# ut-vision/Rot-MVGaze

Hardware: AMD Instinct MI355X
Metric: multi-view samples/sec (fwd+bwd), BxVx3x224x224 (higher is better)
Workload: dtype f32; 1 GPU; C3: ResNet-50, V=4, B=128 per GPU, 3x224x224, fwd+loss+bwd; backbone=ResNet-50, views=4, batch_per_gpu=128, global_batch=128, image=3x224x224, parallelism=dp1, weights=random init, seed 0 (kaiming-normal convs, default Linear), rccl_ranks=1, step_launch=eager: every kernel queued from Python

## Files before the change

include/rotmvgaze.h:

```cpp
#ifndef ROTMVGAZE_H
#define ROTMVGAZE_H

#include <stddef.h>
#include <stdint.h>

#ifdef __cplusplus
extern "C" {
#endif

#define MVG_ABI_VERSION 11

int mvg_abi_version(void);
const char *mvg_last_error(void);
int mvg_device_cus(void);
int mvg_set_scratch(void *ptr, size_t bytes, void *stream);
size_t mvg_scratch_bytes(void);
void *mvg_stream_create_low_priority(void);
int mvg_set_reserved_cus(int n);

enum {
  MVG_K_CONV_FPROP = 0, MVG_K_CONV_DGRAD = 1, MVG_K_CONV_WGRAD = 2, MVG_K_WGRAD_REDUCE = 3,
  MVG_K_BN_FINALIZE = 4, MVG_K_BN_APPLY = 5, MVG_K_BN_BWD_REDUCE = 6, MVG_K_BN_BWD_APPLY = 7,
  MVG_K_POOL = 8, MVG_K_LAYOUT = 9, MVG_K_LINEAR_FPROP = 10, MVG_K_LINEAR_DGRAD = 11,
  MVG_K_LINEAR_WGRAD = 12, MVG_K_ROTCAT = 13, MVG_K_COLSUM = 14, MVG_K_LOSS = 15,
// ... 203 lines not shown
                           int fout, void *stream);
int mvg_linear_dgrad_mixed(const float *dy, const void *wt_bf16, const float *mask, const float *addend, float *dx,
                           int rows, int fin, int fout, void *stream);
int mvg_linear_wgrad_mixed(const float *x, const float *dy, float *dw, float *db, int rows, int fin, int fout,
                           float *workspace, int splits, int accumulate, void *stream);
int mvg_bn_apply_bf16(const uint16_t *y, const float *scale, const float *shift, const uint16_t *residual,
                      const float *res_scale, const float *res_shift, int relu, uint16_t *out, int groups,
                      int64_t rows_per_group, int c, void *stream);
int mvg_bn_bwd_reduce_bf16(const uint16_t *g, const uint16_t *act, const uint16_t *y, const float *mean,
                           const float *invstd, const float *relu_scale, const float *relu_shift, int groups,
                           int64_t rows_per_group, int c, float *s1, float *s2, float *dgamma, float *dbeta,
                           int accumulate, float *workspace, uint16_t *dz_out, void *stream);
int mvg_bn_bwd_apply_bf16(const uint16_t *g, const uint16_t *act, const uint16_t *y, const float *mean,
                          const float *invstd, const float *gamma, const float *s1, const float *s2,
                          const float *relu_scale, const float *relu_shift, int groups, int64_t rows_per_group,
                          int c, uint16_t *dy, uint16_t *dz_out, void *stream);
int mvg_bn_relu_maxpool_fwd_bf16(const uint16_t *y, const float *scale, const float *shift, uint16_t *pooled,
                                 uint8_t *argmax, int groups, int n_per_group, int h, int w, int c, int ho,
                                 int wo, void *stream);
int mvg_bn_relu_maxpool_bwd_reduce_bf16(const uint16_t *g_pooled, const uint8_t *argmax, const uint16_t *y,
                                        const float *mean, const float *invstd, const float *scale,
                                        const float *shift, int groups, int n_per_group, int h, int w, int c,
                                        int ho, int wo, float *s1, float *s2, float *dgamma, float *dbeta,
                                        int accumulate, float *workspace, void *stream);
int mvg_bn_relu_maxpool_bwd_apply_bf16(const uint16_t *g_pooled, const uint8_t *argmax, const uint16_t *y,
                                       const float *mean, const float *invstd, const float *gamma,
                                       const float *scale, const float *shift, const float *s1,
                                       const float *s2, int groups, int n_per_group, int h, int w, int c,
                                       int ho, int wo, uint16_t *dy, void *stream);
int mvg_avgpool_fwd_bf16(const uint16_t *x, float *y, int n, int hw, int c, void *stream);
int mvg_avgpool_bwd_bf16(const float *dy, uint16_t *dx, int n, int hw, int c, void *stream);
int mvg_nchw_to_nhwc8_bf16(const float *src, uint16_t *dst, int n, int c, int h, int w, void *stream);
int mvg_preprocess_u8hwc_resize_bf16(const uint8_t *src, uint16_t *dst, int n, int h, int w, int oh, int ow, float mean0,
                                     float mean1, float mean2, float std0, float std1, float std2, int swap_rb,
                                     void *stream);

int mvg_split_f32(const float *x, void *out_sp, int64_t n, float scale, void *stream);
int mvg_merge_sp(const void *x_sp, float *out, int64_t n, float inv_scale, void *stream);
int mvg_split_weights(const mvg_conv_desc *d, const float *w, void *w_krsc_sp, void *w_crsk_sp, float *stat2, void *items_dev,
                      void *stream);
int mvg_weights_prep_batch(const void *items_dev, int n, int mode, int blocks_per_item , void *stream);
int mvg_conv_stats_partials_split(const mvg_conv_desc *d, int32_t *rows_per_partial);
int mvg_conv_fprop_split(const mvg_conv_desc *d, const void *x_sp, const float *x_sinv, const void *w_sp, const float *w_sinv,
                         float *y, float *stats, void *stream);
int mvg_conv_fprop_split_affine(const mvg_conv_desc *d, const void *x_sp, const float *x_sinv, const void *w_sp, const float *w_sinv,
                                void *out, int out_sp, const float *scale, const float *shift, const void *residual,
                                int residual_sp, int relu, void *stream);
int mvg_conv_fprop_split_affine_ranged(const mvg_conv_desc *d, const void *x_sp, const float *x_sinv, const void *w_sp,
                                       const float *w_sinv, void *out, int out_sp, const float *scale, const float *shift,
                                       const void *residual, int residual_sp, int relu, uint32_t *range_word, void *stream);
int mvg_split_f32_ranged(const float *x, void *out_sp, int64_t n, float scale, uint32_t *range_word, void *stream);
int mvg_conv_dgrad_split(const mvg_conv_desc *d, const void *dy_sp, const float *dy_sinv, const void *w_crsk_sp,
                         const float *w_sinv, float *dx, const float *addend, const void *relu_mask_sp, void *stream);
int mvg_bn_apply_split(const float *y, const float *scale, const float *shift, const void *residual, int residual_sp,
                       const float *res_scale, const float *res_shift, int relu, void *out_sp, uint8_t *relu_bits,
                       int groups, int64_t rows_per_group, int c, void *stream);
int mvg_bn_bwd_reduce_split(const float *g, const uint8_t *relu_bits, const float *y, const float *mean, const float *invstd,
                            const float *relu_scale, const float *relu_shift, int groups, int64_t rows_per_group, int c,
                            float *s1, float *s2, float *dgamma, float *dbeta, int accumulate, float *workspace,
                            float *dz_out, float *mx, const float *gamma, float *dy_sinv, void *stream);
int mvg_bn_bwd_apply_split(const float *g, const float *y, const float *mean, const float *invstd, const float *gamma,
                           const float *s1, const float *s2, const float *relu_scale, const float *relu_shift,
                           int groups, int64_t rows_per_group, int c, void *dy_sp, const float *mx, float *dy_sinv,
                           int dy_sinv_ready, void *stream);
int mvg_bn_relu_maxpool_fwd_split(const float *y, const float *scale, const float *shift, void *pooled_sp,
                                  uint8_t *argmax, int groups, int n_per_group, int h, int w, int c, int ho, int wo,
                                  void *stream);
int mvg_avgpool_fwd_split(const void *x_sp, float *y, int n, int hw, int c, void *stream);
int mvg_act_scales(const void *items_dev, int n, float *slots, int n_slots, void *stream);
int mvg_bn_apply_split_scaled(const float *y, const float *scale, const float *shift, const void *residual, int residual_sp,
                              const float *res_scale, const float *res_shift, const float *res_sinv, int relu, void *out_sp,
                              const float *out_sinv, uint8_t *relu_bits, int groups, int64_t rows_per_group, int c,
                              void *stream);
int mvg_bn_relu_maxpool_fwd_split_scaled(const float *y, const float *scale, const float *shift, void *pooled_sp,
                                         const float *pooled_sinv, uint8_t *argmax, int groups, int n_per_group, int h, int w,
                                         int c, int ho, int wo, void *stream);
int mvg_avgpool_fwd_split_scaled(const void *x_sp, const float *x_sinv, float *y, int n, int hw, int c, void *stream);
int mvg_conv_dgrad_bn_partials_split(const mvg_conv_desc *d);
int mvg_conv_dgrad_split_bnreduce(const mvg_conv_desc *d, const void *dy_sp, const float *dy_sinv, const void *w_crsk_sp,
                                  const float *w_sinv, float *dx, const float *addend, const float *bn_y, const uint8_t *bn_bits,
                                  const float *bn_mean, const float *bn_invstd, const float *relu_scale, const float *relu_shift,
                                  float *partials, float *s1, float *s2, float *dgamma, float *dbeta, int accumulate,
                                  float *mx, const float *bn_gamma, float *dx_dy_sinv, void *stream);
int mvg_conv_dgrad_split_bnapply_bnreduce(const mvg_conv_desc *d, void *dy_sp, const float *dy_sinv, const float *dz, const float *y,
                                          const float *mean, const float *invstd, const float *gamma, const float *un_s1,
                                          const float *un_s2, int64_t rows_per_group, const void *w_crsk_sp, const float *w_sinv,
                                          float *dx, const float *addend, const float *bn_y, const uint8_t *bn_bits,
                                          const float *bn_mean, const float *bn_invstd, const float *relu_scale,
                                          const float *relu_shift, float *partials, float *s1, float *s2, float *dgamma, float *dbeta,
                                          int accumulate, float *mx, const float *bn_gamma, float *dx_dy_sinv, void *stream);
int mvg_conv_fprop_split_stages(const mvg_conv_desc *d);
int mvg_conv_dgrad_split_stages(const mvg_conv_desc *d, int fused_reduce);
int mvg_conv_fprop_split_bnapply(const mvg_conv_desc *d, void *out_sp, const float *out_sinv, const float *bn_y, const float *scale,
                                 const float *shift, const void *residual, int residual_sp, const float *res_scale,
                                 const float *res_shift, const float *res_sinv, uint8_t *relu_bits, const void *w_sp,
                                 const float *w_sinv, float *y, float *stats, void *stream);
int mvg_stem_rowwindow_split(const float *x_nhwc4, void *xw_sp, int64_t images, int h, int w, void *stream);
int mvg_stem_rowwindow_split_nchw(const float *x_nchw, void *xw_sp, int64_t images, int h, int w, void *stream);
int mvg_stem_fprop_split(const mvg_conv_desc *d, const void *xw_sp, const void *w_sp, const float *w_sinv, float *y, float *stats,
                         void *stream);
int mvg_stem_wgrad_splits_split(const mvg_conv_desc *d);
int mvg_stem_wgrad_split(const mvg_conv_desc *d, const void *xw_sp, const void *dy_sp, const float *dy_sinv, float *dw_rw,
                         float *workspace, int splits, int accumulate, void *stream);
int mvg_bn_relu_maxpool_bwd_reduce_split(const float *g_pooled, const uint8_t *argmax, const float *y, const float *mean,
                                         const float *invstd, const float *scale, const float *shift, int groups,
                                         int n_per_group, int h, int w, int c, int ho, int wo, float *s1, float *s2,
                                         float *dgamma, float *dbeta, int accumulate, float *workspace, float *mx, const float *gamma,
                                         float *dy_sinv, void *stream);
int mvg_bn_relu_maxpool_bwd_apply_split(const float *g_pooled, const uint8_t *argmax, const float *y, const float *mean,
                                        const float *invstd, const float *gamma, const float *scale, const float *shift,
                                        const float *s1, const float *s2, int groups, int n_per_group, int h, int w, int c,
                                        int ho, int wo, void *dy_sp, const float *mx, float *dy_sinv, int dy_sinv_ready, void *stream);
int mvg_conv_wgrad_splits_split(const mvg_conv_desc *d);
int mvg_conv_wgrad_split_tile(const mvg_conv_desc *d, int32_t *bm, int32_t *bn, int32_t *incremental);
int mvg_conv_wgrad_split(const mvg_conv_desc *d, const void *x_sp, const void *dy_sp, const float *dy_sinv, float *dw,
                         float *workspace, int splits, int accumulate, void *stream);
int mvg_conv_wgrad_split_slabs(const mvg_conv_desc *d, const void *x_sp, const void *dy_sp, const float *dy_sinv, float *workspace,
                               int splits, void *stream);
int mvg_conv_wgrad_split_xs(const mvg_conv_desc *d, const void *x_sp, const float *x_sinv, const void *dy_sp, const float *dy_sinv,
                            float *dw, float *workspace, int splits, int accumulate, void *stream);
int mvg_conv_wgrad_split_slabs_xs(const mvg_conv_desc *d, const void *x_sp, const float *x_sinv, const void *dy_sp,
                                  const float *dy_sinv, float *workspace, int splits, void *stream);
int mvg_wgrad_reduce_batch(const float *const *host_slabs, float *const *host_dw, const int64_t *host_n, const int32_t *host_splits,
                           const int32_t *host_accumulate, int n, void *stream);

int mvg_absmax_multi(const float *const *host_ptrs, const int64_t *host_counts, float *const *host_out_slots, int n, void *stream);
int mvg_fuse_build_split(const float *img_feat, const float *feat, const float *rel, const int32_t *row_img, const int32_t *row_src_f,
                         const int32_t *row_src_h, void *xf_sp, void *xh_sp, const float *am_img, const float *am_feat,
                         float *xf_sinv, float *xh_sinv, int rows, int cf, int nvec, void *stream);
int mvg_fuse_unbuild(const float *dxh, const float *dxn, const float *rel, const int32_t *seg, const int32_t *vi, float *dfeat, float *da,
                     int da_accumulate, int segments, int views, int dirs, int batch, int cf, int nvec, float *absmax, void *stream);
int mvg_linear_fprop_split(int rows, int fin, int fout, const void *x_sp, const float *x_sinv, const void *w_sp, const float *w_sinv,
                           const float *bias, int relu, void *out, int out_sp, float *out_sinv, const float *bias_absmax,
                           float *out_absmax, void *stream);
int mvg_linear_dgrad_split(int rows, int fin, int fout, const void *dy_sp, const float *dy_sinv, const void *wt_sp, const float *w_sinv,
                           float *dx, const float *addend, const void *relu_mask_sp, float *out_absmax, void *stream);
int mvg_linear_wgrad_split(int rows, int fin, int fout, const void *x_sp, const float *x_sinv, const void *dy_sp, const float *dy_sinv,
                           float *dw, float *workspace, int splits, int accumulate, void *stream);
int mvg_split_colsum(const float *g, int rows, int cols, const float *absmax, void *out_sp, float *out_sinv, float *db, int accumulate,
                     void *stream);

typedef struct mvg_session mvg_session;
typedef struct {
  int32_t depth;
  int32_t num_iter;
  int32_t views, batch;
  int32_t height, width;
  int32_t share_weights, ignore_rotmat;
  int32_t split;
  int32_t raw_u8;
  int32_t in_h, in_w, input_bgr;
} mvg_session_cfg;

int mvg_session_create(const mvg_session_cfg *cfg, mvg_session **out);
#define MVG_SESSION_FP32 0
#define MVG_SESSION_BF16 1
int mvg_session_create_ex(const mvg_session_cfg *cfg, int32_t compute, mvg_session **out);
int mvg_session_compute(const mvg_session *s);
void mvg_session_destroy(mvg_session *s);
int mvg_session_num_tensors(const mvg_session *s);
const char *mvg_session_tensor_name(const mvg_session *s, int i);
int64_t mvg_session_tensor_numel(const mvg_session *s, int i);
size_t mvg_session_workspace_bytes(const mvg_session *s);
int mvg_session_launches(const mvg_session *s);
int mvg_session_num_steps(const mvg_session *s);
const char *mvg_session_step_name(const mvg_session *s, int i);
// ... 12 lines not shown
```

rot-mvgaze_amd/_lib.py:

```python
from __future__ import annotations

import ctypes as C
import os

_HERE = os.path.dirname(os.path.abspath(__file__))
LIB_PATH = os.path.join(_HERE, "csrc", "librotmvgaze_hip.so")

K_FAMILIES = 18
ABI_VERSION = 11
SESSION_FP32, SESSION_BF16 = 0, 1


class ConvDesc(C.Structure):
    _fields_ = [(n, C.c_int32) for n in
                ("groups", "n", "h", "w", "cin", "cout", "r", "s", "stride", "pad", "ho", "wo")]

    @classmethod
    def make(cls, groups, n, h, w, cin, cout, k, stride, pad):
        ho = (h + 2 * pad - k) // stride + 1
        wo = (w + 2 * pad - k) // stride + 1
        return cls(groups, n, h, w, cin, cout, k, k, stride, pad, ho, wo)

    @classmethod
    def linear(cls, rows, fin, fout):
        return cls(1, rows, 1, 1, fin, fout, 1, 1, 1, 0, 1, 1)


class ProfEntry(C.Structure):
    _fields_ = [("launches", C.c_int64), ("ms", C.c_double), ("flops", C.c_double), ("bytes", C.c_double)]


class SessionCfg(C.Structure):
    _fields_ = [(n, C.c_int32) for n in
                ("depth", "num_iter", "views", "batch", "height", "width", "share_weights", "ignore_rotmat", "split", "raw_u8",
                 "in_h", "in_w", "input_bgr")]


_P = C.c_void_p
_I = C.c_int
_I64 = C.c_int64
_F = C.c_float
_D = C.POINTER(ConvDesc)

SIGNATURES = {
    "mvg_abi_version": (_I, []),
    "mvg_last_error": (C.c_char_p, []),
    "mvg_device_cus": (_I, []),
    "mvg_set_scratch": (_I, [_P, C.c_size_t, _P]),
    "mvg_scratch_bytes": (C.c_size_t, []),
    "mvg_set_reserved_cus": (_I, [_I]),
    "mvg_stream_create_low_priority": (_P, []),
    "mvg_prof_enable": (_I, [_I]),
    "mvg_prof_reset": (_I, []),
    "mvg_prof_collect": (_I, [C.POINTER(ProfEntry)]),
    "mvg_prof_family_name": (C.c_char_p, [_I]),
    "mvg_conv_fprop": (_I, [_D, _P, _P, _P, _P, _I, _P, _P]),
    "mvg_conv_fprop_affine": (_I, [_D, _P, _P, _P, _P, _P, _P, _I, _P]),
    "mvg_conv_stats_partials": (_I, [_D, C.POINTER(C.c_int32)]),
    "mvg_conv_dgrad": (_I, [_D, _P, _P, _P, _P, _P, _P]),
    "mvg_conv_wgrad": (_I, [_D, _P, _P, _P, _P, _I, _I, _P]),
    "mvg_conv_wgrad_splits": (_I, [_D]),
    "mvg_linear_wgrad": (_I, [_P, _P, _P, _P, _I, _I, _I, _P, _I, _I, _P]),
    "mvg_fuser_fprop": (_I, [_P, _P, _P, _P, _P, _P, _P, _I, _P, _I, _I, _I, _I, _I, _I, _P, C.c_size_t, _P]),
    "mvg_fuser_wgrad": (_I, [_P, _P, _P, _P, _P, _P, _P, _P, _I, _I, _I, _I, _I, _I, _P, _I, _I, _P]),
    "mvg_linear_workspace_floats": (C.c_size_t, [_I, _I, _I]),
    "mvg_linear_fprop": (_I, [_P, _P, _P, _I, _P, _I, _I, _I, _P, C.c_size_t, _P]),
    "mvg_linear_dgrad": (_I, [_P, _P, _P, _P, _P, _I, _I, _I, _P, C.c_size_t, _P]),
    "mvg_bn_finalize": (_I, [_P, _I, _I, _I, _I64, _I, _P, _P, _P, _P, _F, _F, _P, _P, _P, _P, _P]),
    "mvg_bn_eval_affine": (_I, [_I, _I, _P, _P, _P, _P, _F, _P, _P, _P]),
    "mvg_bn_eval_affine_batch": (_I, [_P, _I, _I, _F, _P]),
    "mvg_bn_apply": (_I, [_P, _P, _P, _P, _P, _P, _I, _P, _I, _I64, _I, _P]),
    "mvg_bn_bwd_reduce": (_I, [_P, _P, _P, _P, _P, _P, _P, _I, _I64, _I, _P, _P, _P, _P, _I, _P, _P, _P]),
    "mvg_split_f32": (_I, [_P, _P, _I64, _F, _P]),
    "mvg_merge_sp": (_I, [_P, _P, _I64, _F, _P]),
    "mvg_split_weights": (_I, [_D, _P, _P, _P, _P, _P, _P]),
    "mvg_weights_prep_batch": (_I, [_P, _I, _I, _I, _P]),
    "mvg_conv_stats_partials_split": (_I, [_D, C.POINTER(C.c_int32)]),
    "mvg_conv_fprop_split": (_I, [_D, _P, _P, _P, _P, _P, _P, _P]),
    "mvg_conv_fprop_split_affine": (_I, [_D, _P, _P, _P, _P, _P, _I, _P, _P, _P, _I, _I, _P]),
    "mvg_conv_dgrad_split": (_I, [_D, _P, _P, _P, _P, _P, _P, _P, _P]),
    "mvg_bn_apply_split": (_I, [_P, _P, _P, _P, _I, _P, _P, _I, _P, _P, _I, _I64, _I, _P]),
    "mvg_bn_bwd_apply_split": (_I, [_P, _P, _P, _P, _P, _P, _P, _P, _P, _I, _I64, _I, _P, _P, _P, _I, _P]),
    "mvg_bn_bwd_reduce_split": (_I, [_P, _P, _P, _P, _P, _P, _P, _I, _I64, _I, _P, _P, _P, _P, _I, _P, _P, _P, _P, _P, _P]),
    "mvg_bn_relu_maxpool_fwd_split": (_I, [_P, _P, _P, _P, _P, _I, _I, _I, _I, _I, _I, _I, _P]),
    "mvg_avgpool_fwd_split": (_I, [_P, _P, _I, _I, _I, _P]),
    "mvg_act_scales": (_I, [_P, _I, _P, _I, _P]),
    "mvg_bn_apply_split_scaled": (_I, [_P, _P, _P, _P, _I, _P, _P, _P, _I, _P, _P, _P, _I, _I64, _I, _P]),
    "mvg_bn_relu_maxpool_fwd_split_scaled": (_I, [_P, _P, _P, _P, _P, _P, _I, _I, _I, _I, _I, _I, _I, _P]),
    "mvg_avgpool_fwd_split_scaled": (_I, [_P, _P, _P, _I, _I, _I, _P]),
    "mvg_conv_wgrad_split_xs": (_I, [_D, _P, _P, _P, _P, _P, _P, _I, _I, _P]),
    "mvg_conv_wgrad_split_slabs_xs": (_I, [_D, _P, _P, _P, _P, _P, _I, _P]),
    "mvg_stem_rowwindow_split": (_I, [_P, _P, _I64, _I, _I, _P]),
    "mvg_stem_rowwindow_split_nchw": (_I, [_P, _P, _I64, _I, _I, _P]),
    "mvg_stem_fprop_split": (_I, [_D, _P, _P, _P, _P, _P, _P]),
    "mvg_stem_wgrad_splits_split": (_I, [_D]),
    "mvg_stem_wgrad_split": (_I, [_D, _P, _P, _P, _P, _P, _I, _I, _P]),
    "mvg_bn_relu_maxpool_bwd_reduce_split": (_I, [_P, _P, _P, _P, _P, _P, _P, _I, _I, _I, _I, _I, _I, _I, _P, _P, _P, _P, _I, _P, _P, _P, _P, _P]),
    "mvg_bn_relu_maxpool_bwd_apply_split": (_I, [_P, _P, _P, _P, _P, _P, _P, _P, _P, _P, _I, _I, _I, _I, _I, _I, _I, _P, _P, _P, _I, _P]),
    "mvg_conv_dgrad_bn_partials_split": (_I, [_D]),
    "mvg_conv_dgrad_split_bnreduce": (_I, [_D, _P, _P, _P, _P, _P, _P, _P, _P, _P, _P, _P, _P, _P, _P, _P, _P, _P, _I, _P, _P, _P, _P]),
    "mvg_conv_dgrad_split_bnapply_bnreduce": (_I, [_D] + [_P] * 9 + [_I64] + [_P] * 15 + [_I, _P, _P, _P, _P]),
    "mvg_conv_fprop_split_stages": (_I, [_D]),
    "mvg_conv_dgrad_split_stages": (_I, [_D, _I]),
    "mvg_conv_fprop_split_bnapply": (_I, [_D] + [_P] * 6 + [_I] + [_P] * 9),
    "mvg_conv_wgrad_splits_split": (_I, [_D]),
    "mvg_conv_wgrad_split_tile": (_I, [_D, C.POINTER(C.c_int32), C.POINTER(C.c_int32), C.POINTER(C.c_int32)]),
    "mvg_conv_wgrad_split": (_I, [_D, _P, _P, _P, _P, _P, _I, _I, _P]),
    "mvg_conv_wgrad_split_slabs": (_I, [_D, _P, _P, _P, _P, _I, _P]),
    "mvg_wgrad_reduce_batch": (_I, [C.POINTER(C.c_void_p), C.POINTER(C.c_void_p), C.POINTER(C.c_int64), C.POINTER(C.c_int32),
                                    C.POINTER(C.c_int32), _I, _P]),
    "mvg_bn_apply_bits": (_I, [_P, _P, _P, _P, _P, _P, _P, _P, _I, _I64, _I, _P]),
    "mvg_bn_bwd_reduce_bits": (_I, [_P, _P, _P, _P, _P, _I, _I64, _I, _P, _P, _P, _P, _I, _P, _P, _P]),
    "mvg_bn_apply_bits_bf16": (_I, [_P, _P, _P, _P, _P, _P, _P, _P, _I, _I64, _I, _P]),
    "mvg_bn_bwd_reduce_bits_bf16": (_I, [_P, _P, _P, _P, _P, _I, _I64, _I, _P, _P, _P, _P, _I, _P, _P, _P]),
    "mvg_bn_bwd_workspace_floats": (C.c_size_t, [_I, _I64, _I]),
    "mvg_bn_bwd_apply": (_I, [_P, _P, _P, _P, _P, _P, _P, _P, _P, _P, _I, _I64, _I, _P, _P, _P]),
    "mvg_maxpool3x3s2_fwd": (_I, [_P, _P, _P, _I, _I, _I, _I, _I, _I, _P]),
    "mvg_maxpool3x3s2_bwd": (_I, [_P, _P, _P, _I, _I, _I, _I, _I, _I, _P]),
    "mvg_bn_relu_maxpool_fwd": (_I, [_P, _P, _P, _P, _P, _I, _I, _I, _I, _I, _I, _I, _P]),
    "mvg_bn_relu_maxpool_bwd_reduce": (_I, [_P, _P, _P, _P, _P, _P, _P, _I, _I, _I, _I, _I, _I, _I, _P, _P, _P, _P, _I, _P,
                                            _P]),
    "mvg_bn_relu_maxpool_bwd_apply": (_I, [_P, _P, _P, _P, _P, _P, _P, _P, _P, _P, _I, _I, _I, _I, _I, _I, _I, _P, _P]),
    "mvg_bn_eval_bwd": (_I, [_P, _P, _P, _P, _P, _P, _P, _P, _P, _F, _I, _I64, _I, _P, _P, _P, _P, _I, _P, _P]),
    "mvg_bn_eval_bwd_workspace_floats": (C.c_size_t, [_I, _I64, _I]),
    "mvg_bn_relu_maxpool_eval_bwd": (_I, [_P, _P, _P, _P, _P, _P, _P, _P, _F, _I, _I, _I, _I, _I, _I, _I, _P, _P, _P, _I, _P,
                                          _P]),
    "mvg_avgpool_fwd": (_I, [_P, _P, _I, _I, _I, _P]),
    "mvg_avgpool_bwd": (_I, [_P, _P, _I, _I, _I, _P]),
    "mvg_nchw_to_nhwc4": (_I, [_P, _P, _I, _I, _I, _I, _P]),
    "mvg_nhwc4_to_nchw": (_I, [_P, _P, _I, _I, _I, _I, _P]),
    "mvg_preprocess_u8hwc": (_I, [_P, _P, _I, _I, _I, _F, _F, _F, _F, _F, _F, _I, _P]),
    "mvg_gaze_lp_loss": (_I, [_P, _P, _I, _I, _P, _P, _P]),
    "mvg_preprocess_u8hwc_resize": (_I, [_P, _P, _I, _I, _I, _I, _I, _F, _F, _F, _F, _F, _F, _I, _P]),
    "mvg_multi_erase_nchw": (_I, [_P, _P, _P, _I, _I, _I, _I, _I, _P]),
    "mvg_rotation_matrix_2d": (_I, [_P, _P, _I, _I, _P]),
    "mvg_relative_rotation": (_I, [_P, _P, _P, _P, _I, _I, _I, _P]),
    "mvg_rotcat_fwd": (_I, [_P, _P, _P, _P, _P, _P, _I, _I, _I, _I, _P]),
    "mvg_rotcat_bwd": (_I, [_P, _P, _P, _P, _I, _I, _I, _I, _P]),
    "mvg_rotcat_ext_fwd": (_I, [_P, _P, _P, _P, _P, _P, _P, _I, _I, _I, _I, _I, _P]),
    "mvg_rotcat_ext_bwd": (_I, [_P, _I, _P, _P, _P, _I, _I, _I, _I, _P]),
    "mvg_ibn_scales": (_I, [_P, _P, _P, _P, _P, _I, _F, _F, _P, _I, _I, _I, _P]),
    "mvg_paircat_fwd": (_I, [_P, _P, _P, _P, _P, _P, _P, _I, _I, _I, _P]),
    "mvg_paircat_bwd": (_I, [_P, _P, _P, _P, _P, _P, _I, _I, _I, _P]),
    "mvg_segment_sum": (_I, [_P, _I64, _I, _P, _P, _I, _I, _I, _I, _P]),
    "mvg_axpby": (_I, [_P, _P, _F, _F, _I64, _P]),
    "mvg_scale_by": (_I, [_P, _P, _P, _I64, _P]),
    "mvg_linear_skinny_fwd": (_I, [_P, _P, _P, _P, _I, _I, _I, _P]),
    "mvg_linear_skinny_bwd": (_I, [_P, _P, _P, _P, _P, _P, _P, _I, _I, _I, _I, _P, _P]),
    "mvg_adam_step": (_I, [_P, _P, _P, _P, _I64, _F, _F, _F, _F, _F, _I, _P]),
    "mvg_gaze_angular_loss": (_I, [_P, _P, _I, _F, _P, _I, _P, _P, _P]),
    "mvg_gaze_angular_loss_multi": (_I, [_P, _P, _I, _I, _I, C.POINTER(C.c_float), _P, _P, _P]),
    "mvg_adam_step_dev": (_I, [_P, _P, _P, _P, _I64, _P, _P, _F, _F, _F, _F, _P]),
    "mvg_absmax_multi": (_I, [C.POINTER(C.c_void_p), C.POINTER(C.c_int64), C.POINTER(C.c_void_p), _I, _P]),
    "mvg_fuse_build_split": (_I, [_P, _P, _P, _P, _P, _P, _P, _P, _P, _P, _P, _P, _I, _I, _I, _P]),
    "mvg_fuse_unbuild": (_I, [_P, _P, _P, _P, _P, _P, _P, _I, _I, _I, _I, _I, _I, _I, _P, _P]),
    "mvg_linear_fprop_split": (_I, [_I, _I, _I, _P, _P, _P, _P, _P, _I, _P, _I, _P, _P, _P, _P]),
    "mvg_linear_dgrad_split": (_I, [_I, _I, _I, _P, _P, _P, _P, _P, _P, _P, _P, _P]),
    "mvg_linear_wgrad_split": (_I, [_I, _I, _I, _P, _P, _P, _P, _P, _P, _I, _I, _P]),
    "mvg_split_colsum": (_I, [_P, _I, _I, _P, _P, _P, _P, _I, _P]),
    "mvg_cast_weights_bf16": (_I, [_D, _P, _I, _P, _P, _P]),
    "mvg_conv_fprop_bf16": (_I, [_D, _P, _P, _P, _P, _I, _P, _P]),
    "mvg_conv_stats_partials_bf16": (_I, [_D, C.POINTER(C.c_int32)]),
    "mvg_conv_fprop_bf16_affine": (_I, [_D, _P, _P, _P, _P, _P, _P, _I, _P]),
    "mvg_conv_dgrad_bf16": (_I, [_D, _P, _P, _P, _P, _P, _P]),
    "mvg_conv_dgrad_bn_partials_bf16": (_I, [_D]),
    "mvg_conv_dgrad_bf16_bnreduce": (_I, [_D, _P, _P, _P, _P, _P, _P, _P, _P, _P, _P, _P, _P, _P, _P, _P, _I, _P]),
    "mvg_conv_wgrad_bf16": (_I, [_D, _P, _P, _P, _P, _I, _I, _P]),
    "mvg_stem_rowwindow_bf16": (_I, [_P, _P, _I64, _I, _I, _P]),
    "mvg_stem_fprop_bf16": (_I, [_D, _P, _P, _P, _P, _P]),
    "mvg_stem_wgrad_splits_bf16": (_I, [_D]),
    "mvg_stem_wgrad_bf16": (_I, [_D, _P, _P, _P, _P, _I, _I, _P]),
    "mvg_conv_wgrad_splits_bf16": (_I, [_D]),
    "mvg_conv_wgrad_bf16_slabs": (_I, [_D, _P, _P, _P, _I, _P]),
    "mvg_linear_fprop_mixed": (_I, [_P, _P, _P, _I, _P, _I, _I, _I, _P]),
    "mvg_linear_dgrad_mixed": (_I, [_P, _P, _P, _P, _P, _I, _I, _I, _P]),
    "mvg_linear_wgrad_mixed": (_I, [_P, _P, _P, _P, _I, _I, _I, _P, _I, _I, _P]),
    "mvg_bn_apply_bf16": (_I, [_P, _P, _P, _P, _P, _P, _I, _P, _I, _I64, _I, _P]),
    "mvg_bn_bwd_reduce_bf16": (_I, [_P, _P, _P, _P, _P, _P, _P, _I, _I64, _I, _P, _P, _P, _P, _I, _P, _P, _P]),
    "mvg_bn_bwd_apply_bf16": (_I, [_P, _P, _P, _P, _P, _P, _P, _P, _P, _P, _I, _I64, _I, _P, _P, _P]),
    "mvg_bn_relu_maxpool_fwd_bf16": (_I, [_P, _P, _P, _P, _P, _I, _I, _I, _I, _I, _I, _I, _P]),
    "mvg_bn_relu_maxpool_bwd_reduce_bf16": (_I, [_P, _P, _P, _P, _P, _P, _P, _I, _I, _I, _I, _I, _I, _I, _P, _P, _P, _P, _I,
                                                 _P, _P]),
    "mvg_bn_relu_maxpool_bwd_apply_bf16": (_I, [_P, _P, _P, _P, _P, _P, _P, _P, _P, _P, _I, _I, _I, _I, _I, _I, _I, _P, _P]),
# ... 56 lines not shown
```

rot-mvgaze_amd/backbone.py:

```python
from __future__ import annotations

import math
import os
from dataclasses import dataclass
from typing import Callable, Dict, List, NamedTuple, Optional

import numpy as np
import torch

from . import ops
from ._lib import ConvDesc
from .arch import RANGE_OVER_BITS, BackboneSpec, ConvSpec, backbone_spec, range_unit_names

Tensor = torch.Tensor
BN_EPS, BN_MOMENTUM = 1e-5, 0.1
IMAGE_MEAN, IMAGE_STD = (0.485, 0.456, 0.406), (0.229, 0.224, 0.225)


BN_APPLY_DGRAD_MAX_COUT = 512


def bn_apply_dgrad_eligible(c: ConvSpec, *, split: bool, trained: bool, fused_in: bool, carries_reduce: bool,
                            need_dimg: bool = False) -> bool:
    return bool(split and trained and not need_dimg and fused_in and carries_reduce
                and c.k == 1 and c.stride == 1 and c.pad == 0 and c.cin in (64, 128)
                and c.cout % 32 == 0 and c.cout <= BN_APPLY_DGRAD_MAX_COUT)


def bn_apply_dgrad_units(spec: BackboneSpec, *, split: bool = True, bf16: bool = False, training: bool = True,
                         need_dimg: bool = False, fuse_bn_split: bool = True, enabled: bool = True) -> List[str]:
    on = enabled and split and not bf16 and fuse_bn_split
    nb = len(spec.blocks)
    return [blk.convs[-1].name for bi, blk in reversed(list(enumerate(spec.blocks)))
            if bn_apply_dgrad_eligible(blk.convs[-1], split=on, trained=training, fused_in=bi < nb - 1,
                                       carries_reduce=len(blk.convs) > 1, need_dimg=need_dimg)]


BN_APPLY_FPROP_MAX_CIN = 512


def bn_apply_fprop_eligible(producer: ConvSpec, consumer: ConvSpec, *, split: bool, trained: bool, residual: bool = True,
                            relu: bool = True, single_stage: bool = True) -> bool:
    return bool(split and trained and residual and relu and single_stage
                and consumer.k == 1 and consumer.stride == 1 and consumer.pad == 0 and consumer.cout in (64, 128)
                and consumer.cin == producer.cout and consumer.cin % 32 == 0 and consumer.cin <= BN_APPLY_FPROP_MAX_CIN)


def bn_apply_fprop_pairs(spec: BackboneSpec, *, split: bool = True, bf16: bool = False, training: bool = True, enabled: bool = True,
                         single_stage: Optional[Callable[[ConvSpec], bool]] = None) -> List[tuple]:
    on = enabled and split and not bf16
    return [(a.convs[-1].name, b.convs[0].name) for a, b in zip(spec.blocks[:-1], spec.blocks[1:])
            if bn_apply_fprop_eligible(a.convs[-1], b.convs[0], split=on, trained=training,
                                       single_stage=True if single_stage is None else single_stage(b.convs[0]))]


class GradSink:

    def view(self, p: torch.nn.Parameter) -> Tensor:
        raise NotImplementedError

    def accumulate(self, p: torch.nn.Parameter) -> bool:
        raise NotImplementedError

    def publish(self, ps: List[torch.nn.Parameter]) -> None:
        raise NotImplementedError


@dataclass(slots=True)
class _Unit:
    spec: Optional[ConvSpec] = None
    desc: Optional[ConvDesc] = None
    x_in: Optional[Tensor] = None
    y: Optional[Tensor] = None
    out: Optional[Tensor] = None
    mean: Optional[Tensor] = None
    invstd: Optional[Tensor] = None
    relu: bool = False
    rows: int = 0
    w: Optional[Tensor] = None
    trained: bool = True
    pool: Optional[tuple] = None
    relu_affine: Optional[tuple] = None
    fused_s12: Optional[object] = None
    relu_bits: Optional[Tensor] = None
    split: bool = False
    stem_rw: bool = False


class _Fwd(NamedTuple):
    out: Tensor
    affine: Optional[tuple] = None
    pending: Optional[tuple] = None


class Backbone:
    _guard_scale = 1
    _debug_units: Optional[list] = None

    def __init__(self, depth: int, params: Dict[str, Tensor], prefix: str = "_feat_extractor.0."):
        self.spec: BackboneSpec = backbone_spec(depth, prefix)
        self.p = params
        self.fc_dim = self.spec.fc_dim
        self.overlap_wgrad = True
        self.overlap_head = True
        self.wgrad_low_priority = True
        self.grad_streams: List[torch.cuda.Stream] = []
        self._wg_stream: Optional[torch.cuda.Stream] = None
        self._wg_low = True
        self.act_dtype = torch.float32
        self.relu_bits = True
        self.split = os.environ.get("MVG_SPLIT", "1") != "0"
        self.fuse_bn_split = True
        self.fuse_bn_apply_dgrad = True
        self.fuse_bn_apply_fprop = True
        self.stem_rowwindow = True
        self.split_eval = True
        self.split_eval_guard: Optional[str] = None
        self._range_record: Optional[Tensor] = None
        self._range_slot: Dict[str, int] = {n: i for i, n in enumerate(range_unit_names(depth, prefix))}
        self._range_live = False
        self._range_tripped = False
        self.bf16_fold_eval = True
        self._wprep_infer_ok = False
        self._wk_cache: Dict[str, tuple] = {}
        self.batch_weight_prep = True
        self._wprep: Optional[Dict[str, tuple]] = None
        self._wprep_state = None
        self._wprep_versions = None
        self._ascale_state = None
        self._act_sinv: Optional[Dict[str, Tensor]] = None
        self._wg_defer: Optional[list] = None
        self._split_now = self.split
        self._stem_rw = False
        self._stem_w8 = None

    @property
    def bf16(self) -> bool:
        return self.act_dtype == torch.bfloat16

    def _prepare_weights(self, dev, reuse: bool = False) -> Dict[str, tuple]:
        mode = 0 if self.bf16 else 1
        stem_rw = self._stem_rw
        convs = [c for c in self.spec.all_convs() if not (mode == 1 and c.cin == 3 and not stem_rw)]
        key = (mode, stem_rw, str(dev), tuple(self.p[c.name + ".weight"].data_ptr() for c in convs))
        if self._wprep_state is None or self._wprep_state[0] != key:
            out, rows = {}, []
            wstat = torch.zeros(len(convs), 2, dtype=torch.float32, device=dev)
            self._stem_w8 = None
            for ci, c in enumerate(convs):
                wsrc = self.p[c.name + ".weight"]
                assert wsrc.is_contiguous(memory_format=torch.channels_last) or (c.k == 1 and wsrc.is_contiguous())
                rs = c.k * c.k
                if mode == 1 and c.cin == 3:
                    assert c.k == 7
                    self._stem_w8 = torch.zeros(c.cout, 7, 8, 4, dtype=torch.float32, device=dev)
                    wk = ops.sp_empty(c.cout, 7 * 32, device=dev)
                    wk.sinv = wstat[ci, 1:2]
                    out[c.name] = (wk, None)
                    rows.append([self._stem_w8.data_ptr(), wk.data_ptr(), 0, c.cout | (7 << 32), 32 | (32 << 32), wstat[ci].data_ptr()])
                    continue
                if mode == 0 and c.cin == 3 and stem_rw:
                    assert c.k == 7
                    self._stem_w8 = torch.zeros(2 * c.cout, 7, 16, 4, dtype=torch.float32, device=dev)
                    wk = torch.empty(2 * c.cout, 7, 1, 64, dtype=torch.bfloat16, device=dev)
                    out[c.name] = (wk, None)
                    rows.append([self._stem_w8.data_ptr(), wk.data_ptr(), 0, (2 * c.cout) | (7 << 32), 64 | (64 << 32), wstat[ci].data_ptr()])
                    continue
                if mode == 1:
                    wk = ops.sp_empty(c.cout, rs * c.cin, device=dev)
                    wt = ops.sp_empty(c.cin, rs * c.cout, device=dev)
                    wk.sinv = wt.sinv = wstat[ci, 1:2]
                    cin_pad = c.cin
                else:
                    cin_pad = 8 if c.cin == 3 else c.cin
                    wk = torch.empty(c.cout, c.k, c.k, cin_pad, dtype=torch.bfloat16, device=dev)
                    wt = None if c.cin == 3 else torch.empty(cin_pad, c.k, c.k, c.cout, dtype=torch.bfloat16, device=dev)
                out[c.name] = (wk, wt)
                rows.append([wsrc.data_ptr(), wk.data_ptr(), wt.data_ptr() if wt is not None else 0, c.cout | (rs << 32),
                             c.cin | (cin_pad << 32), wstat[ci].data_ptr()])
            table = torch.tensor(rows, dtype=torch.int64).to(dev)
            self._wprep_state = (key, out, table, len(rows), mode, wstat)
        elif (reuse and self._wprep_infer_ok and
              self._wprep_versions == tuple(self.p[c.name + ".weight"]._version for c in self.spec.all_convs())):
            return self._wprep_state[1]
        _, out, table, n, mode, wstat = self._wprep_state
        self._wprep_infer_ok = reuse
        if mode == 1:
            wstat.zero_()
            if self._stem_w8 is not None:
                self._stem_w8[:, :, 1:, :3].copy_(self.p[self.spec.stem.name + ".weight"].detach().permute(0, 2, 3, 1))
        elif self._stem_w8 is not None:
            wsrc, co = self.p[self.spec.stem.name + ".weight"].detach().permute(0, 2, 3, 1), self.spec.stem.cout
            self._stem_w8[:co, :, 1:8, :3].copy_(wsrc)
            self._stem_w8[co:, :, 3:10, :3].copy_(wsrc)
        ops.weights_prep_batch(table, n, mode)
        self._wprep_versions = tuple(self.p[c.name + ".weight"]._version for c in self.spec.all_convs())
# ... 368 lines not shown
    def _unit_params(self, c: ConvSpec) -> List[torch.nn.Parameter]:
        return [self.p[c.name + ".weight"], self.p[c.bn + ".weight"], self.p[c.bn + ".bias"]]

    def _bn_bwd(self, u: _Unit, g: Tensor, need_dz: bool, sink: GradSink, defer_apply: bool = False):
        if not u.trained:
            return self._bn_bwd_eval(u, g, need_dz, sink)
        c = u.spec
        G = u.y.shape[0]
        gp, bp, acc = self._bn_params(c, sink)
        if u.fused_s12 is not None and u.split:
            (s12, sinv), u.fused_s12 = u.fused_s12, None
            dy = ops.sp_empty(*u.y.shape, device=g.device)
            if defer_apply:
                dy.sinv = sinv
                dy.bn_apply = (g, u.y, u.mean, u.invstd, gp.detach(), s12[0], s12[1], u.rows)
            else:
                ops.bn_bwd_apply_split(g, u.y, u.mean, u.invstd, gp.detach(), s12[0], s12[1], G, u.rows, c.cout, dy, None, s12[2], sinv)
            return dy, (g if need_dz else None)
        if u.fused_s12 is not None:
            s12, u.fused_s12 = u.fused_s12, None
            dy = torch.empty_like(g) if need_dz else g
            ops.bn_bwd_apply(g, None, u.y, u.mean, u.invstd, gp.detach(), s12[0], s12[1], G, u.rows, c.cout, dy, None, None)
            return dy, (g if need_dz else None)
        s12 = torch.empty(3 if u.split else 2, G, c.cout, dtype=torch.float32, device=g.device)
        ra = u.relu_affine
        act = u.out if (u.relu and ra is None) else None
        if u.split:
            assert not (u.relu and ra is None) or u.relu_bits is not None
            sinv = torch.empty(1, dtype=torch.float32, device=g.device)
            bits = u.relu_bits
            ra = None if bits is not None else ra
            ops.bn_bwd_reduce_split(g, bits, u.y, u.mean, u.invstd, G, u.rows, c.cout, s12[0], s12[1], sink.view(gp), sink.view(bp),
                                    acc, s12[2], ra, dz_out=g if bits is not None else None, gamma=gp.detach(), dy_sinv=sinv)
            dy = ops.sp_empty(*u.y.shape, device=g.device)
            ops.bn_bwd_apply_split(g, u.y, u.mean, u.invstd, gp.detach(), s12[0], s12[1], G, u.rows, c.cout, dy, ra, s12[2], sinv)
            return dy, (g if need_dz else None)
        if need_dz and u.relu_bits is not None:
            ops.bn_bwd_reduce_bits(g, u.relu_bits, u.y, u.mean, u.invstd, G, u.rows, c.cout, s12[0], s12[1], sink.view(gp),
                                   sink.view(bp), acc, dz_out=g)
        else:
            ops.bn_bwd_reduce(g, act, u.y, u.mean, u.invstd, G, u.rows, c.cout, s12[0], s12[1], sink.view(gp), sink.view(bp),
                              acc, ra, dz_out=g if need_dz else None)
        if need_dz:
            dy = torch.empty_like(g)
            ops.bn_bwd_apply(g, None, u.y, u.mean, u.invstd, gp.detach(), s12[0], s12[1], G, u.rows, c.cout, dy, None, None)
            return dy, g
        ops.bn_bwd_apply(g, act, u.y, u.mean, u.invstd, gp.detach(), s12[0], s12[1], G, u.rows, c.cout, g, None, ra)
        return g, None

    def _bn_bwd_eval(self, u: _Unit, g: Tensor, need_dz: bool, sink: GradSink):
        c = u.spec
        G = u.y.shape[0]
        gp, bp, acc = self._bn_params(c, sink)
        rm, rv = self.p[c.bn + ".running_mean"], self.p[c.bn + ".running_var"]
        if u.relu_bits is not None:
            mask = {"relu_bits": u.relu_bits}
        elif u.relu_affine is not None:
            mask = {"relu_affine": u.relu_affine}
        elif u.relu:
            mask = {"act": u.out}
        else:
            mask = {}
        dy = torch.empty_like(g) if need_dz else g
        ops.bn_eval_bwd(g, u.y, gp.detach(), rm, rv, BN_EPS, G, u.rows, c.cout, dy, sink.view(gp), sink.view(bp), acc,
                        dz_out=g if need_dz else None, **mask)
        return dy, (g if need_dz else None)

    def _side(self, dev) -> "torch.cuda.Stream":
        if self._wg_stream is None or self._wg_stream.device != dev or self._wg_low != self.wgrad_low_priority:
            old = self._wg_stream if (self._wg_stream is not None and self._wg_stream.device == dev) else None
            self._wg_low = self.wgrad_low_priority
            try:
                if not self._wg_low:
                    raise RuntimeError
                self._wg_stream = ops.low_priority_stream(dev)
            except RuntimeError:
                self._wg_stream = torch.cuda.Stream(device=dev)
            if old is not None:
                self._wg_stream.wait_stream(old)
            self.grad_streams[:] = [self._wg_stream]
        return self._wg_stream

    def _conv_bwd(self, u: _Unit, dy: Tensor, need_dx: bool, addend: Optional[Tensor], sink: GradSink,
                  fuse_for: Optional[_Unit] = None):
        dx = None
        if getattr(dy, "bn_apply", None) is not None:
            dx = torch.empty(ops.sp_shape(u.x_in), dtype=torch.float32, device=dy.device)
            self._dgrad(u, dy, dx, addend, fuse_for, sink)
            need_dx = False
        if self.overlap_wgrad and dy.is_cuda:
            side = self._side(dy.device)
            side.wait_stream(torch.cuda.current_stream())
            with torch.cuda.stream(side):
                self._wgrad(u, dy, sink)
            if getattr(dy, "sinv", None) is not None:
                dy.sinv.record_stream(side)
            dy.record_stream(side)
            u.x_in.record_stream(side)
            if getattr(u.x_in, "sinv", None) is not None:
                u.x_in.sinv.record_stream(side)
        else:
            self._wgrad(u, dy, sink)
        if need_dx:
            dx = torch.empty(ops.sp_shape(u.x_in), dtype=torch.float32, device=dy.device) if u.split else torch.empty_like(u.x_in)
            self._dgrad(u, dy, dx, addend, fuse_for, sink)
        return dx

    def _wgrad(self, u: _Unit, dy: Tensor, sink: GradSink):
        c = u.spec
        wp = self.p[c.name + ".weight"]
        if u.split:
            ops.conv_wgrad_split(u.desc, u.x_in, dy, sink.view(wp), sink.accumulate(wp), defer=self._wg_defer)
        elif u.stem_rw and self.bf16:
            dw16 = torch.empty(2 * c.cout, 7, 16, 4, dtype=torch.float32, device=dy.device)
            ops.stem_wgrad_bf16(u.desc, u.x_in, dy, dw16, False)
            self._stem_grad(wp, sink, dw16[:c.cout, :, 1:8, :3], dw16[c.cout:, :, 3:10, :3])
        elif u.stem_rw:
            dw8 = torch.empty(c.cout, 7, 8, 4, dtype=torch.float32, device=dy.device)
            ops.stem_wgrad_split(u.desc, u.x_in, dy, dw8, False)
            self._stem_grad(wp, sink, dw8[:, :, 1:, :3])
        elif c.cin == 3:
            dw4 = torch.empty(c.cout, c.k, c.k, u.desc.cin, dtype=torch.float32, device=dy.device)
            ops.conv_wgrad(u.desc, u.x_in, dy, dw4, False)
            self._stem_grad(wp, sink, dw4[..., :3])
        else:
            ops.conv_wgrad(u.desc, u.x_in, dy, sink.view(wp), sink.accumulate(wp), defer=self._wg_defer if self.bf16 else None)

    @staticmethod
    def _stem_grad(wp: torch.nn.Parameter, sink: GradSink, dw: Tensor, dw_odd: Optional[Tensor] = None):
        gv = sink.view(wp).permute(0, 2, 3, 1)
        if sink.accumulate(wp):
            gv.add_(dw)
        else:
            gv.copy_(dw)
        if dw_odd is not None:
            gv.add_(dw_odd)

    def _flush_wgrad_reduces(self, dev):
        if not self._wg_defer:
            return
        if self.overlap_wgrad and dev.type == "cuda":
            with torch.cuda.stream(self._side(dev)):
                ops.wgrad_reduce_batch(self._wg_defer)
        else:
            ops.wgrad_reduce_batch(self._wg_defer)

    def _dgrad(self, u: _Unit, dy: Tensor, dx: Tensor, addend: Optional[Tensor], fuse_for: Optional[_Unit] = None,
               sink: Optional[GradSink] = None):
        U = fuse_for
        if (self.bf16 and U is not None and self.fuse_bn_split and u.spec.cin != 3 and u.desc.cin % 64 == 0 and u.desc.cout % 64 == 0
                and (not U.relu or U.relu_bits is not None or U.relu_affine is not None)):
            c = U.spec
            gp, bp, acc = self._bn_params(c, sink)
            s12 = torch.empty(2, dx.shape[0], c.cout, dtype=torch.float32, device=dx.device)
            ops.conv_dgrad_bf16_bnreduce(u.desc, dy, u.w, dx, addend, U.y, U.relu_bits, U.mean, U.invstd,
                                         None if U.relu_bits is not None else U.relu_affine, s12[0], s12[1], sink.view(gp),
                                         sink.view(bp), acc)
            U.fused_s12 = s12
            return
        if u.split:
            if U is not None and U.split and self.fuse_bn_split:
                c = U.spec
                gp, bp, acc = self._bn_params(c, sink)
                s12 = torch.empty(3, dx.shape[0], c.cout, dtype=torch.float32, device=dx.device)
                sinv = torch.empty(1, dtype=torch.float32, device=dx.device)
                ra = None if U.relu_bits is not None else U.relu_affine
                pend = getattr(dy, "bn_apply", None)
                if pend is not None:
                    dz, y, mean, invstd, gamma, us1, us2, rows = pend
                    dy.bn_apply = None
                    ops.conv_dgrad_split_bnapply_bnreduce(u.desc, dy, dy.sinv, dz, y, mean, invstd, gamma, us1, us2, rows, u.w, dx,
                                                          addend, U.y, U.relu_bits, U.mean, U.invstd, ra, s12[0], s12[1],
                                                          sink.view(gp), sink.view(bp), acc, s12[2], gp.detach(), sinv)
                else:
                    ops.conv_dgrad_split_bnreduce(u.desc, dy, u.w, dx, addend, U.y, U.relu_bits, U.mean, U.invstd, ra, s12[0], s12[1],
                                                  sink.view(gp), sink.view(bp), acc, s12[2], gp.detach(), sinv)
                U.fused_s12 = (s12, sinv)
            else:
                ops.conv_dgrad_split(u.desc, dy, u.w, dx, addend)
        else:
            ops.conv_dgrad(u.desc, dy, u.w, dx, None, addend)

    def _stem_bn_bwd(self, stem: _Unit, g: Tensor, V: int, B: int, sink: GradSink) -> Tensor:
        argmax, scale, shift, H1, W1, Hp, Wp = stem.pool
        sc = stem.spec
        P = self.p
        gp, bp, acc = self._bn_params(sc, sink)
        stem_sp = stem.stem_rw and not self.bf16
        s12 = torch.empty(3 if stem_sp else 2, V, sc.cout, dtype=torch.float32, device=g.device)
        if not stem.trained:
            dy = torch.empty_like(stem.y)
            ops.bn_relu_maxpool_eval_bwd(g, argmax, stem.y, scale, shift, gp.detach(), P[sc.bn + ".running_mean"],
                                         P[sc.bn + ".running_var"], BN_EPS, V, B, H1, W1, sc.cout, Hp, Wp, dy, sink.view(gp),
                                         sink.view(bp), acc)
        elif stem_sp:
            sinv = torch.empty(1, dtype=torch.float32, device=g.device)
            ops.bn_relu_maxpool_bwd_reduce_split(g, argmax, stem.y, stem.mean, stem.invstd, scale, shift, V, B, H1, W1, sc.cout, Hp, Wp,
                                                 s12[0], s12[1], sink.view(gp), sink.view(bp), acc, s12[2], gp.detach(), sinv)
            dy = ops.sp_empty(*stem.y.shape, device=g.device)
            ops.bn_relu_maxpool_bwd_apply_split(g, argmax, stem.y, stem.mean, stem.invstd, gp.detach(), scale, shift, s12[0], s12[1],
                                                V, B, H1, W1, sc.cout, Hp, Wp, dy, s12[2], sinv)
        else:
            ops.bn_relu_maxpool_bwd_reduce(g, argmax, stem.y, stem.mean, stem.invstd, scale, shift, V, B, H1, W1, sc.cout, Hp, Wp,
                                           s12[0], s12[1], sink.view(gp), sink.view(bp), acc)
            dy = torch.empty_like(stem.y)
            ops.bn_relu_maxpool_bwd_apply(g, argmax, stem.y, stem.mean, stem.invstd, gp.detach(), scale, shift, s12[0], s12[1],
                                          V, B, H1, W1, sc.cout, Hp, Wp, dy)
        return dy

    def backward(self, tape: dict, dfeat: Tensor, sink: GradSink, need_dimg: bool = False):
        V, B = tape["V"], tape["B"]
        units: List[_Unit] = tape["units"]
        if self.bf16 and not all(u.trained for u in units):
            raise NotImplementedError("backward through eval-mode BatchNorm (running statistics) is not implemented on the "
                                      "bf16 path: call model.train() for gradient steps, or use the fp32 model")
        Hc, Wc = tape["final_hw"]
        if need_dimg and self.bf16:
            raise NotImplementedError("d(loss)/d(img) is not produced by the bf16 path")
        if tape.get("wprep_versions") is not None and tape["wprep_versions"] != getattr(self, "_wprep_versions", None):
            raise RuntimeError("backward of a tape whose bf16 / sp weight copies were overwritten by a later forward with "
                               "DIFFERENT weights (forward, optimizer step, forward, then backward of the first call): "
                               "backward-data would run with the new weights.  Run backward before the weights change "
                               "(PyTorch raises its version-counter error in the same situation)")
        g = torch.empty(V, B, Hc, Wc, self.fc_dim, dtype=self.act_dtype, device=dfeat.device)
        ops.avgpool_bwd(dfeat.contiguous(), g, V * B, Hc * Wc, self.fc_dim)
        self._wg_defer = []
        blocks = tape["blocks"]
        for bi in range(len(blocks) - 1, -1, -1):
            idx, ds_idx = blocks[bi]
            last = units[idx[-1]]
            prev_last = units[blocks[bi - 1][0][-1]] if bi > 0 else None
            done: List[torch.nn.Parameter] = []
            below = units[idx[-2]]
            merge = self.fuse_bn_apply_dgrad and bn_apply_dgrad_eligible(
                last.spec, split=last.split and not self.bf16, trained=last.trained, fused_in=last.fused_s12 is not None,
                carries_reduce=below.split and self.fuse_bn_split, need_dimg=need_dimg)
            dy, dz = self._bn_bwd(last, g, True, sink, defer_apply=merge)
            d = self._conv_bwd(last, dy, True, None, sink, fuse_for=below)
            done += self._unit_params(last.spec)
            last.y = last.out = None
            del dy
            for k in range(len(idx) - 2, -1, -1):
                u = units[idx[k]]
                dy, _ = self._bn_bwd(u, d, False, sink)
                if k == 0:
                    d = self._conv_bwd(u, dy, True, dz if ds_idx is None else None, sink,
                                       fuse_for=prev_last if ds_idx is None else None)
                else:
                    d = self._conv_bwd(u, dy, True, None, sink, fuse_for=units[idx[k - 1]])
                done += self._unit_params(u.spec)
                u.y = u.out = None
            if ds_idx is not None:
                ud = units[ds_idx]
                dyd, _ = self._bn_bwd(ud, dz, False, sink)
                self._conv_bwd(ud, dyd, False, None, sink)
                self._dgrad(ud, dyd, d, d, prev_last, sink)
                done += self._unit_params(ud.spec)
                ud.y = ud.out = None
            self._flush_wgrad_reduces(g.device)
            sink.publish(done)
            g = d
            if "debug" in tape:
                tape["debug"].append(g.clone())
        stem = units[0]
        dy = self._stem_bn_bwd(stem, g, V, B, sink)
        dx0 = self._conv_bwd(stem, dy, need_dimg, None, sink)
        self._flush_wgrad_reduces(g.device)
        self._wg_defer = None
        sink.publish(self._unit_params(stem.spec))
        if self._wg_stream is not None and dy.is_cuda and (self.overlap_wgrad or not torch.cuda.is_current_stream_capturing()):
            torch.cuda.current_stream().wait_stream(self._wg_stream)
        if not need_dimg:
            return None
        H, W = dx0.shape[2], dx0.shape[3]
        outs = []
        for v in range(V):
            o = torch.empty(B, 3, H, W, dtype=torch.float32, device=dx0.device)
            ops.nhwc4_to_nchw(dx0[v], o, B, 3, H, W)
            outs.append(o)
        return outs
```

rot-mvgaze_amd/csrc/bf16_tile.h:

```cpp
#pragma once
#include "conv_shared.h"
#include "bn_math.h"
#include "elem.h"

namespace mvg {

typedef __bf16 bf16x8 __attribute__((ext_vector_type(8)));
typedef short s16x4 __attribute__((ext_vector_type(4)));

__device__ __forceinline__ float bf_lo(unsigned v) { return __uint_as_float(v << 16); }
__device__ __forceinline__ float bf_hi(unsigned v) { return __uint_as_float(v & 0xFFFF0000u); }
__device__ __forceinline__ unsigned pack_bf2(float a, float b) {
  const __bf16 x = (__bf16)a, y = (__bf16)b;
  return (unsigned)__builtin_bit_cast(unsigned short, x) | ((unsigned)__builtin_bit_cast(unsigned short, y) << 16);
}

__device__ __forceinline__ void ld8(const float *p, float (&v)[8]) {
  const float4 a = *reinterpret_cast<const float4 *>(p), b = *reinterpret_cast<const float4 *>(p + 4);
  v[0] = a.x; v[1] = a.y; v[2] = a.z; v[3] = a.w; v[4] = b.x; v[5] = b.y; v[6] = b.z; v[7] = b.w;
}

constexpr unsigned RANGE_OVER_BITS = 0x477FF000u;
__device__ __forceinline__ unsigned range_bits(unsigned mx, float v) {
  const unsigned b = __float_as_uint(v) & 0x7FFFFFFFu;
  return b > mx ? b : mx;
}
__device__ __forceinline__ void range_commit(unsigned mx, unsigned *lds, unsigned *__restrict__ word, int tid) {
#pragma unroll
  for (int o = 32; o > 0; o >>= 1) {
    const unsigned other = (unsigned)__shfl_xor((int)mx, o, 64);
    mx = other > mx ? other : mx;
  }
  __syncthreads();
  if ((tid & 63) == 0) lds[tid >> 6] = mx;
  __syncthreads();
  if (tid == 0) {
    unsigned m = lds[0];
    for (int k = 1; k < 4; ++k) m = lds[k] > m ? lds[k] : m;
    if (m > *word) atomicMax(word, m);
  }
}

template <int BM, int BN, int PASSES, bool BNF, bool AFF = false>
constexpr int bf16_epilogue_bytes() {
  return (BM / PASSES) * (BN + 4) * 4 + BM * 4 + (BNF ? 4 * BN * 4 : 0) + (AFF ? 2 * BN * 4 : 0);
}

template <int BM, int BN, int WGM, bool DGRAD, bool F32IO, int PASSES = 1, bool ACC16 = false, bool BNF = false, bool LIN = false, int WGN = 2,
          bool AFF = false, bool RNG = false, class AccT>
__device__ __forceinline__ void bf16_epilogue(const IgemmParams &p, const IgemmClass &c, AccT &acc,
                                              unsigned short *smem, int tid, int g, int mtile, int ntile) {
  constexpr int NT = WGM * WGN * 64;
  constexpr int WTM = BM / WGM, WTN = BN / WGN;
  constexpr int TS = ACC16 ? 16 : 32, NE = ACC16 ? 4 : 16;
  constexpr int TM = WTM / TS, TN = WTN / TS;
  constexpr int LDO = BN + 4;
  const int lane = tid & 63, wave = tid >> 6;
  const int wm = wave / WGN, wn = wave % WGN;
  const int li = ACC16 ? (lane & 15) : (lane & 31), lh = ACC16 ? (lane >> 4) : (lane >> 5);
  auto erow = [&](int e) { return ACC16 ? 4 * lh + e : (e & 3) + 8 * (e >> 2) + 4 * lh; };
  const int ohw = c.out_h * c.out_w;
  const long long row_base = (long long)mtile * BM + wm * WTM;
  const float osc = F32IO ? (p.a_sinv ? *p.a_sinv : 1.f) * (p.b_sinv ? *p.b_sinv : 1.f) : 1.f;
  float lin_scale = 1.f, lin_max = 0.f;
  unsigned rng_max = 0u;
  static_assert(!RNG || (F32IO && !DGRAD && !LIN && !BNF && !AFF && WGM * WGN == 4), "bf16_epilogue: RNG is a forward form of the split conv kernels");
  if constexpr (LIN && F32IO) {
    if (!DGRAD && p.out_sp && p.out_sinv) {
      const float bound = (float)p.ktotal * 1073741824.f * osc + (p.bias_absmax ? *p.bias_absmax : 0.f);
      lin_scale = sp_scale_for(bound);
      if (tid == 0 && mtile == 0 && ntile == 0 && g == 0) *p.out_sinv = 1.f / lin_scale;
    }
  }
  if (!DGRAD && !AFF && p.stats) {
    long long cnt_ll = c.rows_per_group - row_base;
    const int cnt = cnt_ll <= 0 ? 0 : (cnt_ll > WTM ? WTM : (int)cnt_ll);
#pragma unroll
    for (int j = 0; j < TN; ++j) {
      const int col = ntile * BN + wn * WTN + j * TS + li;
      float csum = 0.f;
#pragma unroll
      for (int i = 0; i < TM; ++i)
#pragma unroll
        for (int e = 0; e < NE; ++e) {
          const int r = i * TS + erow(e);
          csum += (r < cnt) ? acc[i][j][e] : 0.f;
        }
      csum += __shfl_xor(csum, 32, 64);
      if (ACC16) csum += __shfl_xor(csum, 16, 64);
      const float mean = cnt > 0 ? csum / (float)cnt : 0.f;
      float q = 0.f;
#pragma unroll
      for (int i = 0; i < TM; ++i)
#pragma unroll
        for (int e = 0; e < NE; ++e) {
          const int r = i * TS + erow(e);
          const float dlt = acc[i][j][e] - mean;
          q += (r < cnt) ? dlt * dlt : 0.f;
        }
      q += __shfl_xor(q, 32, 64);
      if (ACC16) q += __shfl_xor(q, 16, 64);
      long long P = p.stats_partials ? p.stats_partials : (long long)c.mtiles_per_group * WGM;
      long long pi = (long long)mtile * WGM + wm;
      if (lh == 0 && col < p.ncols && (pi < P || p.stats_fold)) {
        int nc = p.ncols, ch = col;
        if (p.stats_fold) {
          nc = p.ncols >> 1;
          pi = 2 * pi + (col >= nc);
          ch = col - (col >= nc ? nc : 0);
          P *= 2;
        }
        float *st = p.stats + (((long long)g * P + pi) * 2) * nc;
        st[ch] = csum * osc;
        st[nc + ch] = q * (osc * osc);
      }
    }
  }
  static_assert(WGM % PASSES == 0, "bf16_epilogue: the wave rows must divide into the passes");
  constexpr int PR = BM / PASSES;
  float *ot = reinterpret_cast<float *>(smem);
  int *rowoff = reinterpret_cast<int *>(ot + PR * LDO);
  for (int r = tid; r < BM; r += NT) {
    const long long m = (long long)mtile * BM + r;
    int off = -1;
    if (m < c.rows_per_group) {
      if (DGRAD && p.cls_step == 2) {
        const int rr = (int)m;
        const int img = (int)fdiv((unsigned)rr, c.ohw_div), rem = rr - img * ohw;
        const int y2 = (int)fdiv((unsigned)rem, c.ow_div), x2 = rem - y2 * c.out_w;
        off = ((img * p.full_h + 2 * y2 + c.cls_py) * p.full_w + 2 * x2 + c.cls_px) * p.ncols;
      } else {
        off = (int)m * p.ncols;
      }
    }
    rowoff[r] = off;
  }
  const long long gelems = DGRAD ? (long long)p.imgs_per_group * p.full_h * p.full_w * p.ncols
                                 : c.rows_per_group * (long long)p.ncols;
  unsigned short *out_g = reinterpret_cast<unsigned short *>(p.out) + (long long)g * gelems;
  const unsigned short *add_g = p.addend ? reinterpret_cast<const unsigned short *>(p.addend) + (long long)g * gelems : nullptr;
  const unsigned short *mask_g = p.mask ? reinterpret_cast<const unsigned short *>(p.mask) + (long long)g * gelems : nullptr;
  float *out_f = p.out + (long long)g * gelems;
  const float *add_f = p.addend ? p.addend + (long long)g * gelems : nullptr;
  const float *mask_f = p.mask ? p.mask + (long long)g * gelems : nullptr;
  constexpr int CV = BN / 8;
  const bool bnf = BNF && DGRAD && p.bn_part != nullptr;
  bool quad = false;
  if constexpr (F32IO && DGRAD && !LIN) quad = !p.mask && (p.ncols % BN) == 0;
  float bn_s1[8], bn_s2[8], bn_mx[8];
  const bool bn_aff = bnf && p.bn_rscale != nullptr;
  float *bnc = reinterpret_cast<float *>(smem) + (BM / PASSES) * LDO + BM;
  if (bnf) {
    for (int cc = tid; cc < BN; cc += NT) {
      const int colc = ntile * BN + cc;
      const bool ok = colc < p.ncols;
      bnc[cc] = ok ? p.bn_mean[(long long)g * p.ncols + colc] : 0.f;
      bnc[BN + cc] = ok ? p.bn_invstd[(long long)g * p.ncols + colc] : 0.f;
      bnc[2 * BN + cc] = (ok && bn_aff) ? p.bn_rscale[(long long)g * p.ncols + colc] : 0.f;
      bnc[3 * BN + cc] = (ok && bn_aff) ? p.bn_rshift[(long long)g * p.ncols + colc] : 0.f;
    }
#pragma unroll
    for (int k = 0; k < 8; ++k) bn_s1[k] = bn_s2[k] = bn_mx[k] = 0.f;
  }
  float *affc = reinterpret_cast<float *>(smem) + (BM / PASSES) * LDO + BM;
  if constexpr (AFF) {
    static_assert(!DGRAD && !F32IO && !BNF && !LIN, "bf16_epilogue: AFF is the forward form of the bf16 storage kernels");
    for (int cc = tid; cc < BN; cc += NT) {
      const int colc = ntile * BN + cc;
      const bool ok = colc < p.ncols;
      affc[cc] = ok ? p.scale[colc] : 0.f;
      affc[BN + cc] = ok ? p.bias[colc] : 0.f;
    }
  }
#pragma unroll
  for (int ph = 0; ph < PASSES; ++ph) {
  if (PASSES > 1 && ph > 0) __syncthreads();
  if (wm / (WGM / PASSES) == ph) {
#pragma unroll
    for (int i = 0; i < TM; ++i)
#pragma unroll
      for (int j = 0; j < TN; ++j)
#pragma unroll
        for (int e = 0; e < NE; ++e)
          ot[((wm % (WGM / PASSES)) * WTM + i * TS + erow(e)) * LDO + wn * WTN + j * TS + li] = acc[i][j][e];
  }
  __syncthreads();
  auto store_rows = [&](int it) {
    const int v = tid + it * NT;
    const int rl = v / CV, cv = v - rl * CV;
    const int r = ph * PR + rl;
    const int col = ntile * BN + cv * 8;
    const int off = rowoff[r];
    if (off < 0 || col >= p.ncols) return;
    const float4 lo = *reinterpret_cast<const float4 *>(ot + rl * LDO + cv * 8);
    const float4 hi = *reinterpret_cast<const float4 *>(ot + rl * LDO + cv * 8 + 4);
    float x[8] = {lo.x, lo.y, lo.z, lo.w, hi.x, hi.y, hi.z, hi.w};
    if constexpr (F32IO) {
#pragma unroll
      for (int k = 0; k < 8; ++k) x[k] *= osc;
    }
    if constexpr (AFF) {
      asm volatile("" ::: "memory");
      float sa[8], sb[8];
      ld8(affc + cv * 8, sa);
      ld8(affc + BN + cv * 8, sb);
#pragma unroll
      for (int k = 0; k < 8; ++k) x[k] = __builtin_fmaf(x[k], sa[k], sb[k]);
      if (add_g) {
        const u32x4 a = *reinterpret_cast<const u32x4 *>(add_g + off + col);
        const unsigned aa[4] = {a.x, a.y, a.z, a.w};
#pragma unroll
        for (int k = 0; k < 4; ++k) {
          x[2 * k] += bf_lo(aa[k]);
          x[2 * k + 1] += bf_hi(aa[k]);
        }
      }
      if (p.relu) {
#pragma unroll
        for (int k = 0; k < 8; ++k) x[k] = fmaxf(x[k], 0.f);
      }
      u32x4 o;
      o.x = pack_bf2(x[0], x[1]);
      o.y = pack_bf2(x[2], x[3]);
      o.z = pack_bf2(x[4], x[5]);
      o.w = pack_bf2(x[6], x[7]);
      *reinterpret_cast<u32x4 *>(out_g + off + col) = o;
// ... 96 lines not shown
        typedef float f4v __attribute__((ext_vector_type(4)));
        f4v s0 = {x[0], x[1], x[2], x[3]}, s1 = {x[4], x[5], x[6], x[7]};
        __builtin_nontemporal_store(s0, reinterpret_cast<f4v *>(out_f + off + col));
        __builtin_nontemporal_store(s1, reinterpret_cast<f4v *>(out_f + off + col + 4));
      } else {
        *reinterpret_cast<float4 *>(out_f + off + col) = make_float4(x[0], x[1], x[2], x[3]);
        *reinterpret_cast<float4 *>(out_f + off + col + 4) = make_float4(x[4], x[5], x[6], x[7]);
      }
      return;
    }
    if (mask_g) {
      const u32x4 m = *reinterpret_cast<const u32x4 *>(mask_g + off + col);
      const unsigned mm[4] = {m.x, m.y, m.z, m.w};
#pragma unroll
      for (int k = 0; k < 4; ++k) {
        x[2 * k] = bf_lo(mm[k]) > 0.f ? x[2 * k] : 0.f;
        x[2 * k + 1] = bf_hi(mm[k]) > 0.f ? x[2 * k + 1] : 0.f;
      }
    }
    if (add_g) {
      const u32x4 a = *reinterpret_cast<const u32x4 *>(add_g + off + col);
      const unsigned aa[4] = {a.x, a.y, a.z, a.w};
#pragma unroll
      for (int k = 0; k < 4; ++k) {
        x[2 * k] += bf_lo(aa[k]);
        x[2 * k + 1] += bf_hi(aa[k]);
      }
    }
    u32x4 o;
    if (bnf) {
      const u32x4 yv = *reinterpret_cast<const u32x4 *>(reinterpret_cast<const unsigned short *>(p.bn_y) + (long long)g * gelems + off + col);
      const unsigned yw[4] = {yv.x, yv.y, yv.z, yv.w};
      unsigned bits = p.bn_bits ? (unsigned)p.bn_bits[((long long)g * gelems + off + col) >> 3] : 0xFFu;
      asm volatile("" ::: "memory");
      if (bn_aff) {
        float bn_ra[8], bn_rb[8];
        ld8(bnc + 2 * BN + cv * 8, bn_ra);
        ld8(bnc + 3 * BN + cv * 8, bn_rb);
        bits = 0u;
#pragma unroll
        for (int k = 0; k < 4; ++k) {
          bits |= (relu_on(bf_lo(yw[k]), bn_ra[2 * k], bn_rb[2 * k]) ? 1u : 0u) << (2 * k);
          bits |= (relu_on(bf_hi(yw[k]), bn_ra[2 * k + 1], bn_rb[2 * k + 1]) ? 1u : 0u) << (2 * k + 1);
        }
      }
      unsigned ow[4];
#pragma unroll
      for (int k = 0; k < 4; ++k) {
        const float y0 = bf_lo(yw[k]), y1 = bf_hi(yw[k]);
        const bool on0 = ((bits >> (2 * k)) & 1u) != 0u, on1 = ((bits >> (2 * k + 1)) & 1u) != 0u;
        ow[k] = pack_bf2(on0 ? x[2 * k] : 0.f, on1 ? x[2 * k + 1] : 0.f);
        const float d0 = bf_lo(ow[k]), d1 = bf_hi(ow[k]);
        bn_s1[2 * k] += d0;
        bn_s1[2 * k + 1] += d1;
        bn_s2[2 * k] = __builtin_fmaf(d0, y0, bn_s2[2 * k]);
        bn_s2[2 * k + 1] = __builtin_fmaf(d1, y1, bn_s2[2 * k + 1]);
      }
      o.x = ow[0]; o.y = ow[1]; o.z = ow[2]; o.w = ow[3];
    } else {
      o.x = pack_bf2(x[0], x[1]);
      o.y = pack_bf2(x[2], x[3]);
      o.z = pack_bf2(x[4], x[5]);
      o.w = pack_bf2(x[6], x[7]);
    }
    *reinterpret_cast<u32x4 *>(out_g + off + col) = o;
  };
  if (quad) {
    constexpr int HB = BN / 2;
    const int cq = tid % CV;
    const int cA = cq * 4, cB = HB + cq * 4;
    const int colA = ntile * BN + cA, colB = ntile * BN + cB;
#pragma unroll 1
    for (int it = 0; it < PR * CV / NT; ++it) {
      const int rl = (tid + it * NT) / CV;
      const int off = rowoff[ph * PR + rl];
      if (off < 0) continue;
      const float4 qa = *reinterpret_cast<const float4 *>(ot + rl * LDO + cA);
      const float4 qb = *reinterpret_cast<const float4 *>(ot + rl * LDO + cB);
      float x[8] = {qa.x * osc, qa.y * osc, qa.z * osc, qa.w * osc, qb.x * osc, qb.y * osc, qb.z * osc, qb.w * osc};
      if (add_f) {
        const float4 a0 = *reinterpret_cast<const float4 *>(add_f + off + colA), a1 = *reinterpret_cast<const float4 *>(add_f + off + colB);
        x[0] += a0.x; x[1] += a0.y; x[2] += a0.z; x[3] += a0.w; x[4] += a1.x; x[5] += a1.y; x[6] += a1.z; x[7] += a1.w;
      }
      if (bnf) {
        const float *yg = p.bn_y + (long long)g * gelems + off;
        const float4 y0 = *reinterpret_cast<const float4 *>(yg + colA), y1 = *reinterpret_cast<const float4 *>(yg + colB);
        const float yy[8] = {y0.x, y0.y, y0.z, y0.w, y1.x, y1.y, y1.z, y1.w};
        unsigned bits = 0xFFu;
        if (p.bn_bits) {
          const uint8_t *bb = p.bn_bits + (((long long)g * gelems + off) >> 2);
          bits = (bb[colA >> 2] & 0xFu) | ((bb[colB >> 2] & 0xFu) << 4);
        }
        asm volatile("" ::: "memory");
        auto ld44 = [&](const float *base, float (&v)[8]) {
          const float4 u = *reinterpret_cast<const float4 *>(base + cA), w = *reinterpret_cast<const float4 *>(base + cB);
          v[0] = u.x; v[1] = u.y; v[2] = u.z; v[3] = u.w; v[4] = w.x; v[5] = w.y; v[6] = w.z; v[7] = w.w;
        };
        if (bn_aff) {
          float bn_ra[8], bn_rb[8];
          ld44(bnc + 2 * BN, bn_ra);
          ld44(bnc + 3 * BN, bn_rb);
#pragma unroll
          for (int k = 0; k < 8; ++k) bits = (bits & ~(1u << k)) | ((relu_on(yy[k], bn_ra[k], bn_rb[k]) ? 1u : 0u) << k);
        }
        float bn_mu[8], bn_is[8];
        ld44(bnc, bn_mu);
        ld44(bnc + BN, bn_is);
#pragma unroll
        for (int k = 0; k < 8; ++k) {
          x[k] = ((bits >> k) & 1u) != 0u ? x[k] : 0.f;
          bn_mx[k] = fmaxf(bn_mx[k], fabsf(x[k]));
          bn_s1[k] += x[k];
          bn_s2[k] += x[k] * xhat(yy[k], bn_mu[k], bn_is[k]);
        }
      }
      if (p.nt_out) {
        typedef float f4v __attribute__((ext_vector_type(4)));
        const f4v s0 = {x[0], x[1], x[2], x[3]}, s1 = {x[4], x[5], x[6], x[7]};
        __builtin_nontemporal_store(s0, reinterpret_cast<f4v *>(out_f + off + colA));
        __builtin_nontemporal_store(s1, reinterpret_cast<f4v *>(out_f + off + colB));
      } else {
        *reinterpret_cast<float4 *>(out_f + off + colA) = make_float4(x[0], x[1], x[2], x[3]);
        *reinterpret_cast<float4 *>(out_f + off + colB) = make_float4(x[4], x[5], x[6], x[7]);
      }
    }
    continue;
  }
  bool plain4 = false;
  if constexpr (F32IO && !LIN) plain4 = p.nt_out && !p.scale && !p.bias && !p.addend && !p.mask && !p.out_sp && !bnf && !p.relu;
  if (plain4) {
    constexpr int CV4 = BN / 4;
#pragma unroll
    for (int it = 0; it < PR * CV4 / NT; ++it) {
      const int v = tid + it * NT;
      const int rl = v / CV4, c4 = v - rl * CV4;
      const int col = ntile * BN + c4 * 4;
      const int off = rowoff[ph * PR + rl];
      if (off < 0 || col >= p.ncols) continue;
      const float4 q = *reinterpret_cast<const float4 *>(ot + rl * LDO + c4 * 4);
      typedef float f4v __attribute__((ext_vector_type(4)));
      const f4v sv = {q.x * osc, q.y * osc, q.z * osc, q.w * osc};
      __builtin_nontemporal_store(sv, reinterpret_cast<f4v *>(out_f + off + col));
    }
  } else if constexpr (BNF) {
#pragma unroll 1
    for (int it = 0; it < PR * CV / NT; ++it) store_rows(it);
  } else {
#pragma unroll
    for (int it = 0; it < PR * CV / NT; ++it) store_rows(it);
  }
  }
  if constexpr (RNG) range_commit(rng_max, reinterpret_cast<unsigned *>(smem), p.out_absmax, tid);
  if constexpr (LIN && F32IO) {
    if (p.out_absmax) {
#pragma unroll
      for (int o = 32; o > 0; o >>= 1) lin_max = fmaxf(lin_max, __shfl_xor(lin_max, o, 64));
      __syncthreads();
      float *wred = reinterpret_cast<float *>(smem);
      if (lane == 0) wred[wave] = lin_max;
      __syncthreads();
      if (tid == 0) {
        float mx = wred[0];
        for (int k = 1; k < NT / 64; ++k) mx = fmaxf(mx, wred[k]);
        if (mx > 0.f) atomicMax(p.out_absmax, __float_as_uint(mx));
      }
      __syncthreads();
// ... 44 lines not shown
```

rot-mvgaze_amd/csrc/conv_shared.h:

```cpp
#pragma once
#include <stdlib.h>

#include "common.h"

namespace mvg {


typedef float f32x16 __attribute__((ext_vector_type(16)));
typedef unsigned int u32x4 __attribute__((ext_vector_type(4)));

__device__ __forceinline__ unsigned pred_off(unsigned off, bool ok) { return off | ((unsigned)(!ok) << 31); }
__device__ __forceinline__ float4 buf_ld16(__amdgpu_buffer_rsrc_t r, unsigned byte_off) {
  const u32x4 v = __builtin_amdgcn_raw_buffer_load_b128(r, byte_off, 0, 0);
  return make_float4(__uint_as_float(v.x), __uint_as_float(v.y), __uint_as_float(v.z), __uint_as_float(v.w));
}
__device__ __forceinline__ __amdgpu_buffer_rsrc_t make_rsrc(const void *base, long long bytes) {
  unsigned n = bytes > 0x7FFFFFF0ll ? 0x7FFFFFF0u : (bytes < 0 ? 0u : (unsigned)bytes);
  const unsigned long long b = (unsigned long long)base;
  const unsigned lo = __builtin_amdgcn_readfirstlane((unsigned)b);
  const unsigned hi = __builtin_amdgcn_readfirstlane((unsigned)(b >> 32));
  n = __builtin_amdgcn_readfirstlane(n);
  void *ub = (void *)(((unsigned long long)hi << 32) | lo);
  return __builtin_amdgcn_make_buffer_rsrc(ub, 0, (int)n, 0x00020000);
}
// ... 13 lines not shown
}
__device__ __forceinline__ unsigned fdiv(unsigned n, const FastDiv &f) {
  const unsigned t = __umulhi(f.mul, n);
  return (t + ((n - t) >> f.sh1)) >> f.sh2;
}

struct IgemmClass {
  int out_h, out_w;
  int ntaps, tap_ns, tap_r0, tap_s0;
  int ktotal;
  int cls_py, cls_px, cls_cy, cls_cx;
  int mtiles_per_group;
  long long rows_per_group;
  FastDiv tap_ns_div, ohw_div, ow_div;
  int korder;
  FastDiv per_div;
  long long unit0;
  int tile0;
  int KT;
  int part0;
};

struct IgemmParams {
  const float *a;
  const float *b;
  float *out;
  const float *bias;
  const float *scale;
  const float *mask;
  const float *addend;
  float *stats;
  int relu;
  int groups;
  int out_h, out_w;
  int src_h, src_w;
  int src_c;
  int src_c_shift;
  int ncols;
  int r, s, stride_shift, stride, pad;
  int ktotal;
  int cin;
  int rs;
  long long rows_per_group;
  long long src_img_stride;
  int imgs_per_group;
  int mtiles_per_group, ntiles;
  int ntaps, tap_ns, tap_r0, tap_s0, tap_step;
  int cls_step, cls_py, cls_px, cls_cy, cls_cx;
  int full_h, full_w;
  long long a_group_bytes;
  long long b_bytes;
  FastDiv tap_ns_div;
  FastDiv ohw_div, ow_div;
  int splits, ktiles_per_split;
  float *slab;
  int sk_tiles;
  int no_remap;
  int nt_out;
  int ncls;
  IgemmClass cls[4];
  int b_row_len;
  int stats_partials;
  const float *bn_y, *bn_mean, *bn_invstd, *bn_rscale, *bn_rshift;
  float *bn_part;
  int bn_parts;
  int addend_sp, out_sp, mask_sp;
  const float *a_sinv, *b_sinv;
  unsigned *out_absmax;
  float *out_sinv;
  const float *bias_absmax;
  int stride_w, pad_w;
  int stats_fold;
  int bn_part_rows;
  const unsigned char *bn_bits;
  const float *rc_feat, *rc_rel;
  const int *rc_row_img, *rc_row_src;
  int rc_cf, rc_nvec, rc_nvec_shift;
  long long rc_img_bytes, rc_feat_bytes;
  const float *bna_dz, *bna_y, *bna_mean, *bna_invstd, *bna_gamma, *bna_s1, *bna_s2;
  float bna_inv_rows;
  const float *fap_y, *fap_scale, *fap_shift, *fap_res_scale, *fap_res_shift, *fap_res_sinv;
  const void *fap_res;
  unsigned short *fap_bits;
};

__device__ __forceinline__ int xcd_remap(int orig, int nwg) {
  const int q = nwg >> 3, rr = nwg & 7, xcd = orig & 7;
  const int base = (xcd < rr) ? xcd * (q + 1) : rr * (q + 1) + (xcd - rr) * q;
  return base + (orig >> 3);
}


struct WgradParams {
  const float *x;
  const float *dy;
  float *out;
  int h, w, cin, cout, r, s, stride, pad, ho, wo;
  int ncols;
  long long pixels;
  long long pixels_per_split;
  long long x_bytes;
  int mtiles, ntiles;
  int accumulate;
  float *db;
  const float *rc_feat, *rc_rel;
  const int *rc_row_img, *rc_row_src;
  int rc_cf, rc_nvec;
  long long rc_img_bytes, rc_feat_bytes;
  FastDiv ohw_div, wo_div, cin_div, s_div;
  const float *dy_sinv;
  const float *x_sinv;
  int stride_w, pad_w;
};

static __global__ __launch_bounds__(256) void wgrad_reduce_kernel(const float *__restrict__ slabs, float *__restrict__ dw,
                                                           long long n4, int splits, int accumulate, int lanes) {
  __shared__ float4 sh[256];
  const int cols = 256 / lanes;
  const int c = threadIdx.x % cols, l = threadIdx.x / cols;
  const long long i = (long long)blockIdx.x * cols + c;
  float4 s = make_float4(0.f, 0.f, 0.f, 0.f);
  if (i < n4)
    for (int k = l; k < splits; k += lanes) {
      const float4 v = reinterpret_cast<const float4 *>(slabs)[(long long)k * n4 + i];
      s.x += v.x;
      s.y += v.y;
      s.z += v.z;
      s.w += v.w;
    }
  sh[threadIdx.x] = s;
  __syncthreads();
  if (l == 0 && i < n4) {
    float4 t = accumulate ? reinterpret_cast<const float4 *>(dw)[i] : make_float4(0.f, 0.f, 0.f, 0.f);
    for (int k = 0; k < lanes; ++k) {
      const float4 v = sh[k * cols + c];
      t.x += v.x;
      t.y += v.y;
      t.z += v.z;
      t.w += v.w;
    }
    reinterpret_cast<float4 *>(dw)[i] = t;
  }
}

static double alg_cin(const mvg_conv_desc *d) { return d->cin == 4 ? 3.0 : (double)d->cin; }

static int ilog2_exact(int v) {
  int s = 0;
  while ((1 << s) < v) ++s;
  return ((1 << s) == v) ? s : -1;
}

static int validate(const mvg_conv_desc *d) {
  MVG_REQUIRE(d != nullptr, "conv: null descriptor");
  MVG_REQUIRE(d->groups > 0 && d->n > 0 && d->h > 0 && d->w > 0 && d->cin > 0 && d->cout > 0, "conv: bad sizes");
  MVG_REQUIRE(d->stride == 1 || d->stride == 2, "conv: stride must be 1 or 2 (got %d)", d->stride);
  MVG_REQUIRE(d->ho == (d->h + 2 * d->pad - d->r) / d->stride + 1 && d->wo == (d->w + 2 * d->pad - d->s) / d->stride + 1,
              "conv: ho/wo inconsistent with h/w/pad/stride");
  MVG_REQUIRE(d->cin % 4 == 0, "conv: cin %% 4 != 0 (%d)", d->cin);
  if (d->r * d->s > 1) {
    MVG_REQUIRE(ilog2_exact(d->cin) >= 0 && ilog2_exact(d->cout) >= 0, "conv: r*s>1 needs power-of-two channels");
  }
  MVG_REQUIRE((long long)d->n * d->ho * d->wo < (1LL << 31) && (long long)d->n * d->h * d->w < (1LL << 31),
              "conv: rows per group overflow int32");
  return 0;
}
// ... 74 lines not shown
  p.src_h = d->ho;
  p.src_w = d->wo;
  p.src_c = d->cout;
  p.src_c_shift = (d->r * d->s > 1) ? ilog2_exact(d->cout) : 0;
  p.ncols = d->cin;
  p.r = d->r;
  p.s = d->s;
  p.rs = d->r * d->s;
  p.stride = d->stride;
  p.stride_shift = d->stride == 2 ? 1 : 0;
  p.pad = d->pad;
  p.ktotal = d->r * d->s * d->cout;
  p.b_row_len = p.ktotal;
  p.cin = d->cin;
  p.src_img_stride = (long long)d->ho * d->wo * d->cout;
  p.imgs_per_group = d->n;
  p.full_h = d->h;
  p.full_w = d->w;
  p.a_group_bytes = (long long)a_elem * d->n * p.src_img_stride;
  p.b_bytes = (long long)b_elem * d->cin * p.b_row_len;
  MVG_REQUIRE(p.a_group_bytes < 0x7FFFFFF0ll && p.b_bytes < 0x7FFFFFF0ll, "%s: a group / the weights exceed 2 GiB", what);
  return 0;
}

static __global__ __launch_bounds__(256) void dgrad_empty_class_kernel(uint4 *__restrict__ dx, const uint4 *__restrict__ addend,
                                                                       long long n, int sub_h, int sub_w, int full_h, int full_w,
                                                                       int cv, int py, int px) {
  const long long stride = (long long)gridDim.x * blockDim.x;
  for (long long i = (long long)blockIdx.x * blockDim.x + threadIdx.x; i < n; i += stride) {
    const int cc = (int)(i % cv);
    long long t = i / cv;
    const int x2 = (int)(t % sub_w);
    t /= sub_w;
    const int y2 = (int)(t % sub_h);
    const long long img = t / sub_h;
    const long long off = ((img * full_h + 2 * y2 + py) * full_w + 2 * x2 + px) * cv + cc;
    dx[off] = addend ? addend[off] : make_uint4(0u, 0u, 0u, 0u);
  }
}

struct DgradDropped {
  int n;
  struct { int py, px, sub_h, sub_w; } c[4];
};
static void dgrad_plan_classes(IgemmParams &p, const mvg_conv_desc *d, bool keep_tapless, DgradDropped &dropped) {
  const int step = d->stride;
  p.ncls = 0;
  dropped.n = 0;
  for (int py = 0; py < step; ++py)
    for (int px = 0; px < step; ++px) {
      const int sub_h = (d->h - py + step - 1) / step, sub_w = (d->w - px + step - 1) / step;
      if (sub_h <= 0 || sub_w <= 0) continue;
      const int r0 = (py + d->pad) % step, s0 = (px + d->pad) % step;
      const int nr = r0 < d->r ? (d->r - r0 + step - 1) / step : 0;
      const int ns = s0 < d->s ? (d->s - s0 + step - 1) / step : 0;
      if (nr * ns == 0 && !keep_tapless) {
        dropped.c[dropped.n++] = {py, px, sub_h, sub_w};
        continue;
      }
      IgemmClass &c = p.cls[p.ncls++];
      c = make_class(d->n, sub_h, sub_w, nr * ns, ns > 0 ? ns : 1, r0, s0, d->cout);
      c.cls_py = py;
      c.cls_px = px;
      c.cls_cy = (py + d->pad - r0) / step;
      c.cls_cx = (px + d->pad - s0) / step;
      if (p.ncls == 1) {
        p.tap_step = step;
        p.cls_step = step;
        p.rows_per_group = c.rows_per_group;
        p.ktotal = c.ktotal;
        p.out_h = sub_h;
        p.out_w = sub_w;
      }
    }
  for (int i = 1; i < p.ncls; ++i)
    for (int j = i; j > 0 && p.cls[j].ktotal > p.cls[j - 1].ktotal; --j) {
      const IgemmClass t = p.cls[j];
      p.cls[j] = p.cls[j - 1];
      p.cls[j - 1] = t;
    }
  p.no_remap = p.ncls > 1;
}

static int dgrad_classes(IgemmParams &p, const mvg_conv_desc *d, bool keep_tapless, int dx_elem, void *dx, const void *addend,
                         hipStream_t st) {
  DgradDropped dropped;
  dgrad_plan_classes(p, d, keep_tapless, dropped);
  if (addend == dx && addend) return 0;
  for (int i = 0; i < dropped.n; ++i) {
    const int cv = d->cin * dx_elem / 16;
    const long long n = (long long)d->groups * d->n * dropped.c[i].sub_h * dropped.c[i].sub_w * cv;
    long long blocks = (n + 255) / 256;
    if (blocks > 4096) blocks = 4096;
    hipLaunchKernelGGL(dgrad_empty_class_kernel, dim3((unsigned)blocks), dim3(256), 0, st, (uint4 *)dx, (const uint4 *)addend, n,
                       dropped.c[i].sub_h, dropped.c[i].sub_w, d->h, d->w, cv, dropped.c[i].py, dropped.c[i].px);
    if (check_launch("dgrad(empty class)")) return 1;
  }
  return 0;
}

static int wgrad_geometry(WgradParams &p, const mvg_conv_desc *d, int elem, int px_align, float *dw, float *db, float *workspace,
                          int splits, int accumulate, const char *what, int stride_w = -1, int pad_w = -1) {
  MVG_REQUIRE(splits >= 1, "%s: splits < 1", what);
  MVG_REQUIRE(splits == 1 || workspace != nullptr, "%s: workspace required for splits > 1", what);
  p.h = d->h;
  p.w = d->w;
  p.cin = d->cin;
  p.cout = d->cout;
  p.r = d->r;
  p.s = d->s;
  p.stride = d->stride;
  p.pad = d->pad;
  p.stride_w = stride_w >= 0 ? stride_w : d->stride;
  p.pad_w = stride_w >= 0 ? pad_w : d->pad;
  p.ho = d->ho;
  p.wo = d->wo;
  p.ncols = d->r * d->s * d->cin;
  p.pixels = (long long)d->groups * d->n * d->ho * d->wo;
  p.pixels_per_split = ((p.pixels + splits - 1) / splits + px_align - 1) / px_align * px_align;
  p.x_bytes = (long long)elem * d->groups * d->n * d->h * d->w * d->cin;
  p.ohw_div = make_fastdiv((unsigned)(d->ho * d->wo));
  p.wo_div = make_fastdiv((unsigned)d->wo);
  p.cin_div = make_fastdiv((unsigned)d->cin);
  p.s_div = make_fastdiv((unsigned)d->s);
  MVG_REQUIRE(p.pixels_per_split * d->cout * elem < 0x7FFFFFF0ll, "%s: split too large for 32-bit offsets", what);
  MVG_REQUIRE((long long)elem * (p.pixels_per_split / (d->ho * d->wo) + 2) * d->h * d->w * d->cin < 0x7FFFFFF0ll,
              "%s: split too large for 32-bit offsets", what);
  p.out = splits == 1 ? dw : workspace;
  p.accumulate = (splits == 1) ? accumulate : 0;
  p.db = db ? (splits == 1 ? db : workspace + (size_t)splits * d->cout * p.ncols) : nullptr;
  return 0;
}

static int wgrad_reduce_slabs(const WgradParams &p, float *workspace, float *dw, float *db, int splits, int accumulate, hipStream_t st,
                              const char *what) {
  const long long n = (long long)p.cout * p.ncols;
  MVG_REQUIRE(n % 4 == 0, "%s: weight elements %% 4 != 0", what);
  ProfScope ps(MVG_K_WGRAD_REDUCE, st, 0.0, 4.0 * n * (splits + 1));
  const int lanes = splits >= 32 ? 16 : (splits >= 8 ? 4 : 1);
  const long long blocks = (n / 4 + 256 / lanes - 1) / (256 / lanes);
  hipLaunchKernelGGL(wgrad_reduce_kernel, dim3((unsigned)blocks), dim3(256), 0, st, workspace, dw, n / 4, splits, accumulate, lanes);
  if (check_launch("wgrad_reduce")) return 1;
  if (!db) return 0;
  const long long nb = p.cout;
  const long long bblocks = (nb / 4 + 256 / lanes - 1) / (256 / lanes);
  hipLaunchKernelGGL(wgrad_reduce_kernel, dim3((unsigned)bblocks), dim3(256), 0, st, workspace + (size_t)splits * n, db, nb / 4, splits,
                     accumulate, lanes);
  return check_launch("wgrad_reduce(bias)");
}

static int wgrad_split_count(long long tiles, long long pixels, int workgroups_per_cu, int min_pixels) {
  long long want = ((long long)workgroups_per_cu * compute_cus()) / tiles;
  long long maxs = pixels / min_pixels;
  if (maxs < 1) maxs = 1;
  if (want > maxs) want = maxs;
  if (want < 1) want = 1;
  if (want > 1024) want = 1024;
  return (int)want;
}

}
```

rot-mvgaze_amd/csrc/conv_split.hip:

```cpp
#include "bf16_tile.h"
#include "elem.h"

namespace mvg {

typedef _Float16 f16x8 __attribute__((ext_vector_type(8)));

#define SPLIT_ONE(PA, PB, av, bv, acc)                                                                         \
  _Pragma("unroll") for (int i = 0; i < TM; ++i) _Pragma("unroll") for (int j = 0; j < TN; ++j)                \
      acc[i][j] = __builtin_amdgcn_mfma_f32_32x32x16_f16(av[PA][i], bv[PB][j], acc[i][j], 0, 0, 0);
#define SPLIT_PRODUCTS(av, bv, acc) SPLIT_ONE(0, 1, av, bv, acc) SPLIT_ONE(1, 0, av, bv, acc) SPLIT_ONE(0, 0, av, bv, acc)

constexpr int SP_BM = 128, SP_BK = 32;

__global__ __launch_bounds__(256) void split_f32_kernel(const float4 *__restrict__ x, uint4 *__restrict__ out, long long n8, float scale) {
  const long long stride = (long long)gridDim.x * 256;
  for (long long i = (long long)blockIdx.x * 256 + threadIdx.x; i < n8; i += stride) {
    const float4 lo = x[2 * i], hi = x[2 * i + 1];
    const float v[8] = {lo.x * scale, lo.y * scale, lo.z * scale, lo.w * scale, hi.x * scale, hi.y * scale, hi.z * scale, hi.w * scale};
    uint4 q1, q2;
    split2_chunk(v, q1, q2);
    out[2 * i] = q1;
    out[2 * i + 1] = q2;
  }
}
// ... 246 lines not shown
  }
  __device__ __forceinline__ void consts(const float *kc, int C) {
    ld8(kc, mu);
    ld8(kc + C, is);
    ld8(kc + 2 * C, ga);
    ld8(kc + 3 * C, sa);
    ld8(kc + 4 * C, sb);
  }
  __device__ __forceinline__ void form(int i, bool ok, float (&o)[8]) {
    float d[8], v[8];
    unpack8(dzv[i], d);
    unpack8(yv[i], v);
    bn_dy_chunk(d, v, mu, is, ga, sa, sb, inv_rows, dsc, o, false, mu, mu);
#pragma unroll
    for (int k = 0; k < 8; ++k) o[k] = ok ? o[k] : 0.f;
  }
  __device__ __forceinline__ void store_extra(int, unsigned) {}
};

template <bool AFFINE>
struct OutFormer {
  static constexpr int TABLES = AFFINE ? 4 : 2;
  __amdgpu_buffer_rsrc_t rs_y, rs_r;
  float osc, rsi;
  unsigned short *bits_out;
  float4 yv[2][2], rv[2][2];
  float sc[8], sh[8], rs[8], rh[8];
  unsigned mb[2];
  static __device__ __forceinline__ void stage(float *t, const IgemmParams &p, int g, int C, int tid) {
    for (int i = tid; i < C; i += 256) {
      const long long gc = (long long)g * C + i;
      t[i] = p.fap_scale[gc];
      t[C + i] = p.fap_shift[gc];
      if constexpr (AFFINE) {
        t[2 * C + i] = p.fap_res_scale[gc];
        t[3 * C + i] = p.fap_res_shift[gc];
      }
    }
  }
  __device__ __forceinline__ OutFormer(const IgemmParams &p, long long grow0, long long rows_per_group, int C)
      : rs_y(make_rsrc(p.fap_y + grow0 * C, 4ll * rows_per_group * C)),
        rs_r(make_rsrc(reinterpret_cast<const float *>(p.fap_res) + grow0 * C, 4ll * rows_per_group * C)),
        osc(__uint_as_float(__builtin_amdgcn_readfirstlane(__float_as_uint(p.a_sinv ? 1.f / *p.a_sinv : 1.f)))),
        rsi(__uint_as_float(__builtin_amdgcn_readfirstlane(__float_as_uint((!AFFINE && p.fap_res_sinv) ? *p.fap_res_sinv : 1.f)))),
        bits_out(p.fap_bits ? p.fap_bits + grow0 * (C >> 3) : nullptr) {}
  __device__ __forceinline__ void load(int i, unsigned off) {
    yv[i][0] = buf_ld16(rs_y, off);
    yv[i][1] = buf_ld16(rs_y, off + 16u);
    rv[i][0] = buf_ld16(rs_r, off);
    rv[i][1] = buf_ld16(rs_r, off + 16u);
  }
  __device__ __forceinline__ void consts(const float *kc, int C) {
    ld8(kc, sc);
    ld8(kc + C, sh);
    if constexpr (AFFINE) {
      ld8(kc + 2 * C, rs);
      ld8(kc + 3 * C, rh);
    }
  }
  __device__ __forceinline__ void form(int i, bool ok, float (&o)[8]) {
    float v[8], r[8];
    unpack8(yv[i], v);
    if constexpr (AFFINE) {
      unpack8(rv[i], r);
    } else {
      const uint4 r1 = make_uint4(__float_as_uint(rv[i][0].x), __float_as_uint(rv[i][0].y), __float_as_uint(rv[i][0].z), __float_as_uint(rv[i][0].w));
      const uint4 r2 = make_uint4(__float_as_uint(rv[i][1].x), __float_as_uint(rv[i][1].y), __float_as_uint(rv[i][1].z), __float_as_uint(rv[i][1].w));
      merge2_chunk(r1, r2, r);
    }
    mb[i] = bn_apply_chunk(v, sc, sh, true, r, AFFINE, rs, rh, !AFFINE, rsi, true, osc, o);
#pragma unroll
    for (int k = 0; k < 8; ++k) o[k] = ok ? o[k] : 0.f;
  }
  __device__ __forceinline__ void store_extra(int i, unsigned off) {
    if (bits_out) bits_out[off >> 5] = (unsigned short)mb[i];
  }
};

#define MVG_SPLIT_RNG 0
#include "conv_split_igemm.inc"
#undef MVG_SPLIT_RNG
#define MVG_SPLIT_RNG 1
#include "conv_split_igemm.inc"
#undef MVG_SPLIT_RNG

template <int BM, int BN, bool INCR>
__global__ __launch_bounds__(256, BN >= 256 ? 2 : 3) void wgrad_split_kernel(WgradParams p) {
  constexpr int BK = 16, WGM = 2, WGN = 2;
  constexpr int WTM = BM / WGM, WTN = BN / WGN;
  constexpr int TM = WTM / 32, TN = WTN / 32;
  constexpr int LDA = BM + 32, LDB = BN + 32;
  constexpr int MV = BM / 8, NVB = BN / 8;
  constexpr int A_TPR = 256 / BK;
  constexpr int A_CPT = MV / A_TPR > 0 ? MV / A_TPR : 1;
  constexpr int B_CPT = (NVB + A_TPR - 1) / A_TPR;
  constexpr int A_ELEMS = BK * LDA, B_ELEMS = BK * LDB;
  constexpr int STAGE = SP_NP * (A_ELEMS + B_ELEMS);
  __shared__ __attribute__((aligned(16))) unsigned short smem[2 * STAGE];

  const int tid = threadIdx.x;
  const int lane = tid & 63, wave = tid >> 6;
  const int wm = wave / WGN, wn = wave % WGN;
  const int li = lane & 31, lh = lane >> 5;
  const int tiles = p.mtiles * p.ntiles;
  const int logical = xcd_remap(blockIdx.x, gridDim.x);
  const int split = logical / tiles;
  const int tile = logical - split * tiles;
  const int ntile = tile % p.ntiles, mtile = tile / p.ntiles;
  const long long m_begin = (long long)split * p.pixels_per_split;
  long long m_end = m_begin + p.pixels_per_split;
  if (m_end > p.pixels) m_end = p.pixels;
  const int m_count = m_end > m_begin ? (int)(m_end - m_begin) : 0;
  const int ohw = p.ho * p.wo;
  const long long img0 = m_begin / ohw;
  const unsigned rem0 = (unsigned)(m_begin - img0 * ohw);

  const char *dy = reinterpret_cast<const char *>(p.dy);
  const char *x = reinterpret_cast<const char *>(p.x);
  const __amdgpu_buffer_rsrc_t rs_a = make_rsrc(dy + m_begin * p.cout * SP_BYTES, (long long)SP_BYTES * m_count * p.cout);
  const long long x_img_elems = (long long)p.h * p.w * p.cin;
  const __amdgpu_buffer_rsrc_t rs_b = make_rsrc(x + img0 * x_img_elems * SP_BYTES, p.x_bytes - (long long)SP_BYTES * img0 * x_img_elems);
  const int i_row = tid / A_TPR, i_v0 = tid % A_TPR;
  unsigned a_off[A_CPT];
  bool a_on[A_CPT];
#pragma unroll
  for (int j = 0; j < A_CPT; ++j) {
    const int cv = i_v0 + j * A_TPR;
    const int col = mtile * BM + cv * 8;
    a_on[j] = cv < MV;
    a_off[j] = (a_on[j] && col < p.cout) ? (unsigned)(i_row * p.cout + col) * (unsigned)SP_BYTES : 0x80000000u;
  }
  int i_dy[B_CPT], i_dx[B_CPT];
  unsigned i_tconst[B_CPT];
  bool i_cok[B_CPT], b_on[B_CPT];
#pragma unroll
  for (int j = 0; j < B_CPT; ++j) {
    const int cv = i_v0 + j * A_TPR;
    const int col = ntile * BN + cv * 8;
    b_on[j] = cv < NVB;
    i_cok[j] = b_on[j] && col < p.ncols;
    const int tap = (int)fdiv((unsigned)(i_cok[j] ? col : 0), p.cin_div);
    const int cc = (i_cok[j] ? col : 0) - tap * p.cin;
    const int fr = (int)fdiv((unsigned)tap, p.s_div), fs = tap - fr * p.s;
    i_dy[j] = fr - p.pad;
    i_dx[j] = fs - p.pad_w;
    i_tconst[j] = (unsigned)((i_dy[j] * p.w + i_dx[j]) * p.cin + cc) * (unsigned)SP_BYTES;
  }
  const unsigned row_bytes = (unsigned)(p.stride * p.w * p.cin) * (unsigned)SP_BYTES, col_bytes = (unsigned)(p.stride_w * p.cin) * (unsigned)SP_BYTES;
  const unsigned img_bytes = (unsigned)x_img_elems * (unsigned)SP_BYTES;
  int s_oy = 0, s_ox = 0;
  unsigned s_imgoff = 0;
  if (INCR) {
    const unsigned pix = rem0 + (unsigned)i_row;
    const unsigned img = fdiv(pix, p.ohw_div);
    const unsigned rem = pix - img * (unsigned)ohw;
    const unsigned oy = fdiv(rem, p.wo_div);
    s_oy = (int)oy;
    s_ox = (int)(rem - oy * (unsigned)p.wo);
    s_imgoff = img * img_bytes;
  }
  u32x4 a_reg[A_CPT][SP_NP], b_reg[B_CPT][SP_NP];
  auto load_tiles = [&](int kt) {
#pragma unroll
    for (int j = 0; j < A_CPT; ++j) {
#pragma unroll
      for (int pc = 0; pc < SP_NP; ++pc)
// ... 169 lines not shown
}

__global__ __launch_bounds__(256) void stem_rowwindow_nchw_kernel(const float *__restrict__ x, uint4 *__restrict__ xw, long long n, int h, int w) {
  const int wo = w >> 1;
  const long long plane = (long long)h * w;
  for (long long i = (long long)blockIdx.x * 256 + threadIdx.x; i < n; i += (long long)gridDim.x * 256) {
    const int q = (int)(i & 3);
    const long long t = i >> 2;
    const int ox = (int)(t % wo);
    const long long row = t / wo;
    const long long img = row / h;
    const int yy = (int)(row - img * h);
    const int c0 = 2 * ox - 4 + 2 * q;
    float v[8] = {0.f, 0.f, 0.f, 0.f, 0.f, 0.f, 0.f, 0.f};
    if (c0 >= 0 && c0 < w) {
      const float *src = x + img * 3 * plane + (long long)yy * w + c0;
      const float2 r = *reinterpret_cast<const float2 *>(src), g = *reinterpret_cast<const float2 *>(src + plane),
                   b = *reinterpret_cast<const float2 *>(src + 2 * plane);
      v[0] = r.x; v[1] = g.x; v[2] = b.x; v[4] = r.y; v[5] = g.y; v[6] = b.y;
    }
    uint4 q1, q2;
    split2_chunk(v, q1, q2);
    xw[SP_NP * i] = q1;
    xw[SP_NP * i + 1] = q2;
  }
}

static int validate_split(const mvg_conv_desc *d) {
  if (validate(d)) return 2;
  MVG_REQUIRE(d->cin % 32 == 0 && d->cout % 32 == 0, "split conv: cin and cout must be multiples of 32 (got %d, %d)", d->cin,
              d->cout);
  MVG_REQUIRE(d->r * d->s <= 32, "split conv: at most 32 filter taps");
  return 0;
}

static int split_tile_rows(int ncols, int taps, long long rows) { return (ncols < 128 && taps > 1 && rows >= 65536) ? 256 : SP_BM; }

struct SplitPlan { int bm, bn, kt_max; long long tiles; bool pipelined; };
static int split_conv_stages(const SplitPlan &pl) { return (pl.pipelined && pl.bn == 128 && pl.bm == SP_BM) ? 2 : 1; }
static SplitPlan split_plan(int ncols, int taps, long long rows, int groups, bool lin, IgemmClass *cls, int ncls) {
  SplitPlan pl;
  pl.bm = lin ? SP_BM : split_tile_rows(ncols, taps, rows);
  pl.bn = ncols >= 128 ? 128 : 64;
  if (lin && pl.bn == 128 && ncls == 1) {
    const long long t128 = (long long)groups * ceil_div(cls[0].rows_per_group, pl.bm) * ceil_div(ncols, 128);
    if (2 * t128 <= compute_cus()) pl.bn = 64;
  }
  pl.tiles = 0, pl.kt_max = 0;
  for (int i = 0; i < ncls; ++i) {
    IgemmClass &c = cls[i];
    c.mtiles_per_group = ceil_div(c.rows_per_group, pl.bm);
    c.KT = ceil_div(c.ktotal, SP_BK);
    c.tile0 = (int)pl.tiles;
    pl.tiles += (long long)groups * c.mtiles_per_group * ceil_div(ncols, pl.bn);
    pl.kt_max = c.KT > pl.kt_max ? c.KT : pl.kt_max;
  }
  pl.pipelined = pl.tiles <= 2LL * compute_cus() || (pl.tiles <= 4LL * compute_cus() && pl.kt_max >= 48);
  return pl;
}

template <bool DGRAD>
static int launch_igemm_split(IgemmParams &p, hipStream_t st, bool lin, int taps, long long rows, AForm af = A_DMA, bool ranged = false) {
  const SplitPlan pl = split_plan(p.ncols, taps, rows, p.groups, lin, p.cls, p.ncls);
  const int bm = pl.bm, bn = pl.bn;
  const bool pipelined = pl.pipelined;
  p.ntiles = ceil_div(p.ncols, bn);
  p.splits = 1;
  p.sk_tiles = 0;
  p.bn_parts = 0;
  for (int i = 0; i < p.ncls; ++i) {
    IgemmClass &c = p.cls[i];
    c.korder = c.ntaps > 1 ? 1 : 0;
    c.per_div = make_fastdiv((unsigned)(c.ntaps > 0 ? c.ntaps : 1));
    c.unit0 = 0;
    c.part0 = p.bn_parts;
    p.bn_parts += c.mtiles_per_group;
    MVG_REQUIRE((c.ntaps >= 1 || (DGRAD && p.bn_part)) && c.ntaps <= 32 && c.ktotal % SP_BK == 0, "split conv: class shape not covered");
  }
  MVG_REQUIRE(pl.tiles < (1LL << 31), "split conv: grid too large");
  if (pl.tiles <= 0) return 0;
  p.nt_out = (!lin && !(DGRAD && p.cls_step == 2)) ? 1 : 0;
  dim3 grid((unsigned)pl.tiles), block(256);
  if (af != A_DMA) {
    MVG_REQUIRE(!lin && bm == SP_BM && p.ntiles == 1 && p.ncls == 1 && DGRAD == (af == A_DY), "split conv: the operand-forming loaders take one column tile");
    if constexpr (DGRAD) {
      if (bn == 128) hipLaunchKernelGGL((igemm_split16_kernel<128, true, false, 2, 1, A_DY>), grid, block, 0, st, p);
      else hipLaunchKernelGGL((igemm_split16_kernel<64, true, false, 2, 1, A_DY>), grid, block, 0, st, p);
      return check_launch("conv_dgrad_split_bnapply");
    } else {
      if (bn == 128 && af == A_OUT_AFFINE) hipLaunchKernelGGL((igemm_split16_kernel<128, false, false, 2, 1, A_OUT_AFFINE>), grid, block, 0, st, p);
      else if (bn == 128) hipLaunchKernelGGL((igemm_split16_kernel<128, false, false, 2, 1, A_OUT_SP>), grid, block, 0, st, p);
      else if (af == A_OUT_AFFINE) hipLaunchKernelGGL((igemm_split16_kernel<64, false, false, 2, 1, A_OUT_AFFINE>), grid, block, 0, st, p);
      else hipLaunchKernelGGL((igemm_split16_kernel<64, false, false, 2, 1, A_OUT_SP>), grid, block, 0, st, p);
      return check_launch("conv_fprop_split_bnapply");
    }
  }
  if (ranged) {
    MVG_REQUIRE(!DGRAD && !lin && p.out_sp && p.out_absmax, "split conv: the range record goes with a forward that stores sp");
    if constexpr (!DGRAD) {
      if (bm == 256) hipLaunchKernelGGL((igemm_split16_ranged_kernel<64, 4>), grid, block, 0, st, p);
      else if (split_conv_stages(pl) == 2) hipLaunchKernelGGL((igemm_split16_ranged_kernel<128, 2, 2>), grid, block, 0, st, p);
      else if (bn == 128) hipLaunchKernelGGL((igemm_split16_ranged_kernel<128>), grid, block, 0, st, p);
      else hipLaunchKernelGGL((igemm_split16_ranged_kernel<64>), grid, block, 0, st, p);
    }
    return check_launch("conv_fprop_split_ranged");
  }
  if (lin) {
    if (bn == 128 && pipelined) hipLaunchKernelGGL((igemm_split16_kernel<128, DGRAD, true, 2, 2>), grid, block, 0, st, p);
    else if (bn == 128) hipLaunchKernelGGL((igemm_split16_kernel<128, DGRAD, true>), grid, block, 0, st, p);
    else if (pipelined) hipLaunchKernelGGL((igemm_split16_kernel<64, DGRAD, true, 2, 2>), grid, block, 0, st, p);
    else hipLaunchKernelGGL((igemm_split16_kernel<64, DGRAD, true>), grid, block, 0, st, p);
  } else if (bm == 256) hipLaunchKernelGGL((igemm_split16_kernel<64, DGRAD, false, 4>), grid, block, 0, st, p);
  else if (split_conv_stages(pl) == 2) hipLaunchKernelGGL((igemm_split16_kernel<128, DGRAD, false, 2, 2>), grid, block, 0, st, p);
  else if (bn == 128) hipLaunchKernelGGL((igemm_split16_kernel<128, DGRAD>), grid, block, 0, st, p);
  else hipLaunchKernelGGL((igemm_split16_kernel<64, DGRAD>), grid, block, 0, st, p);
  return check_launch(DGRAD ? "conv_dgrad_split" : "conv_fprop_split");
}

}

using namespace mvg;

extern "C" {

int mvg_split_f32(const float *x, void *out_sp, int64_t n, float scale, void *stream) {
  MVG_REQUIRE(x && out_sp && n >= 0 && n % 8 == 0, "split_f32: null argument or n %% 8 != 0");
  MVG_REQUIRE(scale > 0.f, "split_f32: scale must be positive (a power of two keeps the round trip exact)");
  if (n == 0) return 0;
  hipStream_t st = (hipStream_t)stream;
  ProfScope ps(MVG_K_LAYOUT, st, 0.0, (4.0 + SP_BYTES) * (double)n);
  long long blocks = (n / 8 + 255) / 256;
  if (blocks > 8192) blocks = 8192;
  hipLaunchKernelGGL(split_f32_kernel, dim3((unsigned)blocks), dim3(256), 0, st, (const float4 *)x, (uint4 *)out_sp, (long long)(n / 8), scale);
  return check_launch("split_f32");
}

int mvg_split_f32_ranged(const float *x, void *out_sp, int64_t n, float scale, uint32_t *range_word, void *stream) {
  MVG_REQUIRE(x && out_sp && range_word && n >= 0 && n % 8 == 0, "split_f32_ranged: null argument or n %% 8 != 0");
  MVG_REQUIRE(scale > 0.f, "split_f32_ranged: scale must be positive (a power of two keeps the round trip exact)");
  if (n == 0) return 0;
  hipStream_t st = (hipStream_t)stream;
  ProfScope ps(MVG_K_LAYOUT, st, 0.0, (4.0 + SP_BYTES) * (double)n);
  long long blocks = (n / 8 + 255) / 256;
  if (blocks > 8192) blocks = 8192;
  hipLaunchKernelGGL(split_f32_ranged_kernel, dim3((unsigned)blocks), dim3(256), 0, st, (const float4 *)x, (uint4 *)out_sp, (long long)(n / 8), scale,
                     (unsigned *)range_word);
  return check_launch("split_f32_ranged");
}

int mvg_merge_sp(const void *x_sp, float *out, int64_t n, float inv_scale, void *stream) {
  MVG_REQUIRE(x_sp && out && n >= 0 && n % 8 == 0, "merge_sp: null argument or n %% 8 != 0");
  if (n == 0) return 0;
  hipStream_t st = (hipStream_t)stream;
  ProfScope ps(MVG_K_LAYOUT, st, 0.0, (4.0 + SP_BYTES) * (double)n);
  long long blocks = (n / 8 + 255) / 256;
  if (blocks > 8192) blocks = 8192;
  hipLaunchKernelGGL(merge_sp_kernel, dim3((unsigned)blocks), dim3(256), 0, st, (const uint4 *)x_sp, (float4 *)out, (long long)(n / 8), inv_scale);
  return check_launch("merge_sp");
}

int mvg_split_weights(const mvg_conv_desc *d, const float *w, void *w_krsc_sp, void *w_crsk_sp, float *stat2, void *items_dev,
                      void *stream) {
  MVG_REQUIRE(d && w && w_krsc_sp && stat2 && items_dev, "split_weights: null argument");
  if (validate_split(d)) return 2;
  hipStream_t st = (hipStream_t)stream;
  WPrepItem it;
  memset(&it, 0, sizeof(it));
  it.w = w;
  it.wk = w_krsc_sp;
  it.wt = w_crsk_sp;
  it.cout = d->cout;
  it.rs = d->r * d->s;
  it.cin = d->cin;
  it.cin_pad = d->cin;
  it.stat = stat2;
  static_assert(sizeof(WPrepItem) <= 64, "WPrepItem grew: update the callers' table record size");
  hipLaunchKernelGGL(wprep_stage_item_kernel, dim3(1), dim3(64), 0, st, it, (WPrepItem *)items_dev);
  if (check_launch("split_weights: staging the table record")) return 1;
// ... 68 lines not shown
    p.fap_shift = fap->shift;
    p.fap_res = fap->res;
    p.fap_res_scale = fap->res_scale;
    p.fap_res_shift = fap->res_shift;
    p.fap_res_sinv = fap->res_sinv;
    p.fap_bits = (unsigned short *)fap->bits;
  }
  if (fprop_geometry(p, d, SP_BYTES, SP_BYTES, "split conv", stride_w, pad_w)) return 2;
  MVG_REQUIRE(p.rows_per_group * (long long)d->cout < (1ll << 31), "split conv: a group of the output exceeds 2^31 elements");
  const double flops = 2.0 * d->groups * (double)p.rows_per_group * d->cout * d->r * d->s * d->cin * (stride_w >= 0 ? 147.0 / 224.0 : 1.0);
  const double bytes = (double)SP_BYTES * (d->groups * (double)d->n * d->h * d->w * d->cin + (double)d->cout * d->r * d->s * d->cin) +
                       4.0 * d->groups * (double)p.rows_per_group * d->cout +
                       (fap ? 8.0 + 1.0 / 4.0 : 0.0) * d->groups * (double)d->n * d->h * d->w * d->cin;
  const bool lin = d->r == 1 && d->s == 1 && d->h == 1 && d->w == 1;
  ProfScope ps(lin ? MVG_K_LINEAR_FPROP : MVG_K_CONV_FPROP, (hipStream_t)stream, flops, bytes);
  p.stats_partials = ceil_div(p.rows_per_group, SP_BM) * 2;
  return launch_igemm_split<false>(p, (hipStream_t)stream, aff && aff->lin, d->r * d->s, p.rows_per_group,
                                   fap ? (fap->res_scale ? A_OUT_AFFINE : A_OUT_SP) : A_DMA, aff && aff->range_word);
}

int mvg_conv_fprop_split(const mvg_conv_desc *d, const void *x_sp, const float *x_sinv, const void *w_sp, const float *w_sinv, float *y,
                         float *stats, void *stream) {
  return fprop_split_impl(d, x_sp, x_sinv, w_sp, w_sinv, y, stats, stream, nullptr);
}

int mvg_conv_fprop_split_stages(const mvg_conv_desc *d) {
  if (validate_split(d)) return -1;
  IgemmClass c;
  memset(&c, 0, sizeof(c));
  c.rows_per_group = (long long)d->n * d->ho * d->wo;
  c.ktotal = d->r * d->s * d->cin;
  const SplitPlan pl = split_plan(d->cout, d->r * d->s, c.rows_per_group, d->groups, false, &c, 1);
  return split_conv_stages(pl);
}

int mvg_conv_fprop_split_bnapply(const mvg_conv_desc *d, void *out_sp, const float *out_sinv, const float *bn_y, const float *scale,
                                 const float *shift, const void *residual, int residual_sp, const float *res_scale,
                                 const float *res_shift, const float *res_sinv, uint8_t *relu_bits, const void *w_sp,
                                 const float *w_sinv, float *y, float *stats, void *stream) {
  MVG_REQUIRE(d && out_sp && bn_y && scale && shift && residual && w_sp && y, "fprop_split_bnapply: null argument");
  MVG_REQUIRE(d->r == 1 && d->s == 1 && d->stride == 1 && d->pad == 0, "fprop_split_bnapply: 1x1, stride 1, pad 0 only");
  MVG_REQUIRE(d->cout == 64 || d->cout == 128, "fprop_split_bnapply: cout must be 64 or 128 (one column tile; got %d)", d->cout);
  MVG_REQUIRE(d->cin % 32 == 0 && d->cin <= BNA_MAX_C, "fprop_split_bnapply: cin must be a multiple of 32, at most %d (got %d)", BNA_MAX_C,
              d->cin);
  MVG_REQUIRE(residual_sp ? (!res_scale && !res_shift) : (res_scale && res_shift && !res_sinv),
              "fprop_split_bnapply: the residual is an sp identity (no res_scale / res_shift) or fp32 with res_scale and res_shift");
  MVG_REQUIRE((long long)d->n * d->h * d->w * d->cin < (1ll << 29), "fprop_split_bnapply: a group of the input exceeds 2 GiB");
  const SplitFwdApply a = {bn_y, scale, shift, res_scale, res_shift, res_sinv, residual, relu_bits};
  return fprop_split_impl(d, out_sp, out_sinv, w_sp, w_sinv, y, stats, stream, nullptr, -1, -1, &a);
}

int mvg_conv_fprop_split_affine(const mvg_conv_desc *d, const void *x_sp, const float *x_sinv, const void *w_sp, const float *w_sinv,
                                void *out, int out_sp, const float *scale, const float *shift, const void *residual, int residual_sp,
                                int relu, void *stream) {
  MVG_REQUIRE(scale && shift && out, "fprop_split_affine: scale, shift and out are required");
  const SplitAffine a = {scale, shift, residual, residual_sp, relu, out_sp, 0, nullptr, nullptr, nullptr, nullptr};
  return fprop_split_impl(d, x_sp, x_sinv, w_sp, w_sinv, out, nullptr, stream, &a);
}

int mvg_conv_fprop_split_affine_ranged(const mvg_conv_desc *d, const void *x_sp, const float *x_sinv, const void *w_sp, const float *w_sinv,
                                       void *out, int out_sp, const float *scale, const float *shift, const void *residual,
                                       int residual_sp, int relu, uint32_t *range_word, void *stream) {
  MVG_REQUIRE(scale && shift && out, "fprop_split_affine_ranged: scale, shift and out are required");
  MVG_REQUIRE(range_word && out_sp, "fprop_split_affine_ranged: range_word is required and the output must be sp (out_sp != 0)");
  const SplitAffine a = {scale, shift, residual, residual_sp, relu, out_sp, 0, nullptr, nullptr, nullptr, range_word};
  return fprop_split_impl(d, x_sp, x_sinv, w_sp, w_sinv, out, nullptr, stream, &a);
}

struct SplitBnFuse {
  const float *y;
  const uint8_t *bits;
  const float *mean, *invstd, *rscale, *rshift;
  float *part;
  int part_rows;
};

struct SplitBnApply {
  const float *dz, *y, *mean, *invstd, *gamma, *s1, *s2;
  long long rows_per_group;
};

static int dgrad_split_impl(const mvg_conv_desc *d, const void *dy_sp, const float *dy_sinv, const void *w_crsk_sp, const float *w_sinv,
                            float *dx, const float *addend, void *stream, const SplitBnFuse *bnf, const void *relu_mask_sp = nullptr,
                            bool lin_kernel = false, float *out_absmax = nullptr, const SplitBnApply *bna = nullptr) {
  if (validate_split(d)) return 2;
  IgemmParams p;
  memset(&p, 0, sizeof(p));
  p.a = (const float *)dy_sp;
  p.b = (const float *)w_crsk_sp;
  p.a_sinv = dy_sinv;
  p.b_sinv = w_sinv;
  p.out = dx;
  p.addend = addend;
  p.mask = (const float *)relu_mask_sp;
  p.mask_sp = relu_mask_sp != nullptr;
  p.out_absmax = (unsigned *)out_absmax;
  if (bnf) {
    p.bn_y = bnf->y;
    p.bn_bits = bnf->bits;
    p.bn_mean = bnf->mean;
    p.bn_invstd = bnf->invstd;
    p.bn_rscale = bnf->rscale;
    p.bn_rshift = bnf->rshift;
    p.bn_part = bnf->part;
    p.bn_part_rows = bnf->part_rows;
  }
  if (bna) {
    p.bna_dz = bna->dz;
    p.bna_y = bna->y;
    p.bna_mean = bna->mean;
    p.bna_invstd = bna->invstd;
    p.bna_gamma = bna->gamma;
    p.bna_s1 = bna->s1;
    p.bna_s2 = bna->s2;
    p.bna_inv_rows = 1.0f / (float)bna->rows_per_group;
  }
  if (dgrad_geometry(p, d, SP_BYTES, SP_BYTES, "split conv")) return 2;
  MVG_REQUIRE((long long)d->n * d->h * d->w * d->cin < (1ll << 31), "split conv: a group of dx exceeds 2^31 elements");
  const double flops = 2.0 * d->groups * (double)d->n * d->ho * d->wo * d->cout * d->r * d->s * d->cin;
  const double bytes = (double)SP_BYTES * (d->groups * (double)d->n * d->ho * d->wo * d->cout + (double)d->cout * d->r * d->s * d->cin) +
                       (bnf ? 8.25 : 4.0) * d->groups * (double)d->n * d->h * d->w * d->cin +
                       (bna ? 8.0 : 0.0) * d->groups * (double)d->n * d->ho * d->wo * d->cout;
  const bool lin = d->r == 1 && d->s == 1 && d->h == 1 && d->w == 1;
  ProfScope ps(lin ? MVG_K_LINEAR_DGRAD : MVG_K_CONV_DGRAD, (hipStream_t)stream, flops, bytes);
  if (int e = dgrad_classes(p, d, bnf != nullptr, 4, dx, addend, (hipStream_t)stream)) return e;
  if (p.ncls == 0) return 0;
  return launch_igemm_split<true>(p, (hipStream_t)stream, lin_kernel, d->r * d->s, (long long)d->n * d->h * d->w, bna ? A_DY : A_DMA);
}

int mvg_conv_dgrad_split(const mvg_conv_desc *d, const void *dy_sp, const float *dy_sinv, const void *w_crsk_sp, const float *w_sinv,
                         float *dx, const float *addend, const void *relu_mask_sp, void *stream) {
  MVG_REQUIRE(!relu_mask_sp || d->stride == 1, "dgrad_split: the sp ReLU mask is for stride-1 launches (Linear layers)");
  return dgrad_split_impl(d, dy_sp, dy_sinv, w_crsk_sp, w_sinv, dx, addend, stream, nullptr, relu_mask_sp);
}

int mvg_conv_dgrad_split_stages(const mvg_conv_desc *d, int fused_reduce) {
  if (validate_split(d)) return -1;
  IgemmParams p;
  memset(&p, 0, sizeof(p));
  if (dgrad_geometry(p, d, SP_BYTES, SP_BYTES, "split conv")) return -1;
  DgradDropped dropped;
  dgrad_plan_classes(p, d, fused_reduce != 0, dropped);
  return split_conv_stages(split_plan(p.ncols, d->r * d->s, (long long)d->n * d->h * d->w, p.groups, false, p.cls, p.ncls));
}

int mvg_conv_dgrad_bn_partials_split(const mvg_conv_desc *d) {
  if (validate_split(d)) return -1;
  return dgrad_bn_partials(d, split_tile_rows(d->cin, d->r * d->s, (long long)d->n * d->h * d->w));
}

static int dgrad_split_bnreduce_impl(const char *who, const mvg_conv_desc *d, const void *dy_sp, const float *dy_sinv, const void *w_crsk_sp,
                                     const float *w_sinv, float *dx, const float *addend, const float *bn_y, const uint8_t *bn_bits,
                                     const float *bn_mean, const float *bn_invstd, const float *relu_scale, const float *relu_shift,
                                     float *partials, float *s1, float *s2, float *dgamma, float *dbeta, int accumulate, float *mx,
                                     const float *bn_gamma, float *dx_dy_sinv, void *stream, const SplitBnApply *bna) {
  MVG_REQUIRE(bn_y && bn_mean && bn_invstd && partials && s1 && s2, "%s: null argument", who);
  MVG_REQUIRE((bn_gamma == nullptr) == (dx_dy_sinv == nullptr) && (!dx_dy_sinv || mx), "%s: bn_gamma, dx_dy_sinv (and mx) go together", who);
  MVG_REQUIRE(!(bn_bits && relu_scale) && ((relu_scale == nullptr) == (relu_shift == nullptr)),
              "%s: give the ReLU mask either as bits or as (relu_scale, relu_shift)", who);
  const int P = mvg_conv_dgrad_bn_partials_split(d);
  MVG_REQUIRE(P > 0, "%s: bad descriptor", who);
  const SplitBnFuse f = {bn_y, bn_bits, bn_mean, bn_invstd, relu_scale, relu_shift, partials, mx ? 3 : 2};
  if (dgrad_split_impl(d, dy_sp, dy_sinv, w_crsk_sp, w_sinv, dx, addend, stream, &f, nullptr, false, nullptr, bna)) return 1;
  ProfScope ps(MVG_K_BN_BWD_REDUCE, (hipStream_t)stream, 0.0, 8.0 * d->groups * (double)P * d->cin);
  return bn_bwd_finalize_launch(partials, d->groups, P, d->cin, s1, s2, dgamma, dbeta, accumulate, (hipStream_t)stream, mx, nullptr, nullptr,
                                bn_gamma, bn_invstd, (long long)d->n * d->h * d->w, dx_dy_sinv);
}

int mvg_conv_dgrad_split_bnreduce(const mvg_conv_desc *d, const void *dy_sp, const float *dy_sinv, const void *w_crsk_sp,
                                  const float *w_sinv, float *dx, const float *addend, const float *bn_y, const uint8_t *bn_bits,
                                  const float *bn_mean, const float *bn_invstd, const float *relu_scale, const float *relu_shift,
                                  float *partials, float *s1, float *s2, float *dgamma, float *dbeta, int accumulate,
                                  float *mx, const float *bn_gamma, float *dx_dy_sinv, void *stream) {
  return dgrad_split_bnreduce_impl("dgrad_split_bnreduce", d, dy_sp, dy_sinv, w_crsk_sp, w_sinv, dx, addend, bn_y, bn_bits, bn_mean, bn_invstd,
                                   relu_scale, relu_shift, partials, s1, s2, dgamma, dbeta, accumulate, mx, bn_gamma, dx_dy_sinv, stream, nullptr);
}

int mvg_conv_dgrad_split_bnapply_bnreduce(const mvg_conv_desc *d, void *dy_sp, const float *dy_sinv, const float *dz, const float *y,
                                          const float *mean, const float *invstd, const float *gamma, const float *un_s1,
                                          const float *un_s2, int64_t rows_per_group, const void *w_crsk_sp, const float *w_sinv,
                                          float *dx, const float *addend, const float *bn_y, const uint8_t *bn_bits,
                                          const float *bn_mean, const float *bn_invstd, const float *relu_scale,
                                          const float *relu_shift, float *partials, float *s1, float *s2, float *dgamma, float *dbeta,
                                          int accumulate, float *mx, const float *bn_gamma, float *dx_dy_sinv, void *stream) {
  MVG_REQUIRE(d && dy_sp && dz && y && mean && invstd && gamma && un_s1 && un_s2 && w_crsk_sp && dx,
              "dgrad_split_bnapply_bnreduce: null argument");
  MVG_REQUIRE(dy_sinv, "dgrad_split_bnapply_bnreduce: dy_sinv (the 2^-k the reduce pass left for this unit's dy) is required");
  MVG_REQUIRE(d->r == 1 && d->s == 1 && d->stride == 1 && d->pad == 0, "dgrad_split_bnapply_bnreduce: 1x1, stride 1, pad 0 only");
  MVG_REQUIRE(d->cin == 64 || d->cin == 128, "dgrad_split_bnapply_bnreduce: cin must be 64 or 128 (one column tile; got %d)", d->cin);
  MVG_REQUIRE(d->cout % 32 == 0 && d->cout <= BNA_MAX_C, "dgrad_split_bnapply_bnreduce: cout must be a multiple of 32, at most %d (got %d)",
              BNA_MAX_C, d->cout);
  MVG_REQUIRE(rows_per_group == (int64_t)d->n * d->ho * d->wo, "dgrad_split_bnapply_bnreduce: rows_per_group is not n * ho * wo");
  const SplitBnApply a = {dz, y, mean, invstd, gamma, un_s1, un_s2, (long long)rows_per_group};
  return dgrad_split_bnreduce_impl("dgrad_split_bnapply_bnreduce", d, dy_sp, dy_sinv, w_crsk_sp, w_sinv, dx, addend, bn_y, bn_bits, bn_mean,
                                   bn_invstd, relu_scale, relu_shift, partials, s1, s2, dgamma, dbeta, accumulate, mx, bn_gamma, dx_dy_sinv, stream, &a);
}

static void wgrad_split_tile(const mvg_conv_desc *d, int &bm, int &bn, bool &incr) {
  incr = (long long)d->ho * d->wo >= 32;
  const int ncols = d->r * d->s * d->cin;
  bm = d->cout >= 128 ? 128 : 64;
  bn = ncols >= 128 ? 128 : 64;
  if (bm == 128 && ncols >= 256 && ncols % 256 == 0) bn = 256;
  else if (ncols % 192 == 0) bn = 192;
}

int mvg_conv_wgrad_splits_split(const mvg_conv_desc *d) {
  if (validate_split(d)) return -1;
  int bm, bn;
  bool incr;
  wgrad_split_tile(d, bm, bn, incr);
  const long long tiles = (long long)ceil_div(d->cout, bm) * ceil_div(d->r * d->s * d->cin, bn);
  return wgrad_split_count(tiles, (long long)d->groups * d->n * d->ho * d->wo, bn == 256 ? 2 : 3, 256);
}

int mvg_conv_wgrad_split_tile(const mvg_conv_desc *d, int32_t *bm, int32_t *bn, int32_t *incremental) {
  if (validate_split(d)) return -1;
  int tm, tn;
  bool incr;
  wgrad_split_tile(d, tm, tn, incr);
  if (bm) *bm = tm;
  if (bn) *bn = tn;
  if (incremental) *incremental = incr ? 1 : 0;
  return 0;
}

static int wgrad_split_impl(const mvg_conv_desc *d, const void *x_sp, const void *dy_sp, const float *dy_sinv, float *dw, float *workspace,
                            int splits, int accumulate, void *stream, int stride_w = -1, int pad_w = -1, const float *x_sinv = nullptr,
                            bool slabs_only = false) {
  if (stride_w < 0 && validate_split(d)) return 2;
  WgradParams p;
  memset(&p, 0, sizeof(p));
  p.x = (const float *)x_sp;
  p.dy = (const float *)dy_sp;
  p.dy_sinv = dy_sinv;
  p.x_sinv = x_sinv;
  if (wgrad_geometry(p, d, SP_BYTES, 16, dw, nullptr, workspace, splits, accumulate, "wgrad_split", stride_w, pad_w)) return 2;
  int bm, bn;
  bool incr;
  wgrad_split_tile(d, bm, bn, incr);
  p.mtiles = ceil_div(d->cout, bm);
  p.ntiles = ceil_div(p.ncols, bn);
  hipStream_t st = (hipStream_t)stream;
  const bool lin = d->r == 1 && d->s == 1 && d->h == 1 && d->w == 1;
  {
    const double flops = 2.0 * (double)p.pixels * d->cout * d->r * d->s * d->cin * (stride_w >= 0 ? 147.0 / 224.0 : 1.0);
    const double bytes = (double)SP_BYTES * ((double)d->groups * d->n * d->h * d->w * d->cin + (double)p.pixels * d->cout) +
                         4.0 * (double)d->cout * d->r * d->s * d->cin;
    ProfScope ps(lin ? MVG_K_LINEAR_WGRAD : MVG_K_CONV_WGRAD, st, flops, bytes);
    MVG_REQUIRE((long long)p.mtiles * p.ntiles * splits < (1LL << 31), "wgrad_split: grid too large");
    dim3 grid(p.mtiles * p.ntiles * splits), block(256);
#define MVG_WGRAD_SPLIT(BM_, BN_)                                                                  \
  do {                                                                                             \
    if (incr) hipLaunchKernelGGL((wgrad_split_kernel<BM_, BN_, true>), grid, block, 0, st, p);     \
    else hipLaunchKernelGGL((wgrad_split_kernel<BM_, BN_, false>), grid, block, 0, st, p);         \
  } while (0)
    if (bm == 128 && bn == 256) MVG_WGRAD_SPLIT(128, 256);
    else if (bm == 128 && bn == 192) MVG_WGRAD_SPLIT(128, 192);
// ... 160 lines not shown
```

rot-mvgaze_amd/csrc/conv_split_igemm.inc:

```
#ifndef MVG_SPLIT_RNG
#error "conv_split_igemm.inc: define MVG_SPLIT_RNG (0 or 1) before including"
#endif

#if MVG_SPLIT_RNG
template <int BN, int WGM = 2, int STAGES = 1>
__global__ __launch_bounds__(256, STAGES == 2 ? 2 : WGM == 4 ? 3 : 4) void igemm_split16_ranged_kernel(IgemmParams p) {
  constexpr bool DGRAD = false, LIN = false;
  constexpr AForm AF = A_DMA;
#else
template <int BN, bool DGRAD, bool LIN = false, int WGM = 2, int STAGES = 1, AForm AF = A_DMA>
__global__ __launch_bounds__(256, STAGES == 2 ? 2 : (DGRAD || WGM == 4 || AF != A_DMA) ? 3 : 4) void igemm_split16_kernel(IgemmParams p) {
#endif
  constexpr int BM = 64 * WGM, WGN = 4 / WGM, NW = 4;
  static_assert(WGM == 2 || (WGM == 4 && BN == 64), "tiles: 128 x BN (2 x 2 waves) or 256 x 64 (4 x 1)");
  static_assert(STAGES == 1 || STAGES == 2, "one LDS stage, or the two-stage pipeline");
  static_assert(AF == A_DMA || (DGRAD == (AF == A_DY) && !LIN && WGM == 2 && STAGES == 1),
                "operand-forming loaders: dy in backward-data, the block output in forward; 128-row tiles, one stage");
  using Former = std::conditional_t<AF == A_DY, DyFormer, OutFormer<AF == A_OUT_AFFINE>>;
  constexpr int WTM = BM / WGM, WTN = BN / WGN;
  constexpr int TM = WTM / 16, TN = WTN / 16;
  constexpr int SLOTS = 4 * SP_NP;
  constexpr int ROWB = 16 * SLOTS, ROWS = BM + BN, STAGE_B = ROWS * ROWB;
  constexpr int NQ = ROWS * SLOTS / 64;
  constexpr int QA = BM * SLOTS / 64;
  constexpr int A_PER = QA / NW, B_PER = (NQ - QA) / NW;
  static_assert(QA % NW == 0 && (NQ - QA) % NW == 0, "whole instructions per wave");
  constexpr int EPI_B = bf16_epilogue_bytes<BM, BN, WGM, DGRAD>();
  constexpr int INFO_OFF = STAGES * STAGE_B > EPI_B ? STAGES * STAGE_B : EPI_B;
  constexpr int BNK_OFF = INFO_OFF + BM * 8;
  constexpr int SMEM_B = BNK_OFF + (AF != A_DMA ? Former::TABLES : 0) * BNA_MAX_C * 4;
  __shared__ __attribute__((aligned(16))) unsigned char smem[SMEM_B];

  const int tid = threadIdx.x;
  const int lane = tid & 63, wave = __builtin_amdgcn_readfirstlane(tid >> 6);
  const int wm = wave / WGN, wn = wave % WGN;
  const int nwg = gridDim.x;
  const int wg_all = p.no_remap ? (int)blockIdx.x : xcd_remap(blockIdx.x, nwg);
  int ci = 0;
  for (int i = 1; i < p.ncls; ++i) ci += wg_all >= p.cls[i].tile0;
  const IgemmClass &c = p.cls[ci];
  const int wg = wg_all - c.tile0;
  const int ntile = wg % p.ntiles;
  const int mt_all = wg / p.ntiles;
  const int g = mt_all / c.mtiles_per_group;
  const int mtile = mt_all - g * c.mtiles_per_group;
  const int KT = c.KT;
  const int ohw = c.out_h * c.out_w;

  uint2 *rowinfo = reinterpret_cast<uint2 *>(smem + INFO_OFF);
  if (tid < BM) {
    const long long m = (long long)mtile * BM + tid;
    const bool ok = m < c.rows_per_group;
    const int mm = ok ? (int)m : 0;
    const int img = (int)fdiv((unsigned)mm, c.ohw_div);
    const int rem = mm - img * ohw;
    const int oy = (int)fdiv((unsigned)rem, c.ow_div), ox = rem - oy * c.out_w;
    const int y0 = DGRAD ? oy + c.cls_cy : oy * p.stride - p.pad;
    const int x0 = DGRAD ? ox + c.cls_cx : ox * p.stride_w - p.pad_w;
    const unsigned base = (unsigned)(img * p.src_img_stride * SP_BYTES) + (unsigned)((y0 * p.src_w + x0) * p.src_c) * (unsigned)SP_BYTES;
    unsigned msk = 0;
    for (int t = 0; t < c.ntaps; ++t) {
      const int fr = (int)fdiv((unsigned)t, c.tap_ns_div), fs = t - fr * c.tap_ns;
      const int iy = DGRAD ? y0 - fr : y0 + fr;
      const int ix = DGRAD ? x0 - fs : x0 + fs;
      msk |= (unsigned)(((unsigned)iy < (unsigned)p.src_h) & ((unsigned)ix < (unsigned)p.src_w)) << t;
    }
    rowinfo[tid] = make_uint2(base, ok ? msk : 0u);
  }
  if constexpr (AF != A_DMA) Former::stage(reinterpret_cast<float *>(smem + BNK_OFF), p, g, p.src_c, tid);
  __syncthreads();
  unsigned a_base[A_PER], a_vmask[A_PER], b_base[B_PER];
#pragma unroll
  for (int i = 0; i < A_PER; ++i) {
    const int sl = (wave + NW * i) * 64 + lane;
    const int row = sl / SLOTS, j = (sl % SLOTS) ^ sp_row_swz(row);
    const uint2 ri = rowinfo[row];
    a_base[i] = ri.x + 16u * (unsigned)j;
    a_vmask[i] = ri.y;
  }
#pragma unroll
  for (int i = 0; i < B_PER; ++i) {
    const int sl = (wave + NW * (A_PER + i)) * 64 + lane - BM * SLOTS;
    const int row = sl / SLOTS, j = (sl % SLOTS) ^ sp_row_swz(row);
    const int n = ntile * BN + row;
    b_base[i] = pred_off(((unsigned)n * (unsigned)p.b_row_len) * (unsigned)SP_BYTES + 16u * (unsigned)j, n < p.ncols);
  }
  const __amdgpu_buffer_rsrc_t rs_a =
      make_rsrc(reinterpret_cast<const char *>(p.a) + (long long)g * p.imgs_per_group * p.src_img_stride * SP_BYTES, p.a_group_bytes);
  const __amdgpu_buffer_rsrc_t rs_b = make_rsrc(p.b, p.b_bytes);
  typedef __attribute__((address_space(3))) void *lds_vp;

  auto issue = [&](int kt, int stage_off) {
    int kstart = kt * SP_BK;
    if (c.korder) {
      const int cblk = (int)fdiv((unsigned)kt, c.per_div), rem = kt - cblk * c.ntaps;
      kstart = (rem << p.src_c_shift) + cblk * SP_BK;
    }
    const int ks = __builtin_amdgcn_readfirstlane(kstart);
    const int tap_u = c.ntaps > 1 ? (ks >> p.src_c_shift) : 0;
    const int chb = ks - (tap_u << p.src_c_shift);
    const int fru = (int)fdiv((unsigned)tap_u, c.tap_ns_div), fsu = tap_u - fru * c.tap_ns;
    const int disp = (fru * p.src_w + fsu) * p.src_c;
    const unsigned sdelta = (unsigned)(((DGRAD ? -disp : disp) + chb) * SP_BYTES);
    unsigned kb = (unsigned)ks * (unsigned)SP_BYTES;
    if (DGRAD) {
      const int btap = (c.tap_r0 + p.tap_step * fru) * p.s + c.tap_s0 + p.tap_step * fsu;
      kb = (unsigned)(btap * p.src_c + chb) * (unsigned)SP_BYTES;
    }
    if constexpr (AF == A_DMA) {
#pragma unroll
      for (int i = 0; i < A_PER; ++i) {
        const bool ok = ((a_vmask[i] >> tap_u) & 1u) != 0u;
        __builtin_amdgcn_raw_ptr_buffer_load_lds(rs_a, (lds_vp)(smem + stage_off + (wave + NW * i) * 1024), 16, (int)pred_off(a_base[i] + sdelta, ok), 0, 0, 0);
      }
    }
#pragma unroll
    for (int i = 0; i < B_PER; ++i)
      __builtin_amdgcn_raw_ptr_buffer_load_lds(rs_b, (lds_vp)(smem + stage_off + (wave + NW * (A_PER + i)) * 1024), 16, (int)(b_base[i] + kb), 0, 0, 0);
  };

  f32x4 acc[TM][TN];
#pragma unroll
  for (int i = 0; i < TM; ++i)
#pragma unroll
    for (int j = 0; j < TN; ++j)
#pragma unroll
      for (int e = 0; e < 4; ++e) acc[i][j][e] = 0.f;

  const int cc_l = lane >> 4;
  int a_off[TM][SP_NP], b_off[TN][SP_NP];
#pragma unroll
  for (int i = 0; i < TM; ++i) {
    const int R = wm * WTM + i * 16 + (lane & 15);
#pragma unroll
    for (int pc = 0; pc < SP_NP; ++pc) a_off[i][pc] = R * ROWB + (((2 * cc_l + pc) ^ sp_row_swz(R)) << 4);
  }
#pragma unroll
  for (int j = 0; j < TN; ++j) {
    const int R = wn * WTN + j * 16 + (lane & 15);
#pragma unroll
    for (int pc = 0; pc < SP_NP; ++pc) b_off[j][pc] = (BM + R) * ROWB + (((2 * cc_l + pc) ^ sp_row_swz(R)) << 4);
// ... 22 lines not shown
      const long long m = (long long)mtile * BM + a_r0 + 64 * i;
      a_ok[i] = m < c.rows_per_group;
      a_goff[i] = pred_off((unsigned)m * (unsigned)C * 4u + 32u * (unsigned)a_cc, a_ok[i]);
    }
    auto a_load = [&](int kt) {
#pragma unroll
      for (int i = 0; i < 2; ++i) f.load(i, a_goff[i] + 128u * (unsigned)kt);
    };
    constexpr bool PREFETCH = BN == 64;
    if (PREFETCH) a_load(0);
    for (int kt = 0; kt < KT; ++kt) {
      issue(kt, 0);
      if (!PREFETCH) a_load(kt);
      uint4 q[2][SP_NP];
      f.consts(reinterpret_cast<const float *>(smem + BNK_OFF) + kt * SP_BK + a_cc * 8, C);
#pragma unroll
      for (int i = 0; i < 2; ++i) {
        float o[8];
        f.form(i, a_ok[i], o);
        split2_chunk(o, q[i][0], q[i][1]);
        const int R = a_r0 + 64 * i;
#pragma unroll
        for (int pc = 0; pc < SP_NP; ++pc)
          *reinterpret_cast<uint4 *>(smem + R * ROWB + (((2 * a_cc + pc) ^ sp_row_swz(R)) << 4)) = q[i][pc];
      }
      asm volatile("s_waitcnt vmcnt(0)" ::: "memory");
      __syncthreads();
#pragma unroll
      for (int i = 0; i < 2; ++i)
        if (a_ok[i]) {
          const unsigned off = a_goff[i] + 128u * (unsigned)kt;
          uint4 *dst = a_out + (off >> 4);
          dst[0] = q[i][0];
          dst[1] = q[i][1];
          f.store_extra(i, off);
        }
      if (PREFETCH && kt + 1 < KT) a_load(kt + 1);
      {
        f16x8 av[SP_NP][TM], bv[SP_NP][TN];
        load_frags(smem, av, bv);
        products(av, bv);
      }
      __syncthreads();
    }
  } else if constexpr (STAGES == 1) {
    for (int kt = 0; kt < KT; ++kt) {
      issue(kt, 0);
      asm volatile("s_waitcnt vmcnt(0)" ::: "memory");
      __syncthreads();
      {
        f16x8 av[SP_NP][TM], bv[SP_NP][TN];
        load_frags(smem, av, bv);
        products(av, bv);
      }
      __syncthreads();
    }
  } else {
    constexpr int G = A_PER + B_PER;
    if (KT > 0) issue(0, 0);
    if (KT > 1) {
      issue(1, STAGE_B);
      asm volatile("s_waitcnt vmcnt(%0)\n\ts_barrier" ::"n"(G) : "memory");
    } else {
      asm volatile("s_waitcnt vmcnt(0)\n\ts_barrier" ::: "memory");
    }
    f16x8 a0[SP_NP][TM], b0[SP_NP][TN], a1[SP_NP][TM], b1[SP_NP][TN];
    load_frags(smem, a0, b0);
    int cur = 0;
    auto step = [&](int kt, const f16x8 (&ca)[SP_NP][TM], const f16x8 (&cb)[SP_NP][TN], f16x8 (&na)[SP_NP][TM], f16x8 (&nb)[SP_NP][TN]) {
      if (kt + 1 < KT) {
        asm volatile("s_waitcnt vmcnt(0) lgkmcnt(0)\n\ts_barrier" ::: "memory");
        if (kt + 2 < KT) issue(kt + 2, cur);
        cur ^= STAGE_B;
        load_frags(smem + cur, na, nb);
      }
      products(ca, cb);
    };
    for (int kt = 0; kt < KT; kt += 2) {
      step(kt, a0, b0, a1, b1);
      if (kt + 1 < KT) step(kt + 1, a1, b1, a0, b0);
    }
    __syncthreads();
  }
#if MVG_SPLIT_RNG
  bf16_epilogue<BM, BN, WGM, DGRAD, true, WGM, true, DGRAD, LIN, WGN, false, true>(p, c, acc, reinterpret_cast<unsigned short *>(smem), tid, g, mtile,
                                                                                     ntile);
#else
  bf16_epilogue<BM, BN, WGM, DGRAD, true, WGM, true, DGRAD, LIN, WGN>(p, c, acc, reinterpret_cast<unsigned short *>(smem), tid, g, mtile, ntile);
#endif
}
```

rot-mvgaze_amd/ops.py:

```python
from __future__ import annotations

import ctypes as C
from typing import Optional

import torch

from ._lib import ConvDesc, K_FAMILIES, ProfEntry, check, lib

Tensor = torch.Tensor


def _p(t: Optional[Tensor]):
    if t is None:
        return None
    assert t.is_cuda and t.dtype in _PTR_DTYPES, (t.device, t.dtype)
    return t.data_ptr()


_PTR_DTYPES = frozenset((torch.float32, torch.int32, torch.uint8, torch.int16, torch.bfloat16, torch.float16))
_workspaces = {}
_MAX_WORKSPACES = 8
_raw_stream = getattr(torch._C, "_cuda_getCurrentRawStream", None)


# ... 243 lines not shown
    check(lib().mvg_conv_dgrad_split(C.byref(d), _p(dy_sp), _sinv(dy_sp), _p(wt_sp), _sinv(wt_sp), _p(dx), _p(addend), _p(relu_mask_sp),
                                     _s()), "conv_dgrad_split")


def stem_rowwindow_split(x_nhwc4: Tensor) -> Tensor:
    G, N, H, W, C = x_nhwc4.shape
    assert C == 4 and W % 2 == 0 and x_nhwc4.dtype == torch.float32 and x_nhwc4.is_contiguous()
    xw = sp_empty(G, N, H, W // 2, 32, device=x_nhwc4.device)
    check(lib().mvg_stem_rowwindow_split(_p(x_nhwc4), _p(xw), G * N, H, W, _s()), "stem_rowwindow_split")
    xw.sinv = None
    return xw


def stem_rowwindow_split_nchw(x_nchw: Tensor, out: Tensor):
    B, Cc, H, W = x_nchw.shape
    assert Cc == 3 and W % 2 == 0 and x_nchw.dtype == torch.float32 and x_nchw.is_contiguous() and is_sp(out) and out.is_contiguous()
    assert sp_shape(out) == (B, H, W // 2, 32)
    check(lib().mvg_stem_rowwindow_split_nchw(_p(x_nchw), _p(out), B, H, W, _s()), "stem_rowwindow_split_nchw")


def stem_fprop_split(d: ConvDesc, xw: Tensor, w_sp: Tensor, y: Tensor, stats: Optional[Tensor]):
    check(lib().mvg_stem_fprop_split(C.byref(d), _p(xw), _p(w_sp), _sinv(w_sp), _p(y), _p(stats), _s()), "stem_fprop_split")


def stem_wgrad_split(d: ConvDesc, xw: Tensor, dy_sp: Tensor, dw_rw: Tensor, accumulate: bool = False):
    splits, ws = _wgrad_slabs(lib().mvg_stem_wgrad_splits_split, "stem_wgrad_splits_split", d, d.cout * 224, xw.device)
    check(lib().mvg_stem_wgrad_split(C.byref(d), _p(xw), _p(dy_sp), _sinv(dy_sp), _p(dw_rw), _p(ws), splits, int(accumulate), _s()),
          "stem_wgrad_split")


def bn_relu_maxpool_bwd_reduce_split(g_pooled, argmax, y, mean, invstd, scale, shift, groups, n_per_group, h, w, c, ho, wo, s1, s2,
                                     dgamma, dbeta, accumulate, mx, gamma=None, dy_sinv=None):
    n = lib().mvg_bn_bwd_workspace_floats(groups, n_per_group * h * w, c)
    ws = torch.empty(n, dtype=torch.float32, device=y.device)
    check(lib().mvg_bn_relu_maxpool_bwd_reduce_split(_p(g_pooled), _p(argmax), _p(y), _p(mean), _p(invstd), _p(scale), _p(shift), groups,
                                                     n_per_group, h, w, c, ho, wo, _p(s1), _p(s2), _p(dgamma), _p(dbeta), int(accumulate),
                                                     _p(ws), _p(mx), _p(gamma), _p(dy_sinv), _s(True)), "bn_relu_maxpool_bwd_reduce_split")


def bn_relu_maxpool_bwd_apply_split(g_pooled, argmax, y, mean, invstd, gamma, scale, shift, s1, s2, groups, n_per_group, h, w, c, ho, wo,
                                    dy_sp, mx, dy_sinv=None):
    ready = dy_sinv is not None
    dy_sp.sinv = dy_sinv if ready else torch.empty(1, dtype=torch.float32, device=y.device)
    check(lib().mvg_bn_relu_maxpool_bwd_apply_split(_p(g_pooled), _p(argmax), _p(y), _p(mean), _p(invstd), _p(gamma), _p(scale), _p(shift),
                                                    _p(s1), _p(s2), groups, n_per_group, h, w, c, ho, wo, _p(dy_sp), _p(mx), _p(dy_sp.sinv),
                                                    int(ready), _s()), "bn_relu_maxpool_bwd_apply_split")


def stem_rowwindow_bf16(x_nchw: Tensor, out: Tensor):
    B, Cc, H, W = x_nchw.shape
    assert Cc == 3 and W % 4 == 0 and x_nchw.dtype == torch.float32 and x_nchw.is_contiguous()
    assert out.dtype == torch.bfloat16 and out.shape == (B, H, W // 4, 64) and out.is_contiguous()
    check(lib().mvg_stem_rowwindow_bf16(_p(x_nchw), _p(out), B, H, W, _s()), "stem_rowwindow_bf16")


def stem_fprop_bf16(d: ConvDesc, xw: Tensor, w_fold: Tensor, y: Tensor, stats: Optional[Tensor]):
    check(lib().mvg_stem_fprop_bf16(C.byref(d), _p(xw), _p(w_fold), _p(y), _p(stats), _s()), "stem_fprop_bf16")


def stem_wgrad_bf16(d: ConvDesc, xw: Tensor, dy: Tensor, dw_fold: Tensor, accumulate: bool = False):
    splits, ws = _wgrad_slabs(lib().mvg_stem_wgrad_splits_bf16, "stem_wgrad_splits_bf16", d, 2 * d.cout * 448, xw.device)
    check(lib().mvg_stem_wgrad_bf16(C.byref(d), _p(xw), _p(dy), _p(dw_fold), _p(ws), splits, int(accumulate), _s()), "stem_wgrad_bf16")


def conv_dgrad_bn_partials_split(d: ConvDesc) -> int:
    n = lib().mvg_conv_dgrad_bn_partials_split(C.byref(d))
    if n < 0:
        check(1, "conv_dgrad_bn_partials_split")
    return n


def conv_dgrad_split_bnreduce(d: ConvDesc, dy_sp, wt_sp, dx, addend, bn_y, bn_bits, bn_mean, bn_invstd, relu_affine, s1, s2, dgamma,
                              dbeta, accumulate: bool, mx: Optional[Tensor] = None, bn_gamma: Optional[Tensor] = None,
                              dx_dy_sinv: Optional[Tensor] = None):
    P = conv_dgrad_bn_partials_split(d)
    part = torch.empty(d.groups * P * 3 * d.cin, dtype=torch.float32, device=dx.device)
    rs, rh = relu_affine if relu_affine is not None else (None, None)
    check(lib().mvg_conv_dgrad_split_bnreduce(C.byref(d), _p(dy_sp), _sinv(dy_sp), _p(wt_sp), _sinv(wt_sp), _p(dx), _p(addend), _p(bn_y),
                                              _p(bn_bits), _p(bn_mean), _p(bn_invstd), _p(rs), _p(rh), _p(part), _p(s1), _p(s2),
                                              _p(dgamma), _p(dbeta), int(accumulate), _p(mx), _p(bn_gamma), _p(dx_dy_sinv), _s(True)),
          "conv_dgrad_split_bnreduce")


def conv_dgrad_split_bnapply_bnreduce(d: ConvDesc, dy_sp, dy_sinv, dz, y, mean, invstd, gamma, un_s1, un_s2, rows_per_group, wt_sp, dx,
                                      addend, bn_y, bn_bits, bn_mean, bn_invstd, relu_affine, s1, s2, dgamma, dbeta, accumulate: bool,
                                      mx: Optional[Tensor] = None, bn_gamma: Optional[Tensor] = None,
                                      dx_dy_sinv: Optional[Tensor] = None):
    P = conv_dgrad_bn_partials_split(d)
    part = torch.empty(d.groups * P * 3 * d.cin, dtype=torch.float32, device=dx.device)
    rs, rh = relu_affine if relu_affine is not None else (None, None)
    dy_sp.sinv = dy_sinv
    check(lib().mvg_conv_dgrad_split_bnapply_bnreduce(C.byref(d), _p(dy_sp), _p(dy_sinv), _p(dz), _p(y), _p(mean), _p(invstd), _p(gamma),
                                                      _p(un_s1), _p(un_s2), rows_per_group, _p(wt_sp), _sinv(wt_sp), _p(dx), _p(addend),
                                                      _p(bn_y), _p(bn_bits), _p(bn_mean), _p(bn_invstd), _p(rs), _p(rh), _p(part), _p(s1),
                                                      _p(s2), _p(dgamma), _p(dbeta), int(accumulate), _p(mx), _p(bn_gamma),
                                                      _p(dx_dy_sinv), _s(True)), "conv_dgrad_split_bnapply_bnreduce")


def conv_dgrad_bf16_bnreduce(d: ConvDesc, dy, wt, dx, addend, bn_y, bn_bits, bn_mean, bn_invstd, relu_affine, s1, s2, dgamma, dbeta,
                             accumulate: bool):
    P = lib().mvg_conv_dgrad_bn_partials_bf16(C.byref(d))
    if P < 1:
        check(1, "conv_dgrad_bn_partials_bf16")
    part = torch.empty(d.groups * P * 2 * d.cin, dtype=torch.float32, device=dx.device)
    rs, rh = relu_affine if relu_affine is not None else (None, None)
    check(lib().mvg_conv_dgrad_bf16_bnreduce(C.byref(d), _p(dy), _p(wt), _p(dx), _p(addend), _p(bn_y), _p(bn_bits), _p(bn_mean),
                                             _p(bn_invstd), _p(rs), _p(rh), _p(part), _p(s1), _p(s2), _p(dgamma), _p(dbeta),
                                             int(accumulate), _s()), "conv_dgrad_bf16_bnreduce")


def conv_wgrad_split(d: ConvDesc, x_sp: Tensor, dy_sp: Tensor, dw: Tensor, accumulate: bool = False, defer: Optional[list] = None):
    splits, ws = _wgrad_slabs(lib().mvg_conv_wgrad_splits_split, "conv_wgrad_splits_split", d, dw.numel(), dw.device)
    if defer is not None and splits > 1:
        check(lib().mvg_conv_wgrad_split_slabs_xs(C.byref(d), _p(x_sp), _sinv(x_sp), _p(dy_sp), _sinv(dy_sp), _p(ws), splits, _s()),
              "conv_wgrad_split_slabs")
        defer.append((ws, dw, splits, bool(accumulate)))
        return
    check(lib().mvg_conv_wgrad_split_xs(C.byref(d), _p(x_sp), _sinv(x_sp), _p(dy_sp), _sinv(dy_sp), _p(dw), _p(ws), splits,
                                        int(accumulate), _s()), "conv_wgrad_split")


def wgrad_reduce_batch(items: list):
    for i in range(0, len(items), 8):
        chunk = items[i:i + 8]
        n = len(chunk)
        for ws, dw, splits, acc in chunk:
            assert dw.dtype == torch.float32 and ws.numel() == splits * dw.numel() and dw.numel() % 4 == 0
        check(lib().mvg_wgrad_reduce_batch((C.c_void_p * n)(*[c[0].data_ptr() for c in chunk]), (C.c_void_p * n)(*[c[1].data_ptr() for c in chunk]),
                                           (C.c_int64 * n)(*[c[1].numel() for c in chunk]), (C.c_int32 * n)(*[c[2] for c in chunk]),
                                           (C.c_int32 * n)(*[int(c[3]) for c in chunk]), n, _s()), "wgrad_reduce_batch")
    items.clear()


def bn_apply_split(y, scale, shift, residual, relu, out_sp, groups, rows_per_group, c, residual_affine=None, want_bits=False):
    bits = torch.empty(groups * rows_per_group * c // 4, dtype=torch.uint8, device=y.device) if want_bits else None
    rs, rh = residual_affine if residual_affine is not None else (None, None)
    res_sp = is_sp(residual)
    check(lib().mvg_bn_apply_split_scaled(_p(y), _p(scale), _p(shift), _p(residual), int(res_sp), _p(rs), _p(rh),
                                          _sinv(residual) if res_sp else None, int(relu), _p(out_sp), _sinv(out_sp), _p(bits), groups,
                                          rows_per_group, c, _s()), "bn_apply_split")
    return bits


def act_scales(table: Tensor, n: int, slots: Tensor):
    assert table.is_cuda and table.dtype == torch.int64 and table.is_contiguous() and table.shape == (n, 4)
    assert slots.dtype == torch.float32 and slots.is_contiguous()
    check(lib().mvg_act_scales(C.c_void_p(table.data_ptr()), n, _p(slots), slots.numel(), _s()), "act_scales")


def bn_bwd_reduce_split(g, relu_bits, y, mean, invstd, groups, rows_per_group, c, s1, s2, dgamma, dbeta, accumulate, mx,
                        relu_affine=None, dz_out=None, gamma=None, dy_sinv=None):
    rs, rh = relu_affine if relu_affine is not None else (None, None)
    n = lib().mvg_bn_bwd_workspace_floats(groups, rows_per_group, c)
    ws = torch.empty(n, dtype=torch.float32, device=g.device)
    check(lib().mvg_bn_bwd_reduce_split(_p(g), _p(relu_bits), _p(y), _p(mean), _p(invstd), _p(rs), _p(rh), groups, rows_per_group, c,
                                        _p(s1), _p(s2), _p(dgamma), _p(dbeta), int(accumulate), _p(ws), _p(dz_out), _p(mx), _p(gamma),
                                        _p(dy_sinv), _s(True)), "bn_bwd_reduce_split")


def bn_bwd_apply_split(g, y, mean, invstd, gamma, s1, s2, groups, rows_per_group, c, dy_sp, relu_affine=None, mx=None, dy_sinv=None):
    rs, rh = relu_affine if relu_affine is not None else (None, None)
    assert mx is not None and mx.dtype == torch.float32 and mx.numel() == groups * c
    ready = dy_sinv is not None
    dy_sp.sinv = dy_sinv if ready else torch.empty(1, dtype=torch.float32, device=g.device)
    check(lib().mvg_bn_bwd_apply_split(_p(g), _p(y), _p(mean), _p(invstd), _p(gamma), _p(s1), _p(s2), _p(rs), _p(rh), groups,
                                       rows_per_group, c, _p(dy_sp), _p(mx), _p(dy_sp.sinv), int(ready), _s()), "bn_bwd_apply_split")
# ... 349 lines not shown
```

Before: 1682 samples/s.

## Fuse downsample shortcut gradient as compact addend into first-conv dgrad epilogue

For bottleneck blocks whose downsample is a 1x1 stride-2 conv, the backward pass now runs the shortcut branch first. It computes its data gradient as a compact stride-1 dgrad on the subsampled grid, then has the first 1x1 conv's fused BN-reduce dgrad add that compact tensor at even-parity positions in its epilogue, using parity-class tiles. This removes the separate scattered full-resolution dgrad of the stride-2 shortcut and the read-modify-write of dx that went with it. In exchange it adds a new kernel variant, extra shared memory for per-row sub-offsets, and parity tiling of the first conv's dgrad, which may change tile efficiency.

```diff
diff --git a/include/rotmvgaze.h b/include/rotmvgaze.h
--- a/include/rotmvgaze.h
+++ b/include/rotmvgaze.h
@@ -309,6 +309,12 @@
                                   const float *bn_mean, const float *bn_invstd, const float *relu_scale, const float *relu_shift,
                                   float *partials, float *s1, float *s2, float *dgamma, float *dbeta, int accumulate,
                                   float *mx, const float *bn_gamma, float *dx_dy_sinv, void *stream);
+int mvg_conv_dgrad_split_bnreduce_subaddend(const mvg_conv_desc *d, const void *dy_sp, const float *dy_sinv, const void *w_crsk_sp,
+                                            const float *w_sinv, float *dx, const float *addend_sub, int add_h, int add_w, int parity_tiles,
+                                            const float *bn_y, const uint8_t *bn_bits, const float *bn_mean, const float *bn_invstd,
+                                            const float *relu_scale, const float *relu_shift, float *partials, float *s1, float *s2,
+                                            float *dgamma, float *dbeta, int accumulate, float *mx, const float *bn_gamma,
+                                            float *dx_dy_sinv, void *stream);
 int mvg_conv_dgrad_split_bnapply_bnreduce(const mvg_conv_desc *d, void *dy_sp, const float *dy_sinv, const float *dz, const float *y,
                                           const float *mean, const float *invstd, const float *gamma, const float *un_s1,
                                           const float *un_s2, int64_t rows_per_group, const void *w_crsk_sp, const float *w_sinv,
diff --git a/rot-mvgaze_amd/_lib.py b/rot-mvgaze_amd/_lib.py
--- a/rot-mvgaze_amd/_lib.py
+++ b/rot-mvgaze_amd/_lib.py
@@ -99,6 +99,7 @@
     "mvg_bn_relu_maxpool_bwd_apply_split": (_I, [_P, _P, _P, _P, _P, _P, _P, _P, _P, _P, _I, _I, _I, _I, _I, _I, _I, _P, _P, _P, _I, _P]),
     "mvg_conv_dgrad_bn_partials_split": (_I, [_D]),
     "mvg_conv_dgrad_split_bnreduce": (_I, [_D, _P, _P, _P, _P, _P, _P, _P, _P, _P, _P, _P, _P, _P, _P, _P, _P, _P, _I, _P, _P, _P, _P]),
+    "mvg_conv_dgrad_split_bnreduce_subaddend": (_I, [_D] + [_P] * 6 + [_I, _I, _I] + [_P] * 11 + [_I, _P, _P, _P, _P]),
     "mvg_conv_dgrad_split_bnapply_bnreduce": (_I, [_D] + [_P] * 9 + [_I64] + [_P] * 15 + [_I, _P, _P, _P, _P]),
     "mvg_conv_fprop_split_stages": (_I, [_D]),
     "mvg_conv_dgrad_split_stages": (_I, [_D, _I]),
diff --git a/rot-mvgaze_amd/backbone.py b/rot-mvgaze_amd/backbone.py
--- a/rot-mvgaze_amd/backbone.py
+++ b/rot-mvgaze_amd/backbone.py
@@ -34,6 +34,20 @@
     return [blk.convs[-1].name for bi, blk in reversed(list(enumerate(spec.blocks)))
             if bn_apply_dgrad_eligible(blk.convs[-1], split=on, trained=training, fused_in=bi < nb - 1,
                                        carries_reduce=len(blk.convs) > 1, need_dimg=need_dimg)]
+
+
+def ds_addend_eligible(conv1: ConvSpec, downsample: Optional[ConvSpec], *, split: bool, trained: bool, fuse_bn_split: bool,
+                       prev_split: bool) -> bool:
+    return bool(split and trained and fuse_bn_split and prev_split and downsample is not None
+                and conv1.k == 1 and conv1.stride == 1 and conv1.pad == 0 and (conv1.cin == 64 or conv1.cin % 128 == 0)
+                and downsample.k == 1 and downsample.stride == 2 and downsample.pad == 0 and downsample.cin == conv1.cin)
+
+
+def ds_addend_blocks(spec: BackboneSpec, *, split: bool = True, bf16: bool = False, training: bool = True, fuse_bn_split: bool = True,
+                     enabled: bool = True) -> List[str]:
+    on = enabled and split and not bf16
+    return [blk.downsample.name for bi, blk in enumerate(spec.blocks)
+            if ds_addend_eligible(blk.convs[0], blk.downsample, split=on, trained=training, fuse_bn_split=fuse_bn_split, prev_split=bi > 0)]
 
 
 BN_APPLY_FPROP_MAX_CIN = 512
@@ -112,6 +126,7 @@
         self.split = os.environ.get("MVG_SPLIT", "1") != "0"
         self.fuse_bn_split = True
         self.fuse_bn_apply_dgrad = True
+        self.fuse_ds_addend = True
         self.fuse_bn_apply_fprop = True
         self.stem_rowwindow = True
         self.split_eval = True
@@ -646,11 +661,11 @@
         return self._wg_stream
 
     def _conv_bwd(self, u: _Unit, dy: Tensor, need_dx: bool, addend: Optional[Tensor], sink: GradSink,
-                  fuse_for: Optional[_Unit] = None):
+                  fuse_for: Optional[_Unit] = None, sub_addend: bool = False):
         dx = None
         if getattr(dy, "bn_apply", None) is not None:
             dx = torch.empty(ops.sp_shape(u.x_in), dtype=torch.float32, device=dy.device)
-            self._dgrad(u, dy, dx, addend, fuse_for, sink)
+            self._dgrad(u, dy, dx, addend, fuse_for, sink, sub_addend)
             need_dx = False
         if self.overlap_wgrad and dy.is_cuda:
             side = self._side(dy.device)
@@ -667,7 +682,7 @@
             self._wgrad(u, dy, sink)
         if need_dx:
             dx = torch.empty(ops.sp_shape(u.x_in), dtype=torch.float32, device=dy.device) if u.split else torch.empty_like(u.x_in)
-            self._dgrad(u, dy, dx, addend, fuse_for, sink)
+            self._dgrad(u, dy, dx, addend, fuse_for, sink, sub_addend)
         return dx
 
     def _wgrad(self, u: _Unit, dy: Tensor, sink: GradSink):
@@ -710,8 +725,10 @@
             ops.wgrad_reduce_batch(self._wg_defer)
 
     def _dgrad(self, u: _Unit, dy: Tensor, dx: Tensor, addend: Optional[Tensor], fuse_for: Optional[_Unit] = None,
-               sink: Optional[GradSink] = None):
+               sink: Optional[GradSink] = None, sub_addend: bool = False):
         U = fuse_for
+        if sub_addend:
+            assert u.split and U is not None and U.split and self.fuse_bn_split and not self.bf16 and getattr(dy, "bn_apply", None) is None
         if (self.bf16 and U is not None and self.fuse_bn_split and u.spec.cin != 3 and u.desc.cin % 64 == 0 and u.desc.cout % 64 == 0
                 and (not U.relu or U.relu_bits is not None or U.relu_affine is not None)):
             c = U.spec
@@ -736,6 +753,10 @@
                     ops.conv_dgrad_split_bnapply_bnreduce(u.desc, dy, dy.sinv, dz, y, mean, invstd, gamma, us1, us2, rows, u.w, dx,
                                                           addend, U.y, U.relu_bits, U.mean, U.invstd, ra, s12[0], s12[1],
                                                           sink.view(gp), sink.view(bp), acc, s12[2], gp.detach(), sinv)
+                elif sub_addend:
+                    ops.conv_dgrad_split_bnreduce_subaddend(u.desc, dy, u.w, dx, addend, U.y, U.relu_bits, U.mean, U.invstd, ra, s12[0],
+                                                            s12[1], sink.view(gp), sink.view(bp), acc, s12[2], gp.detach(), sinv,
+                                                            parity_tiles=True)
                 else:
                     ops.conv_dgrad_split_bnreduce(u.desc, dy, u.w, dx, addend, U.y, U.relu_bits, U.mean, U.invstd, ra, s12[0], s12[1],
                                                   sink.view(gp), sink.view(bp), acc, s12[2], gp.detach(), sinv)
@@ -800,6 +821,19 @@
                 last.spec, split=last.split and not self.bf16, trained=last.trained, fused_in=last.fused_s12 is not None,
                 carries_reduce=below.split and self.fuse_bn_split, need_dimg=need_dimg)
             dy, dz = self._bn_bwd(last, g, True, sink, defer_apply=merge)
+            ds_first = False
+            if ds_idx is not None:
+                ud, u1 = units[ds_idx], units[idx[0]]
+                ds_first = self.fuse_ds_addend and ds_addend_eligible(
+                    u1.spec, ud.spec, split=u1.split and ud.split and not self.bf16, trained=u1.trained and ud.trained,
+                    fuse_bn_split=self.fuse_bn_split, prev_split=prev_last is not None and prev_last.split)
+            if ds_first:
+                dyd, _ = self._bn_bwd(ud, dz, False, sink)
+                self._conv_bwd(ud, dyd, False, None, sink)
+                d_ds = torch.empty(V, B, ud.desc.ho, ud.desc.wo, ud.desc.cin, dtype=torch.float32, device=g.device)
+                ops.conv_dgrad_split(ops.shortcut_dgrad_desc(ud.desc), dyd, ud.w, d_ds, None)
+                ud.y = ud.out = None
+                del dyd
             d = self._conv_bwd(last, dy, True, None, sink, fuse_for=below)
             done += self._unit_params(last.spec)
             last.y = last.out = None
@@ -807,14 +841,19 @@
             for k in range(len(idx) - 2, -1, -1):
                 u = units[idx[k]]
                 dy, _ = self._bn_bwd(u, d, False, sink)
-                if k == 0:
+                if k == 0 and ds_first:
+                    d = self._conv_bwd(u, dy, True, d_ds, sink, fuse_for=prev_last, sub_addend=True)
+                    del d_ds
+                elif k == 0:
                     d = self._conv_bwd(u, dy, True, dz if ds_idx is None else None, sink,
                                        fuse_for=prev_last if ds_idx is None else None)
                 else:
                     d = self._conv_bwd(u, dy, True, None, sink, fuse_for=units[idx[k - 1]])
                 done += self._unit_params(u.spec)
                 u.y = u.out = None
-            if ds_idx is not None:
+            if ds_first:
+                done += self._unit_params(ud.spec)
+            elif ds_idx is not None:
                 ud = units[ds_idx]
                 dyd, _ = self._bn_bwd(ud, dz, False, sink)
                 self._conv_bwd(ud, dyd, False, None, sink)
diff --git a/rot-mvgaze_amd/csrc/bf16_tile.h b/rot-mvgaze_amd/csrc/bf16_tile.h
--- a/rot-mvgaze_amd/csrc/bf16_tile.h
+++ b/rot-mvgaze_amd/csrc/bf16_tile.h
@@ -41,13 +41,13 @@
   }
 }
 
-template <int BM, int BN, int PASSES, bool BNF, bool AFF = false>
+template <int BM, int BN, int PASSES, bool BNF, bool AFF = false, bool DSA = false>
 constexpr int bf16_epilogue_bytes() {
-  return (BM / PASSES) * (BN + 4) * 4 + BM * 4 + (BNF ? 4 * BN * 4 : 0) + (AFF ? 2 * BN * 4 : 0);
+  return (BM / PASSES) * (BN + 4) * 4 + BM * 4 + (BNF ? 4 * BN * 4 : 0) + (AFF ? 2 * BN * 4 : 0) + (DSA ? BM * 4 : 0);
 }
 
 template <int BM, int BN, int WGM, bool DGRAD, bool F32IO, int PASSES = 1, bool ACC16 = false, bool BNF = false, bool LIN = false, int WGN = 2,
-          bool AFF = false, bool RNG = false, class AccT>
+          bool AFF = false, bool RNG = false, bool DSA = false, class AccT>
 __device__ __forceinline__ void bf16_epilogue(const IgemmParams &p, const IgemmClass &c, AccT &acc,
                                               unsigned short *smem, int tid, int g, int mtile, int ntile) {
   constexpr int NT = WGM * WGN * 64;
@@ -65,6 +65,7 @@
   float lin_scale = 1.f, lin_max = 0.f;
   unsigned rng_max = 0u;
   static_assert(!RNG || (F32IO && !DGRAD && !LIN && !BNF && !AFF && WGM * WGN == 4), "bf16_epilogue: RNG is a forward form of the split conv kernels");
+  static_assert(!DSA || (F32IO && DGRAD && BNF && !LIN && !AFF && !RNG), "bf16_epilogue: DSA is a fused-reduce backward-data form of the split conv kernels");
   if constexpr (LIN && F32IO) {
     if (!DGRAD && p.out_sp && p.out_sinv) {
       const float bound = (float)p.ktotal * 1073741824.f * osc + (p.bias_absmax ? *p.bias_absmax : 0.f);
@@ -120,6 +121,7 @@
   constexpr int PR = BM / PASSES;
   float *ot = reinterpret_cast<float *>(smem);
   int *rowoff = reinterpret_cast<int *>(ot + PR * LDO);
+  int *suboff = rowoff + BM + 4 * BN;
   for (int r = tid; r < BM; r += NT) {
     const long long m = (long long)mtile * BM + r;
     int off = -1;
@@ -134,6 +136,17 @@
       }
     }
     rowoff[r] = off;
+    if constexpr (DSA) {
+      int so = -1;
+      if (m < c.rows_per_group) {
+        const int rr = (int)m;
+        const int img = (int)fdiv((unsigned)rr, c.ohw_div), rem = rr - img * ohw;
+        const int y2 = (int)fdiv((unsigned)rem, c.ow_div), x2 = rem - y2 * c.out_w;
+        const int y = y2 * p.cls_step + c.cls_py, x = x2 * p.cls_step + c.cls_px;
+        if (((y | x) & 1) == 0) so = ((img * p.addend_sub_h + (y >> 1)) * p.addend_sub_w + (x >> 1)) * p.ncols;
+      }
+      suboff[r] = so;
+    }
   }
   const long long gelems = DGRAD ? (long long)p.imgs_per_group * p.full_h * p.full_w * p.ncols
                                  : c.rows_per_group * (long long)p.ncols;
@@ -141,7 +154,8 @@
   const unsigned short *add_g = p.addend ? reinterpret_cast<const unsigned short *>(p.addend) + (long long)g * gelems : nullptr;
   const unsigned short *mask_g = p.mask ? reinterpret_cast<const unsigned short *>(p.mask) + (long long)g * gelems : nullptr;
   float *out_f = p.out + (long long)g * gelems;
-  const float *add_f = p.addend ? p.addend + (long long)g * gelems : nullptr;
+  const float *add_f = (p.addend && !DSA) ? p.addend + (long long)g * gelems : nullptr;
+  const float *sub_f = DSA ? p.addend + (long long)g * p.imgs_per_group * p.addend_sub_h * p.addend_sub_w * p.ncols : nullptr;
   const float *mask_f = p.mask ? p.mask + (long long)g * gelems : nullptr;
   constexpr int CV = BN / 8;
   const bool bnf = BNF && DGRAD && p.bn_part != nullptr;
@@ -404,6 +418,13 @@
         const float4 a0 = *reinterpret_cast<const float4 *>(add_f + off + colA), a1 = *reinterpret_cast<const float4 *>(add_f + off + colB);
         x[0] += a0.x; x[1] += a0.y; x[2] += a0.z; x[3] += a0.w; x[4] += a1.x; x[5] += a1.y; x[6] += a1.z; x[7] += a1.w;
       }
+      if constexpr (DSA) {
+        const int so = suboff[ph * PR + rl];
+        if (so >= 0) {
+          const float4 a0 = *reinterpret_cast<const float4 *>(sub_f + so + colA), a1 = *reinterpret_cast<const float4 *>(sub_f + so + colB);
+          x[0] += a0.x; x[1] += a0.y; x[2] += a0.z; x[3] += a0.w; x[4] += a1.x; x[5] += a1.y; x[6] += a1.z; x[7] += a1.w;
+        }
+      }
       if (bnf) {
         const float *yg = p.bn_y + (long long)g * gelems + off;
         const float4 y0 = *reinterpret_cast<const float4 *>(yg + colA), y1 = *reinterpret_cast<const float4 *>(yg + colB);
diff --git a/rot-mvgaze_amd/csrc/conv_shared.h b/rot-mvgaze_amd/csrc/conv_shared.h
--- a/rot-mvgaze_amd/csrc/conv_shared.h
+++ b/rot-mvgaze_amd/csrc/conv_shared.h
@@ -119,6 +119,7 @@
   const float *fap_y, *fap_scale, *fap_shift, *fap_res_scale, *fap_res_shift, *fap_res_sinv;
   const void *fap_res;
   unsigned short *fap_bits;
+  int addend_sub_h, addend_sub_w;
 };
 
 __device__ __forceinline__ int xcd_remap(int orig, int nwg) {
@@ -359,6 +360,28 @@
   p.no_remap = p.ncls > 1;
 }
 
+static void dgrad_parity_classes_1x1(IgemmParams &p, const mvg_conv_desc *d) {
+  p.ncls = 0;
+  for (int py = 0; py < 2; ++py)
+    for (int px = 0; px < 2; ++px) {
+      const int sub_h = (d->h - py + 1) / 2, sub_w = (d->w - px + 1) / 2;
+      if (sub_h <= 0 || sub_w <= 0) continue;
+      IgemmClass &c = p.cls[p.ncls++];
+      c = make_class(d->n, sub_h, sub_w, 1, 1, 0, 0, d->cout);
+      c.cls_py = py;
+      c.cls_px = px;
+      if (p.ncls == 1) {
+        p.rows_per_group = c.rows_per_group;
+        p.ktotal = c.ktotal;
+        p.out_h = sub_h;
+        p.out_w = sub_w;
+      }
+    }
+  p.tap_step = 1;
+  p.cls_step = 2;
+  p.no_remap = p.ncls > 1;
+}
+
 static int dgrad_classes(IgemmParams &p, const mvg_conv_desc *d, bool keep_tapless, int dx_elem, void *dx, const void *addend,
                          hipStream_t st) {
   DgradDropped dropped;
diff --git a/rot-mvgaze_amd/csrc/conv_split.hip b/rot-mvgaze_amd/csrc/conv_split.hip
--- a/rot-mvgaze_amd/csrc/conv_split.hip
+++ b/rot-mvgaze_amd/csrc/conv_split.hip
@@ -352,6 +352,12 @@
 #undef MVG_SPLIT_RNG
 #define MVG_SPLIT_RNG 1
 #include "conv_split_igemm.inc"
+#undef MVG_SPLIT_RNG
+#define MVG_SPLIT_RNG 0
+#undef MVG_SPLIT_DSA
+#define MVG_SPLIT_DSA 1
+#include "conv_split_igemm.inc"
+#undef MVG_SPLIT_DSA
 #undef MVG_SPLIT_RNG
 
 template <int BM, int BN, bool INCR>
@@ -687,7 +693,8 @@
   p.nt_out = (!lin && !(DGRAD && p.cls_step == 2)) ? 1 : 0;
   dim3 grid((unsigned)pl.tiles), block(256);
   if (af != A_DMA) {
-    MVG_REQUIRE(!lin && bm == SP_BM && p.ntiles == 1 && p.ncls == 1 && DGRAD == (af == A_DY), "split conv: the operand-forming loaders take one column tile");
+    MVG_REQUIRE(!lin && bm == SP_BM && p.ntiles == 1 && p.ncls == 1 && DGRAD == (af == A_DY) && p.addend_sub_h == 0,
+                "split conv: the operand-forming loaders take one column tile");
     if constexpr (DGRAD) {
       if (bn == 128) hipLaunchKernelGGL((igemm_split16_kernel<128, true, false, 2, 1, A_DY>), grid, block, 0, st, p);
       else hipLaunchKernelGGL((igemm_split16_kernel<64, true, false, 2, 1, A_DY>), grid, block, 0, st, p);
@@ -699,6 +706,17 @@
       else hipLaunchKernelGGL((igemm_split16_kernel<64, false, false, 2, 1, A_OUT_SP>), grid, block, 0, st, p);
       return check_launch("conv_fprop_split_bnapply");
     }
+  }
+  if (p.addend_sub_h > 0) {
+    MVG_REQUIRE(DGRAD && !lin && bm == SP_BM && p.r * p.s == 1 && p.stride == 1 && p.pad == 0 && p.bn_part && p.addend && !p.mask &&
+                    p.ncols % bn == 0 && (p.cls_step == 2 || p.ncls == 1),
+                "split conv: the sub-sampled addend goes with a 1x1 stride-1 fused-reduce backward-data of whole column tiles");
+    if constexpr (DGRAD) {
+      if (split_conv_stages(pl) == 2) hipLaunchKernelGGL((igemm_split16_subadd_kernel<128, 2>), grid, block, 0, st, p);
+      else if (bn == 128) hipLaunchKernelGGL((igemm_split16_subadd_kernel<128>), grid, block, 0, st, p);
+      else hipLaunchKernelGGL((igemm_split16_subadd_kernel<64>), grid, block, 0, st, p);
+    }
+    return check_launch("conv_dgrad_split_subaddend");
   }
   if (ranged) {
     MVG_REQUIRE(!DGRAD && !lin && p.out_sp && p.out_absmax, "split conv: the range record goes with a forward that stores sp");
@@ -933,7 +951,8 @@
 
 static int dgrad_split_impl(const mvg_conv_desc *d, const void *dy_sp, const float *dy_sinv, const void *w_crsk_sp, const float *w_sinv,
                             float *dx, const float *addend, void *stream, const SplitBnFuse *bnf, const void *relu_mask_sp = nullptr,
-                            bool lin_kernel = false, float *out_absmax = nullptr, const SplitBnApply *bna = nullptr) {
+                            bool lin_kernel = false, float *out_absmax = nullptr, const SplitBnApply *bna = nullptr, int add_sub_h = 0,
+                            int add_sub_w = 0, bool parity_tiles = false) {
   if (validate_split(d)) return 2;
   IgemmParams p;
   memset(&p, 0, sizeof(p));
@@ -943,6 +962,8 @@
   p.b_sinv = w_sinv;
   p.out = dx;
   p.addend = addend;
+  p.addend_sub_h = add_sub_h;
+  p.addend_sub_w = add_sub_w;
   p.mask = (const float *)relu_mask_sp;
   p.mask_sp = relu_mask_sp != nullptr;
   p.out_absmax = (unsigned *)out_absmax;
@@ -971,10 +992,12 @@
   const double flops = 2.0 * d->groups * (double)d->n * d->ho * d->wo * d->cout * d->r * d->s * d->cin;
   const double bytes = (double)SP_BYTES * (d->groups * (double)d->n * d->ho * d->wo * d->cout + (double)d->cout * d->r * d->s * d->cin) +
                        (bnf ? 8.25 : 4.0) * d->groups * (double)d->n * d->h * d->w * d->cin +
+                       (add_sub_h > 0 ? 4.0 : 0.0) * d->groups * (double)d->n * add_sub_h * add_sub_w * d->cin +
                        (bna ? 8.0 : 0.0) * d->groups * (double)d->n * d->ho * d->wo * d->cout;
   const bool lin = d->r == 1 && d->s == 1 && d->h == 1 && d->w == 1;
   ProfScope ps(lin ? MVG_K_LINEAR_DGRAD : MVG_K_CONV_DGRAD, (hipStream_t)stream, flops, bytes);
-  if (int e = dgrad_classes(p, d, bnf != nullptr, 4, dx, addend, (hipStream_t)stream)) return e;
+  if (parity_tiles) dgrad_parity_classes_1x1(p, d);
+  else if (int e = dgrad_classes(p, d, bnf != nullptr, 4, dx, addend, (hipStream_t)stream)) return e;
   if (p.ncls == 0) return 0;
   return launch_igemm_split<true>(p, (hipStream_t)stream, lin_kernel, d->r * d->s, (long long)d->n * d->h * d->w, bna ? A_DY : A_DMA);
 }
@@ -1004,15 +1027,20 @@
                                      const float *w_sinv, float *dx, const float *addend, const float *bn_y, const uint8_t *bn_bits,
                                      const float *bn_mean, const float *bn_invstd, const float *relu_scale, const float *relu_shift,
                                      float *partials, float *s1, float *s2, float *dgamma, float *dbeta, int accumulate, float *mx,
-                                     const float *bn_gamma, float *dx_dy_sinv, void *stream, const SplitBnApply *bna) {
+                                     const float *bn_gamma, float *dx_dy_sinv, void *stream, const SplitBnApply *bna, int add_sub_h = 0,
+                                     int add_sub_w = 0, bool parity_tiles = false) {
   MVG_REQUIRE(bn_y && bn_mean && bn_invstd && partials && s1 && s2, "%s: null argument", who);
   MVG_REQUIRE((bn_gamma == nullptr) == (dx_dy_sinv == nullptr) && (!dx_dy_sinv || mx), "%s: bn_gamma, dx_dy_sinv (and mx) go together", who);
   MVG_REQUIRE(!(bn_bits && relu_scale) && ((relu_scale == nullptr) == (relu_shift == nullptr)),
               "%s: give the ReLU mask either as bits or as (relu_scale, relu_shift)", who);
-  const int P = mvg_conv_dgrad_bn_partials_split(d);
+  mvg_conv_desc dp = *d;
+  if (parity_tiles) dp.stride = 2, dp.ho = (d->h + 1) / 2, dp.wo = (d->w + 1) / 2;
+  const int P = mvg_conv_dgrad_bn_partials_split(&dp);
   MVG_REQUIRE(P > 0, "%s: bad descriptor", who);
   const SplitBnFuse f = {bn_y, bn_bits, bn_mean, bn_invstd, relu_scale, relu_shift, partials, mx ? 3 : 2};
-  if (dgrad_split_impl(d, dy_sp, dy_sinv, w_crsk_sp, w_sinv, dx, addend, stream, &f, nullptr, false, nullptr, bna)) return 1;
+  if (dgrad_split_impl(d, dy_sp, dy_sinv, w_crsk_sp, w_sinv, dx, addend, stream, &f, nullptr, false, nullptr, bna, add_sub_h, add_sub_w,
+                       parity_tiles))
+    return 1;
   ProfScope ps(MVG_K_BN_BWD_REDUCE, (hipStream_t)stream, 0.0, 8.0 * d->groups * (double)P * d->cin);
   return bn_bwd_finalize_launch(partials, d->groups, P, d->cin, s1, s2, dgamma, dbeta, accumulate, (hipStream_t)stream, mx, nullptr, nullptr,
                                 bn_gamma, bn_invstd, (long long)d->n * d->h * d->w, dx_dy_sinv);
@@ -1025,6 +1053,24 @@
                                   float *mx, const float *bn_gamma, float *dx_dy_sinv, void *stream) {
   return dgrad_split_bnreduce_impl("dgrad_split_bnreduce", d, dy_sp, dy_sinv, w_crsk_sp, w_sinv, dx, addend, bn_y, bn_bits, bn_mean, bn_invstd,
                                    relu_scale, relu_shift, partials, s1, s2, dgamma, dbeta, accumulate, mx, bn_gamma, dx_dy_sinv, stream, nullptr);
+}
+
+int mvg_conv_dgrad_split_bnreduce_subaddend(const mvg_conv_desc *d, const void *dy_sp, const float *dy_sinv, const void *w_crsk_sp,
+                                            const float *w_sinv, float *dx, const float *addend_sub, int add_h, int add_w, int parity_tiles,
+                                            const float *bn_y, const uint8_t *bn_bits, const float *bn_mean, const float *bn_invstd,
+                                            const float *relu_scale, const float *relu_shift, float *partials, float *s1, float *s2,
+                                            float *dgamma, float *dbeta, int accumulate, float *mx, const float *bn_gamma,
+                                            float *dx_dy_sinv, void *stream) {
+  MVG_REQUIRE(d && addend_sub && dx && addend_sub != dx, "dgrad_split_bnreduce_subaddend: null argument, or the addend aliases dx");
+  MVG_REQUIRE(d->r == 1 && d->s == 1 && d->stride == 1 && d->pad == 0, "dgrad_split_bnreduce_subaddend: 1x1, stride 1, pad 0 only");
+  MVG_REQUIRE(add_h == (d->h + 1) / 2 && add_w == (d->w + 1) / 2,
+              "dgrad_split_bnreduce_subaddend: the addend is %d x %d, dx %d x %d wants %d x %d", add_h, add_w, d->h, d->w, (d->h + 1) / 2,
+              (d->w + 1) / 2);
+  MVG_REQUIRE(d->cin == 64 || d->cin % 128 == 0, "dgrad_split_bnreduce_subaddend: cin must be 64 or a multiple of 128 (whole column tiles; got %d)",
+              d->cin);
+  return dgrad_split_bnreduce_impl("dgrad_split_bnreduce_subaddend", d, dy_sp, dy_sinv, w_crsk_sp, w_sinv, dx, addend_sub, bn_y, bn_bits, bn_mean,
+                                   bn_invstd, relu_scale, relu_shift, partials, s1, s2, dgamma, dbeta, accumulate, mx, bn_gamma, dx_dy_sinv, stream,
+                                   nullptr, add_h, add_w, parity_tiles != 0);
 }
 
 int mvg_conv_dgrad_split_bnapply_bnreduce(const mvg_conv_desc *d, void *dy_sp, const float *dy_sinv, const float *dz, const float *y,
diff --git a/rot-mvgaze_amd/csrc/conv_split_igemm.inc b/rot-mvgaze_amd/csrc/conv_split_igemm.inc
--- a/rot-mvgaze_amd/csrc/conv_split_igemm.inc
+++ b/rot-mvgaze_amd/csrc/conv_split_igemm.inc
@@ -1,8 +1,17 @@
 #ifndef MVG_SPLIT_RNG
 #error "conv_split_igemm.inc: define MVG_SPLIT_RNG (0 or 1) before including"
 #endif
-
-#if MVG_SPLIT_RNG
+#ifndef MVG_SPLIT_DSA
+#define MVG_SPLIT_DSA 0
+#endif
+
+#if MVG_SPLIT_DSA
+template <int BN, int STAGES = 1>
+__global__ __launch_bounds__(256, STAGES == 2 ? 2 : 3) void igemm_split16_subadd_kernel(IgemmParams p) {
+  constexpr bool DGRAD = true, LIN = false;
+  constexpr int WGM = 2;
+  constexpr AForm AF = A_DMA;
+#elif MVG_SPLIT_RNG
 template <int BN, int WGM = 2, int STAGES = 1>
 __global__ __launch_bounds__(256, STAGES == 2 ? 2 : WGM == 4 ? 3 : 4) void igemm_split16_ranged_kernel(IgemmParams p) {
   constexpr bool DGRAD = false, LIN = false;
@@ -25,7 +34,7 @@
   constexpr int QA = BM * SLOTS / 64;
   constexpr int A_PER = QA / NW, B_PER = (NQ - QA) / NW;
   static_assert(QA % NW == 0 && (NQ - QA) % NW == 0, "whole instructions per wave");
-  constexpr int EPI_B = bf16_epilogue_bytes<BM, BN, WGM, DGRAD>();
+  constexpr int EPI_B = bf16_epilogue_bytes<BM, BN, WGM, DGRAD, false, MVG_SPLIT_DSA != 0>();
   constexpr int INFO_OFF = STAGES * STAGE_B > EPI_B ? STAGES * STAGE_B : EPI_B;
   constexpr int BNK_OFF = INFO_OFF + BM * 8;
   constexpr int SMEM_B = BNK_OFF + (AF != A_DMA ? Former::TABLES : 0) * BNA_MAX_C * 4;
@@ -55,8 +64,13 @@
     const int img = (int)fdiv((unsigned)mm, c.ohw_div);
     const int rem = mm - img * ohw;
     const int oy = (int)fdiv((unsigned)rem, c.ow_div), ox = rem - oy * c.out_w;
+#if MVG_SPLIT_DSA
+    const int y0 = oy * p.cls_step + c.cls_py;
+    const int x0 = ox * p.cls_step + c.cls_px;
+#else
     const int y0 = DGRAD ? oy + c.cls_cy : oy * p.stride - p.pad;
     const int x0 = DGRAD ? ox + c.cls_cx : ox * p.stride_w - p.pad_w;
+#endif
     const unsigned base = (unsigned)(img * p.src_img_stride * SP_BYTES) + (unsigned)((y0 * p.src_w + x0) * p.src_c) * (unsigned)SP_BYTES;
     unsigned msk = 0;
     for (int t = 0; t < c.ntaps; ++t) {
@@ -245,7 +259,10 @@
     }
     __syncthreads();
   }
-#if MVG_SPLIT_RNG
+#if MVG_SPLIT_DSA
+  bf16_epilogue<BM, BN, WGM, DGRAD, true, WGM, true, DGRAD, LIN, WGN, false, false, true>(p, c, acc, reinterpret_cast<unsigned short *>(smem), tid, g, mtile,
+                                                                                            ntile);
+#elif MVG_SPLIT_RNG
   bf16_epilogue<BM, BN, WGM, DGRAD, true, WGM, true, DGRAD, LIN, WGN, false, true>(p, c, acc, reinterpret_cast<unsigned short *>(smem), tid, g, mtile,
                                                                                      ntile);
 #else
diff --git a/rot-mvgaze_amd/ops.py b/rot-mvgaze_amd/ops.py
--- a/rot-mvgaze_amd/ops.py
+++ b/rot-mvgaze_amd/ops.py
@@ -349,6 +349,27 @@
           "conv_dgrad_split_bnreduce")
 
 
+def shortcut_dgrad_desc(d: ConvDesc) -> ConvDesc:
+    assert d.r == 1 and d.s == 1 and d.stride == 2 and d.pad == 0
+    return ConvDesc.make(d.groups, d.n, d.ho, d.wo, d.cin, d.cout, 1, 1, 0)
+
+
+def conv_dgrad_split_bnreduce_subaddend(d: ConvDesc, dy_sp, wt_sp, dx, addend_sub, bn_y, bn_bits, bn_mean, bn_invstd, relu_affine, s1, s2,
+                                        dgamma, dbeta, accumulate: bool, mx: Optional[Tensor] = None, bn_gamma: Optional[Tensor] = None,
+                                        dx_dy_sinv: Optional[Tensor] = None, parity_tiles: bool = False):
+    assert addend_sub.dtype == torch.float32 and addend_sub.is_contiguous() and not is_sp(addend_sub)
+    assert tuple(addend_sub.shape) == (d.groups, d.n, (d.h + 1) // 2, (d.w + 1) // 2, d.cin), "the compact addend's dimensions"
+    dp = ConvDesc.make(d.groups, d.n, d.h, d.w, d.cin, d.cout, 1, 2, 0) if parity_tiles else d
+    P = conv_dgrad_bn_partials_split(dp)
+    part = torch.empty(d.groups * P * 3 * d.cin, dtype=torch.float32, device=dx.device)
+    rs, rh = relu_affine if relu_affine is not None else (None, None)
+    check(lib().mvg_conv_dgrad_split_bnreduce_subaddend(C.byref(d), _p(dy_sp), _sinv(dy_sp), _p(wt_sp), _sinv(wt_sp), _p(dx), _p(addend_sub),
+                                                        addend_sub.shape[2], addend_sub.shape[3], int(parity_tiles), _p(bn_y), _p(bn_bits), _p(bn_mean),
+                                                        _p(bn_invstd), _p(rs), _p(rh), _p(part), _p(s1), _p(s2), _p(dgamma), _p(dbeta),
+                                                        int(accumulate), _p(mx), _p(bn_gamma), _p(dx_dy_sinv), _s(True)),
+          "conv_dgrad_split_bnreduce_subaddend")
+
+
 def conv_dgrad_split_bnapply_bnreduce(d: ConvDesc, dy_sp, dy_sinv, dz, y, mean, invstd, gamma, un_s1, un_s2, rows_per_group, wt_sp, dx,
                                       addend, bn_y, bn_bits, bn_mean, bn_invstd, relu_affine, s1, s2, dgamma, dbeta, accumulate: bool,
                                       mx: Optional[Tensor] = None, bn_gamma: Optional[Tensor] = None,
```

After: 1696 samples/s, median of 6. Within noise of the previous version (+0.8%).
